# angeladai/sgnn

Measured on AMD Instinct MI355X. Metric: TSDF blocks/sec fwd+bwd (64^3@5% occ, bs32), higher is better.
Workload: dtype f32

## Files before the change

include/sgnn_hip.h:

```cpp
#ifndef SGNN_HIP_H
#define SGNN_HIP_H

#include <stdint.h>

#ifdef __cplusplus
extern "C" {
#endif

#define SGNN_OK 0
#define SGNN_EINVAL (-1)
#define SGNN_EHIP (-2)
#define SGNN_EOVERFLOW (-3)
#define SGNN_ENOWS (-4)

#define SGNN_STATUS_COORD_RANGE 1
#define SGNN_STATUS_DUPLICATE 2
#define SGNN_STATUS_OVERFLOW 4

typedef void *sgnn_stream_t;

const char *sgnn_last_error(void);
int sgnn_version(void);
const char *sgnn_arch(void);

// ... 7 lines not shown

int sgnn_hash_build(const int32_t *coords, int64_t n, uint64_t *keys, int32_t *vals, int64_t cap,
                    int32_t *status, const int64_t *n_dev, sgnn_stream_t stream);

int sgnn_hash_lookup(const uint64_t *keys, const int32_t *vals, int64_t cap, const int32_t *query,
                     int64_t m, int32_t *rows, const int64_t *m_dev, sgnn_stream_t stream);

#define SGNN_TUNE_UNKNOWN INT64_MIN
typedef struct sgnn_tune {
  int64_t conv_small;
  int64_t conv_small_rows;
  int64_t conv_unrolled;
  int64_t conv_one_round;
  int64_t conv_wide_epi;
  int64_t conv_dw_blocks;
  int64_t conv_dw_c1;
  int64_t rulebook_multi;
  int64_t scan_inline;
  int64_t chain_merged;
  int64_t prog_fusion;
  int64_t prog_lin_bn;
  int64_t prog_lin_add;
  int64_t bn_fuse;
} sgnn_tune;
int64_t sgnn_tune_set(const char *name, int64_t value);
int64_t sgnn_tune_get(const char *name);
const char *sgnn_tune_names(void);
const sgnn_tune *sgnn_tune_current(void);


int sgnn_rulebook_subm3(const uint64_t *keys, const int32_t *vals, int64_t cap,
                        const int32_t *coords, int64_t n, int32_t *nbr, int64_t ld,
                        const int64_t *n_dev, sgnn_stream_t stream);

#define SGNN_RULEBOOK_MULTI_MAX 4
int sgnn_rulebook_subm3_multi(int count, const uint64_t *const *keys, const int32_t *const *vals, const int64_t *caps,
                              const int32_t *const *coords, const int64_t *ns, int32_t *const *nbrs, const int64_t *lds,
                              const int64_t *const *n_devs, sgnn_stream_t stream);

int sgnn_rulebook_subm3_dense(const uint64_t *keys, const int32_t *vals, int64_t cap, const int32_t *coords, int64_t n,
                              int dim_z, int dim_y, int dim_x, int32_t *volume, int64_t volume_entries, int32_t *nbr,
                              int64_t ld, const int64_t *n_dev, sgnn_stream_t stream);
int sgnn_rulebook_subm3_volume(const int32_t *coords, int64_t n, int dim_z, int dim_y, int dim_x, int32_t *volume,
                               int64_t volume_entries, int32_t *nbr, int64_t ld, const int64_t *n_dev, int32_t *status,
                               sgnn_stream_t stream);

int64_t sgnn_down2_ws_bytes(int64_t nf);
int sgnn_rulebook_down2(const int32_t *fine_coords, int64_t nf, uint64_t *ckeys, int32_t *cvals,
                        int64_t ccap, int32_t *parent, int32_t *coarse_coords, int64_t *n_coarse,
                        void *ws, int64_t ws_bytes, sgnn_stream_t stream);
int sgnn_down2_tables(const int32_t *fine_coords, const int32_t *parent, int64_t nf,
                      int32_t *children, int64_t ldc, int64_t nc, int32_t *ptable, int64_t ldf,
                      const int64_t *nf_dev, const int64_t *nc_dev, sgnn_stream_t stream);

int64_t sgnn_down2_chain_ws_bytes(int64_t cap);
int sgnn_down2_chain(const int32_t *fine_coords, int64_t n0, const int64_t *n0_dev, int64_t cap, int depth,
                     void *const *ckeys, void *const *cvals, int64_t ccap, void *const *parent,
                     void *const *coarse_coords, int64_t *counts_dev, const int64_t *level_caps, int32_t *status,
                     void *ws, int64_t ws_bytes, sgnn_stream_t stream);

int64_t sgnn_down2_chain_tables_ws_bytes(int64_t cap, int depth);
int sgnn_down2_chain_tables(const int32_t *fine_coords, const int64_t *n0_dev, int64_t cap, int depth,
                            void *const *ckeys, void *const *cvals, int64_t ccap, void *const *parent,
                            void *const *coarse_coords, int64_t *counts_dev, const int64_t *level_caps,
                            void *const *children, void *const *ptable, int32_t *status, void *ws, int64_t ws_bytes,
                            sgnn_stream_t stream);

#define SGNN_CONV_TRANSPOSE_W 1
#define SGNN_CONV_FLIP_K 2
int sgnn_conv_fwd(const float *x, int64_t n_in, int cin, const float *w, int K, const int32_t *table,
                  int64_t ld, int64_t n_out, int cout, float *y, int flags, int in_shift,
                  sgnn_stream_t stream);

int sgnn_conv_fwd_ex(const float *x, int64_t n_in, int cin, const float *w, int K, const int32_t *table,
                     int64_t ld, int64_t n_out, int cout, float *y, int flags, int in_shift,
                     const int32_t *kmap, const int32_t *kadd, int in_mul, int groups, int table_rows,
                     sgnn_stream_t stream);
int sgnn_conv_bwd_weight_ex(const float *x, int64_t n_in, int cin, const float *dy, int cout,
                            const int32_t *table, int64_t ld, int K, int64_t n_out, float *dw, int in_shift,
                            const int32_t *kmap, const int32_t *kadd, int in_mul, int groups, int table_rows,
                            void *ws, int64_t ws_bytes, sgnn_stream_t stream);

int64_t sgnn_conv_stats_blocks(int64_t n_out);
int sgnn_conv_fwd_epi(const float *x, int64_t n_in, int cin, int64_t ldx, const float *w, int K,
                      const int32_t *table, int64_t ld, int64_t n_out, int cout, float *y, int64_t ldy, int flags,
                      const float *addend, int64_t ld_add, int stats, double *partial, const float *bn_x,
                      int64_t ld_bnx, const float *mean, const float *invstd, const float *gamma, const float *beta,
                      float leak, sgnn_stream_t stream);

int64_t sgnn_conv_bwd_weight_ws_bytes(int64_t n_out, int K, int cin, int cout);
int sgnn_conv_bwd_weight(const float *x, int64_t n_in, int cin, const float *dy, int cout,
                         const int32_t *table, int64_t ld, int K, int64_t n_out, float *dw, int in_shift, void *ws,
                         int64_t ws_bytes, sgnn_stream_t stream);

int sgnn_expand_weights(const float *w, int cin, int cout, float *wc, sgnn_stream_t stream);
int sgnn_expand_weights_bwd(const float *dwc, int cin, int cout, float *dw, sgnn_stream_t stream);

int64_t sgnn_bn_ws_bytes(int64_t n, int c);
int sgnn_bn_fwd(const float *x, int64_t n, int c, const float *gamma, const float *beta,
                float *running_mean, float *running_var, float eps, float momentum, int training,
                float leak, float *save_mean, float *save_invstd, float *y, void *ws,
                int64_t ws_bytes, sgnn_stream_t stream);
int sgnn_bn_bwd(const float *x, const float *dy, int64_t n, int c, const float *gamma,
                const float *beta, const float *save_mean, const float *save_invstd, int training,
                float leak, float *dx, float *dgamma, float *dbeta, void *ws, int64_t ws_bytes,
                sgnn_stream_t stream);
int sgnn_bn_bwd_add(const float *x, const float *dy, int64_t n, int c, const float *gamma, const float *beta,
                    const float *save_mean, const float *save_invstd, int training, float leak,
                    const float *addend, float *dx, float *dgamma, float *dbeta, void *ws, int64_t ws_bytes,
                    sgnn_stream_t stream);

int sgnn_bn_fwd_ex(const float *x, int64_t ldx, int64_t n, int c, const float *gamma, const float *beta,
                   float *running_mean, float *running_var, float eps, float momentum, int training, float leak,
                   float *save_mean, float *save_invstd, float *y, int64_t ldy, const double *pre_partial,
                   int64_t pre_nblk, void *ws, int64_t ws_bytes, sgnn_stream_t stream);
int sgnn_bn_bwd_ex(const float *x, int64_t ldx, const float *dy, int64_t ld_dy, int64_t n, int c, const float *gamma,
                   const float *beta, const float *save_mean, const float *save_invstd, int training, float leak,
                   const float *addend, int64_t ld_add, float *dx, int64_t ld_dx, float *dgamma, float *dbeta,
                   const double *pre_partial, int64_t pre_nblk, void *ws, int64_t ws_bytes, sgnn_stream_t stream);

int sgnn_copy_multi(void *const *dst, const void *const *src, const int64_t *bytes, int nregions, sgnn_stream_t stream);

int sgnn_gather_rows(const float *src, int c, const int32_t *idx, int64_t m, float *dst,
                     sgnn_stream_t stream);
int sgnn_gather_rows_dn(const float *src, int c, const int32_t *idx, const int64_t *m_dev, int64_t m_cap,
                        float *dst, sgnn_stream_t stream);
int sgnn_concat3_rows(const float *a, int ca, const int32_t *ia, const float *b, int cb, const int32_t *ib,
                      const float *c, int cc, const int32_t *ic, int64_t m, float *dst, sgnn_stream_t stream);
int sgnn_concat3_rows_bwd(const float *ddst, int ca, const int32_t *ia, int cb, const int32_t *ib, int cc,
                          const int32_t *ic, int64_t m, float *da, int64_t na, float *db, int64_t nb, float *dc,
                          int64_t nc, sgnn_stream_t stream);
int sgnn_scatter_rows(const float *src, int c, const int32_t *idx, int64_t m, float *dst,
                      int64_t n_dst, const int64_t *m_dev, sgnn_stream_t stream);
int sgnn_gather_sum(const float *src, int c, const int32_t *table, int64_t ld, int K,
                    int64_t n_out, float *dst, sgnn_stream_t stream);
int sgnn_repeat_rows(const float *src, int c, int64_t n, int rep, float *dst, sgnn_stream_t stream);
int sgnn_sum_groups(const float *src, int c, int64_t n, int rep, float *dst, sgnn_stream_t stream);
int sgnn_concat_rows(const float *a, int ca, const int32_t *ia, const float *b, int cb,
                     const int32_t *ib, int64_t m, float *dst, sgnn_stream_t stream);
int sgnn_concat_rows_bwd(const float *ddst, int ca, const int32_t *ia, int cb, const int32_t *ib,
                         int64_t m, float *da, int64_t na, float *db, int64_t nb,
// ... 15 lines not shown
                             int64_t *count2, int64_t keep_cap, int32_t *status, void *ws, int64_t ws_bytes,
                             sgnn_stream_t stream);
int sgnn_compact_dense_cap(const int32_t *coords, int64_t n, const int64_t *n_dev, const float *vol, int batch, int d0,
                           int d1, int d2, int32_t *sel, int64_t *count2, int64_t keep_cap, int32_t *status, void *ws,
                           int64_t ws_bytes, sgnn_stream_t stream);
int sgnn_compact_sigmoid_cap_locs(const float *logits, int64_t stride, int64_t n, const int64_t *n_dev,
                                  const int32_t *coords, int32_t *sel, int32_t *locs, int64_t *count2, int64_t keep_cap,
                                  int32_t *status, void *ws, int64_t ws_bytes, sgnn_stream_t stream);
int sgnn_compact_dense_cap_locs(const int32_t *coords, int64_t n, const int64_t *n_dev, const float *vol, int batch, int d0,
                                int d1, int d2, int32_t *sel, int32_t *locs, int64_t *count2, int64_t keep_cap,
                                int32_t *status, void *ws, int64_t ws_bytes, sgnn_stream_t stream);

int sgnn_sparse_to_dense(const float *feats, const int32_t *coords, int64_t n, int c, float *dense,
                         int batch, int d0, int d1, int d2, sgnn_stream_t stream);
int sgnn_dense_to_sparse(const float *dense, const int32_t *coords, int64_t n, int c, float *feats,
                         int batch, int d0, int d1, int d2, sgnn_stream_t stream);

int64_t sgnn_linear_ws_bytes(int64_t n, int cin, int cout);
int sgnn_linear_fwd(const float *x, int64_t n, int cin, const float *w, const float *bias, int cout,
                    float *y, sgnn_stream_t stream);
int sgnn_linear_bwd(const float *x, const float *dy, int64_t n, int cin, const float *w, int cout,
                    float *dx, float *dw, float *dbias, void *ws, int64_t ws_bytes,
                    sgnn_stream_t stream);

int64_t sgnn_loss_multi_ws_bytes(void);
int sgnn_loss_levels_fwd(const int64_t *levels, int n, const float *coef_host, double *sums, float *out2s, float *total,
                         float *cur, void *ws, int64_t ws_bytes, sgnn_stream_t stream);
int sgnn_loss_levels_bwd(const int64_t *levels, int n, const float *coef_host, const double *sums, const float *g,
                         void *const *dvals, sgnn_stream_t stream);

int sgnn_loss_targets(const float *sdf, const uint8_t *known, const int64_t *input_locs, int64_t n_locs,
                      const int64_t *n_locs_dev, int batch,
                      int d0, int d1, int d2, float trunc, int masking, float weight_missing_geo, int ncoarse,
                      void *const *hier_in, float *tsdf, float *hier_last, float *occ_last, float *w_last,
                      void *const *occ, void *const *w, void *const *hier, sgnn_stream_t stream);

int64_t sgnn_prog_arena_floats(const int32_t *ops, int nops, const int32_t *bufs, int nbuf, int n_ext,
                               const int64_t *lev_n, int nlev, const int32_t *keep, int mode);
int64_t sgnn_prog_ws_bytes(const int32_t *ops, int nops, const int64_t *lev_n, int nlev);
int64_t sgnn_prog_buffer_offset(const int32_t *ops, int nops, const int32_t *bufs, int nbuf, int n_ext,
                                const int64_t *lev_n, int nlev, const int32_t *keep, int infer, int b);
int sgnn_prog_plan(const int32_t *ops, int nops, const int32_t *bufs, int nbuf, int n_ext, const int64_t *lev_n,
                   int nlev, const int32_t *keep, int mode, int32_t *out);
int sgnn_prog_forward(const int32_t *ops, const float *opf, int nops, const int32_t *bufs, int nbuf, int n_ext,
                      const int64_t *lev_n, const int64_t *lev_ld, void *const *lev_nbr,
                      void *const *lev_children, void *const *lev_ptable, void *const *lev_parent,
                      void *const *lev_cnt, int nlev, void *const *params, int nparams,
                      void *const *ext, void *const *idx, int nidx,
                      float *arena, int64_t arena_floats, const int32_t *keep, int training, void *wait_event,
                      void *ws, int64_t ws_bytes, sgnn_stream_t stream);
int sgnn_prog_backward(const int32_t *ops, const float *opf, int nops, const int32_t *bufs, int nbuf, int n_ext,
                       const int64_t *lev_n, const int64_t *lev_ld, void *const *lev_nbr,
                       void *const *lev_children, void *const *lev_ptable, void *const *lev_parent,
                       void *const *lev_cnt, int nlev, void *const *params, void *const *pgrads,
                       int nparams, void *const *ext,
                       void *const *gext, void *const *idx, int nidx, const float *arena, float *garena,
                       int64_t arena_floats, void *const *gout, const int32_t *keep, int training, void *ws,
                       int64_t ws_bytes, sgnn_stream_t stream);

int sgnn_prog_set_side_stream(sgnn_stream_t stream2, void *ws2, int64_t ws2_bytes);
int sgnn_prog_defer_join(int on);
int64_t sgnn_bf16_conv_ws_bytes(int cin, int cout, int K, int expand);
int sgnn_bf16_conv_fwd(const void *x, int64_t n_in, int cin, int64_t ldx, const float *w, int K, const int32_t *table,
                       int64_t ld, int64_t n_out, int cout, void *y, int64_t ldy, const void *addend, int64_t ld_add,
                       const int64_t *n_dev, void *ws, int64_t ws_bytes, sgnn_stream_t stream);
int sgnn_bf16_conv_expand(const void *x, int64_t n, int cin, int64_t ldx, const float *w, const int32_t *nbr, int64_t ld,
                          int cout, void *y, int64_t ldy, const int64_t *n_dev, void *ws, int64_t ws_bytes,
                          sgnn_stream_t stream);
int sgnn_bf16_bn_eval(const void *x, int64_t ldx, int64_t n, int c, const float *gamma, const float *beta,
                      const float *running_mean, const float *running_var, float eps, float leak, void *y, int64_t ldy,
                      const int64_t *n_dev, sgnn_stream_t stream);
int sgnn_bf16_gather_rows(const void *x, int64_t ldx, int c, const int32_t *idx, int64_t m, void *y, int64_t ldy,
                          const int64_t *n_dev, sgnn_stream_t stream);
int sgnn_bf16_add(const void *a, int64_t lda, const void *b, int64_t ldb, int64_t n, int c, void *y, int64_t ldy,
                  const int64_t *n_dev, sgnn_stream_t stream);
int sgnn_bf16_join(const void *a, int64_t lda, int ca, const void *b, int64_t ldb, int cb, int64_t n, void *y, int64_t ldy,
                   const int64_t *n_dev, sgnn_stream_t stream);
int sgnn_bf16_concat3(const float *a, int ca, const int32_t *ia, const float *b, int cb, const int32_t *ib, const float *c,
                      int cc, const int32_t *ic, int64_t m, void *y, int64_t ldy, const int64_t *n_dev, sgnn_stream_t stream);
int sgnn_bf16_linear(const void *x, int64_t ldx, int64_t n, int cin, const float *w, const float *bias, int cout, float *y,
                     const int64_t *n_dev, sgnn_stream_t stream);
int sgnn_bf16_to_f32(const void *x, int64_t ldx, int64_t n, int c, float *y, const int64_t *n_dev, sgnn_stream_t stream);
int sgnn_adam_flat(float *params, const float *grads, float *exp_avg, float *exp_avg_sq, int64_t n, const int64_t *seg,
                   int nseg, const float *lr_dev, float beta1, float beta2, float eps, float weight_decay,
                   float grad_scale, const int32_t *status, sgnn_stream_t stream);
int sgnn_seg_flags(const int64_t *cnt_ptrs, int nseg, float *flags, const int32_t *status, sgnn_stream_t stream);
int sgnn_status_merge(const float *overflow_flag, int32_t *status, sgnn_stream_t stream);

int sgnn_io_layout(const void *bytes, int64_t nbytes, int kind, int64_t *out);
int sgnn_io_flag_entries(const uint32_t *locs_xyz, const float *vals, const float *voxelsize,
                         const int64_t *seg, int nb, int64_t n, float truncation, int64_t max_z,
                         uint8_t *mask, sgnn_stream_t stream);
int sgnn_io_emit_entries(const uint32_t *locs_xyz, const float *vals, const float *voxelsize,
                         const int64_t *seg, int nb, const int32_t *sel, const int64_t *count,
                         int64_t n_max, int64_t *out_locs, float *out_feats, sgnn_stream_t stream);
int sgnn_io_scatter_dense(const uint32_t *locs_xyz, const float *vals, const float *voxelsize,
                          const int64_t *seg, int nb, int64_t n, int d0, int d1, int d2, int64_t max_z,
                          float *dense, sgnn_stream_t stream);

typedef struct sgnn_fuse_frame {
  float m[12];
  float intr[4];
  int32_t box[6];
  int64_t offset;
} sgnn_fuse_frame;
int sgnn_fuse_depth_raw(const uint16_t *raw, int nframes, int h_raw, int w_raw, int h, int w, float depth_shift,
// ... 200 lines not shown
```

sgnn_amd/_lib.py:

```python
import ctypes
import os

import torch

_HERE = os.path.dirname(os.path.abspath(__file__))
LIB_PATH = os.environ.get('SGNN_LIB') or os.path.join(_HERE, 'lib', 'libsgnn_hip.so')

c_i32, c_i64, c_f32, c_vp, c_cp = ctypes.c_int, ctypes.c_int64, ctypes.c_float, ctypes.c_void_p, ctypes.c_char_p

PROTOTYPES = {
    'sgnn_last_error': (c_cp, []),
    'sgnn_version': (c_i32, []),
    'sgnn_arch': (c_cp, []),
    'sgnn_tune_set': (c_i64, [c_cp, c_i64]),
    'sgnn_tune_get': (c_i64, [c_cp]),
    'sgnn_tune_names': (c_cp, []),
    'sgnn_tune_current': (c_vp, []),
    'sgnn_hash_capacity': (c_i64, [c_i64]),
    'sgnn_coords_from_i64': (c_i32, [c_vp, c_i64, c_vp, c_vp, c_vp, c_vp]),
    'sgnn_coords_to_i64': (c_i32, [c_vp, c_i64, c_vp, c_vp, c_vp]),
    'sgnn_hash_build': (c_i32, [c_vp, c_i64, c_vp, c_vp, c_i64, c_vp, c_vp, c_vp]),
    'sgnn_hash_lookup': (c_i32, [c_vp, c_vp, c_i64, c_vp, c_i64, c_vp, c_vp, c_vp]),
    'sgnn_rulebook_subm3': (c_i32, [c_vp, c_vp, c_i64, c_vp, c_i64, c_vp, c_i64, c_vp, c_vp]),
    'sgnn_rulebook_subm3_multi': (c_i32, [c_i32, c_vp, c_vp, c_vp, c_vp, c_vp, c_vp, c_vp, c_vp, c_vp]),
    'sgnn_rulebook_subm3_dense': (c_i32, [c_vp, c_vp, c_i64, c_vp, c_i64, c_i32, c_i32, c_i32, c_vp, c_i64, c_vp, c_i64, c_vp, c_vp]),
    'sgnn_rulebook_subm3_volume': (c_i32, [c_vp, c_i64, c_i32, c_i32, c_i32, c_vp, c_i64, c_vp, c_i64, c_vp, c_vp, c_vp]),
    'sgnn_down2_ws_bytes': (c_i64, [c_i64]),
    'sgnn_rulebook_down2': (c_i32, [c_vp, c_i64, c_vp, c_vp, c_i64, c_vp, c_vp, c_vp, c_vp, c_i64, c_vp]),
    'sgnn_down2_chain_ws_bytes': (c_i64, [c_i64]),
    'sgnn_down2_chain': (c_i32, [c_vp, c_i64, c_vp, c_i64, c_i32, c_vp, c_vp, c_i64, c_vp, c_vp, c_vp, c_vp, c_vp, c_vp, c_i64, c_vp]),
    'sgnn_down2_chain_tables_ws_bytes': (c_i64, [c_i64, c_i32]),
    'sgnn_down2_chain_tables': (c_i32, [c_vp, c_vp, c_i64, c_i32, c_vp, c_vp, c_i64, c_vp, c_vp, c_vp, c_vp, c_vp, c_vp, c_vp, c_vp,
                                        c_i64, c_vp]),
    'sgnn_down2_tables': (c_i32, [c_vp, c_vp, c_i64, c_vp, c_i64, c_i64, c_vp, c_i64, c_vp, c_vp, c_vp]),
    'sgnn_conv_fwd': (c_i32, [c_vp, c_i64, c_i32, c_vp, c_i32, c_vp, c_i64, c_i64, c_i32, c_vp, c_i32, c_i32, c_vp]),
    'sgnn_conv_fwd_ex': (c_i32, [c_vp, c_i64, c_i32, c_vp, c_i32, c_vp, c_i64, c_i64, c_i32, c_vp, c_i32, c_i32, c_vp, c_vp, c_i32, c_i32, c_i32, c_vp]),
    'sgnn_conv_bwd_weight_ex': (c_i32, [c_vp, c_i64, c_i32, c_vp, c_i32, c_vp, c_i64, c_i32, c_i64, c_vp, c_i32, c_vp, c_vp, c_i32, c_i32, c_i32, c_vp, c_i64, c_vp]),
    'sgnn_conv_stats_blocks': (c_i64, [c_i64]),
    'sgnn_conv_fwd_epi': (c_i32, [c_vp, c_i64, c_i32, c_i64, c_vp, c_i32, c_vp, c_i64, c_i64, c_i32, c_vp, c_i64, c_i32, c_vp, c_i64, c_i32, c_vp, c_vp, c_i64, c_vp, c_vp, c_vp, c_vp, c_f32, c_vp]),
    'sgnn_conv_bwd_weight_ws_bytes': (c_i64, [c_i64, c_i32, c_i32, c_i32]),
    'sgnn_conv_bwd_weight': (c_i32, [c_vp, c_i64, c_i32, c_vp, c_i32, c_vp, c_i64, c_i32, c_i64, c_vp, c_i32, c_vp, c_i64, c_vp]),
    'sgnn_bn_ws_bytes': (c_i64, [c_i64, c_i32]),
    'sgnn_bn_fwd': (c_i32, [c_vp, c_i64, c_i32, c_vp, c_vp, c_vp, c_vp, c_f32, c_f32, c_i32, c_f32, c_vp, c_vp, c_vp, c_vp, c_i64, c_vp]),
    'sgnn_bn_bwd': (c_i32, [c_vp, c_vp, c_i64, c_i32, c_vp, c_vp, c_vp, c_vp, c_i32, c_f32, c_vp, c_vp, c_vp, c_vp, c_i64, c_vp]),
    'sgnn_bn_bwd_add': (c_i32, [c_vp, c_vp, c_i64, c_i32, c_vp, c_vp, c_vp, c_vp, c_i32, c_f32, c_vp, c_vp, c_vp, c_vp, c_vp, c_i64, c_vp]),
    'sgnn_bn_fwd_ex': (c_i32, [c_vp, c_i64, c_i64, c_i32, c_vp, c_vp, c_vp, c_vp, c_f32, c_f32, c_i32, c_f32, c_vp, c_vp, c_vp, c_i64, c_vp, c_i64, c_vp, c_i64, c_vp]),
    'sgnn_bn_bwd_ex': (c_i32, [c_vp, c_i64, c_vp, c_i64, c_i64, c_i32, c_vp, c_vp, c_vp, c_vp, c_i32, c_f32, c_vp, c_i64, c_vp, c_i64, c_vp, c_vp, c_vp, c_i64, c_vp, c_i64, c_vp]),
    'sgnn_copy_multi': (c_i32, [c_vp, c_vp, c_vp, c_i32, c_vp]),
    'sgnn_gather_rows': (c_i32, [c_vp, c_i32, c_vp, c_i64, c_vp, c_vp]),
    'sgnn_gather_rows_dn': (c_i32, [c_vp, c_i32, c_vp, c_vp, c_i64, c_vp, c_vp]),
    'sgnn_scatter_rows': (c_i32, [c_vp, c_i32, c_vp, c_i64, c_vp, c_i64, c_vp, c_vp]),
    'sgnn_gather_sum': (c_i32, [c_vp, c_i32, c_vp, c_i64, c_i32, c_i64, c_vp, c_vp]),
    'sgnn_repeat_rows': (c_i32, [c_vp, c_i32, c_i64, c_i32, c_vp, c_vp]),
    'sgnn_sum_groups': (c_i32, [c_vp, c_i32, c_i64, c_i32, c_vp, c_vp]),
    'sgnn_concat_rows': (c_i32, [c_vp, c_i32, c_vp, c_vp, c_i32, c_vp, c_i64, c_vp, c_vp]),
    'sgnn_concat_rows_bwd': (c_i32, [c_vp, c_i32, c_vp, c_i32, c_vp, c_i64, c_vp, c_i64, c_vp, c_i64, c_vp]),
    'sgnn_add': (c_i32, [c_vp, c_vp, c_i64, c_vp, c_vp]),
    'sgnn_expand8_coords': (c_i32, [c_vp, c_i64, c_vp, c_vp, c_vp]),
    'sgnn_expand8_coords_i64': (c_i32, [c_vp, c_i64, c_vp, c_vp, c_vp, c_vp]),
    'sgnn_dense_coords': (c_i32, [c_i32, c_i32, c_i32, c_i32, c_vp, c_vp]),
    'sgnn_compact_ws_bytes': (c_i64, [c_i64]),
    'sgnn_compact_sigmoid': (c_i32, [c_vp, c_i64, c_i64, c_vp, c_vp, c_vp, c_i64, c_vp]),
    'sgnn_compact_dense': (c_i32, [c_vp, c_i64, c_vp, c_i32, c_i32, c_i32, c_i32, c_vp, c_vp, c_vp, c_i64, c_vp]),
    'sgnn_compact_mask': (c_i32, [c_vp, c_i64, c_vp, c_vp, c_vp, c_i64, c_vp]),
    'sgnn_compact_sigmoid_cap': (c_i32, [c_vp, c_i64, c_i64, c_vp, c_vp, c_vp, c_i64, c_vp, c_vp, c_i64, c_vp]),
    'sgnn_compact_dense_cap': (c_i32, [c_vp, c_i64, c_vp, c_vp, c_i32, c_i32, c_i32, c_i32, c_vp, c_vp, c_i64, c_vp, c_vp, c_i64, c_vp]),
    'sgnn_compact_sigmoid_cap_locs': (c_i32, [c_vp, c_i64, c_i64, c_vp, c_vp, c_vp, c_vp, c_vp, c_i64, c_vp, c_vp, c_i64, c_vp]),
    'sgnn_compact_dense_cap_locs': (c_i32, [c_vp, c_i64, c_vp, c_vp, c_i32, c_i32, c_i32, c_i32, c_vp, c_vp, c_vp, c_i64, c_vp, c_vp, c_i64, c_vp]),
    'sgnn_adam_flat': (c_i32, [c_vp, c_vp, c_vp, c_vp, c_i64, c_vp, c_i32, c_vp, c_f32, c_f32, c_f32, c_f32, c_f32, c_vp, c_vp]),
    'sgnn_seg_flags': (c_i32, [c_vp, c_i32, c_vp, c_vp, c_vp]),
    'sgnn_status_merge': (c_i32, [c_vp, c_vp, c_vp]),
    'sgnn_sparse_to_dense': (c_i32, [c_vp, c_vp, c_i64, c_i32, c_vp, c_i32, c_i32, c_i32, c_i32, c_vp]),
    'sgnn_dense_to_sparse': (c_i32, [c_vp, c_vp, c_i64, c_i32, c_vp, c_i32, c_i32, c_i32, c_i32, c_vp]),
    'sgnn_linear_ws_bytes': (c_i64, [c_i64, c_i32, c_i32]),
    'sgnn_linear_fwd': (c_i32, [c_vp, c_i64, c_i32, c_vp, c_vp, c_i32, c_vp, c_vp]),
    'sgnn_linear_bwd': (c_i32, [c_vp, c_vp, c_i64, c_i32, c_vp, c_i32, c_vp, c_vp, c_vp, c_vp, c_i64, c_vp]),
    'sgnn_loss_targets': (c_i32, [c_vp, c_vp, c_vp, c_i64, c_vp, c_i32, c_i32, c_i32, c_i32, c_f32, c_i32, c_f32, c_i32, c_vp, c_vp, c_vp,
                                  c_vp, c_vp, c_vp, c_vp, c_vp, c_vp]),
    'sgnn_loss_multi_ws_bytes': (c_i64, []),
    'sgnn_loss_levels_fwd': (c_i32, [c_vp, c_i32, c_vp, c_vp, c_vp, c_vp, c_vp, c_vp, c_i64, c_vp]),
    'sgnn_loss_levels_bwd': (c_i32, [c_vp, c_i32, c_vp, c_vp, c_vp, c_vp, c_vp]),
    'sgnn_prog_arena_floats': (c_i64, [c_vp, c_i32, c_vp, c_i32, c_i32, c_vp, c_i32, c_vp, c_i32]),
    'sgnn_prog_ws_bytes': (c_i64, [c_vp, c_i32, c_vp, c_i32]),
    'sgnn_prog_buffer_offset': (c_i64, [c_vp, c_i32, c_vp, c_i32, c_i32, c_vp, c_i32, c_vp, c_i32, c_i32]),
    'sgnn_prog_plan': (c_i32, [c_vp, c_i32, c_vp, c_i32, c_i32, c_vp, c_i32, c_vp, c_i32, c_vp]),
    'sgnn_prog_set_side_stream': (c_i32, [c_vp, c_vp, c_i64]),
    'sgnn_prog_defer_join': (c_i32, [c_i32]),
    'sgnn_bf16_conv_ws_bytes': (c_i64, [c_i32, c_i32, c_i32, c_i32]),
    'sgnn_bf16_conv_fwd': (c_i32, [c_vp, c_i64, c_i32, c_i64, c_vp, c_i32, c_vp, c_i64, c_i64, c_i32, c_vp, c_i64, c_vp,
                                   c_i64, c_vp, c_vp, c_i64, c_vp]),
    'sgnn_bf16_conv_expand': (c_i32, [c_vp, c_i64, c_i32, c_i64, c_vp, c_vp, c_i64, c_i32, c_vp, c_i64, c_vp, c_vp, c_i64,
                                      c_vp]),
    'sgnn_bf16_bn_eval': (c_i32, [c_vp, c_i64, c_i64, c_i32, c_vp, c_vp, c_vp, c_vp, c_f32, c_f32, c_vp, c_i64, c_vp, c_vp]),
    'sgnn_bf16_gather_rows': (c_i32, [c_vp, c_i64, c_i32, c_vp, c_i64, c_vp, c_i64, c_vp, c_vp]),
    'sgnn_bf16_add': (c_i32, [c_vp, c_i64, c_vp, c_i64, c_i64, c_i32, c_vp, c_i64, c_vp, c_vp]),
    'sgnn_bf16_join': (c_i32, [c_vp, c_i64, c_i32, c_vp, c_i64, c_i32, c_i64, c_vp, c_i64, c_vp, c_vp]),
    'sgnn_bf16_concat3': (c_i32, [c_vp, c_i32, c_vp, c_vp, c_i32, c_vp, c_vp, c_i32, c_vp, c_i64, c_vp, c_i64, c_vp, c_vp]),
    'sgnn_bf16_linear': (c_i32, [c_vp, c_i64, c_i64, c_i32, c_vp, c_vp, c_i32, c_vp, c_vp, c_vp]),
    'sgnn_bf16_to_f32': (c_i32, [c_vp, c_i64, c_i64, c_i32, c_vp, c_vp, c_vp]),
    'sgnn_prog_forward': (c_i32, [c_vp, c_vp, c_i32, c_vp, c_i32, c_i32, c_vp, c_vp, c_vp, c_vp, c_vp, c_vp, c_vp, c_i32, c_vp,
                                  c_i32, c_vp, c_vp, c_i32, c_vp, c_i64, c_vp, c_i32, c_vp, c_vp, c_i64, c_vp]),
    'sgnn_prog_backward': (c_i32, [c_vp, c_vp, c_i32, c_vp, c_i32, c_i32, c_vp, c_vp, c_vp, c_vp, c_vp, c_vp, c_vp, c_i32, c_vp,
                                   c_vp, c_i32, c_vp, c_vp, c_vp, c_i32, c_vp, c_vp, c_i64, c_vp, c_vp, c_i32, c_vp, c_i64, c_vp]),
    'sgnn_concat3_rows': (c_i32, [c_vp, c_i32, c_vp, c_vp, c_i32, c_vp, c_vp, c_i32, c_vp, c_i64, c_vp, c_vp]),
    'sgnn_concat3_rows_bwd': (c_i32, [c_vp, c_i32, c_vp, c_i32, c_vp, c_i32, c_vp, c_i64, c_vp, c_i64, c_vp, c_i64, c_vp,
                                      c_i64, c_vp]),
    'sgnn_expand_weights': (c_i32, [c_vp, c_i32, c_i32, c_vp, c_vp]),
    'sgnn_expand_weights_bwd': (c_i32, [c_vp, c_i32, c_i32, c_vp, c_vp]),
    'sgnn_io_layout': (c_i32, [c_vp, c_i64, c_i32, c_vp]),
    'sgnn_io_flag_entries': (c_i32, [c_vp, c_vp, c_vp, c_vp, c_i32, c_i64, c_f32, c_i64, c_vp, c_vp]),
    'sgnn_io_emit_entries': (c_i32, [c_vp, c_vp, c_vp, c_vp, c_i32, c_vp, c_vp, c_i64, c_vp, c_vp, c_vp]),
    'sgnn_io_scatter_dense': (c_i32, [c_vp, c_vp, c_vp, c_vp, c_i32, c_i64, c_i32, c_i32, c_i32, c_i64, c_vp, c_vp]),
    'sgnn_fuse_depth_raw': (c_i32, [c_vp, c_i32, c_i32, c_i32, c_i32, c_i32, c_f32, c_f32, c_f32, c_vp, c_vp]),
    'sgnn_fuse_bilateral': (c_i32, [c_vp, c_i32, c_i32, c_i32, c_f32, c_f32, c_vp, c_vp]),
    'sgnn_fuse_integrate': (c_i32, [c_vp, c_vp, c_vp, c_i32, c_i32, c_i32, c_vp, c_i32, c_i32, c_vp, c_i32, c_i32, c_f32,
                                    c_f32, c_f32, c_vp, c_vp]),
    'sgnn_fuse_flag': (c_i32, [c_vp, c_i32, c_i32, c_i32, c_f32, c_f32, c_f32, c_i64, c_vp, c_vp]),
    'sgnn_fuse_emit_block': (c_i32, [c_vp, c_i32, c_i32, c_vp, c_vp, c_i64, c_vp, c_vp, c_vp]),
    'sgnn_fuse_emit_rows': (c_i32, [c_vp, c_i32, c_i32, c_f32, c_vp, c_vp, c_i64, c_vp, c_vp, c_vp]),
    'sgnn_fuse_known': (c_i32, [c_vp, c_i64, c_f32, c_vp, c_vp]),
    'sgnn_fusecol_pack': (c_i32, [c_vp, c_i32, c_i32, c_i32, c_i32, c_i32, c_i32, c_vp, c_vp]),
    'sgnn_fusecol_integrate': (c_i32, [c_vp, c_vp, c_vp, c_vp, c_i32, c_i32, c_i32, c_vp, c_vp, c_i32, c_i32, c_vp, c_i32,
                                       c_i32, c_f32, c_f32, c_f32, c_vp, c_vp]),
    'sgnn_fusecol_export': (c_i32, [c_vp, c_i64, c_vp, c_vp, c_vp]),
    'sgnn_chunk_score': (c_i32, [c_vp, c_vp, c_i32, c_i32, c_i32, c_f32, c_f32, c_f32, c_i32, c_i32, c_i32, c_i32, c_i32,
                                 c_i32, c_i32, c_i32, c_i32, c_vp, c_vp, c_vp]),
    'sgnn_chunk_flag': (c_i32, [c_vp, c_i32, c_i32, c_i32, c_vp, c_i32, c_i32, c_i32, c_i32, c_f32, c_f32, c_f32, c_vp,
                                c_vp]),
    'sgnn_chunk_emit_rows': (c_i32, [c_vp, c_i32, c_i32, c_i32, c_vp, c_i32, c_i32, c_i32, c_i32, c_f32, c_vp, c_vp,
                                     c_i64, c_vp, c_vp, c_vp]),
    'sgnn_chunk_crop': (c_i32, [c_vp, c_i32, c_i32, c_i32, c_vp, c_i32, c_i32, c_i32, c_i32, c_i32, c_f32, c_f32, c_vp,
                                c_vp, c_vp]),
    'sgnn_render_depth': (c_i32, [c_vp, c_i32, c_vp, c_i32, c_vp, c_i32, c_i32, c_i32, c_i32, c_f32, c_f32, c_f32, c_i32,
                                  c_vp, c_vp, c_vp, c_vp]),
    'sgnn_rendercol_draw': (c_i32, [c_vp, c_i32, c_vp, c_i32, c_vp, c_i32, c_i32, c_i32, c_i32, c_f32, c_f32, c_f32,
                                    c_i32, c_vp, c_vp, c_vp, c_vp, c_vp, c_vp, c_vp]),
    'sgnn_meshdist_pack': (c_i32, [c_vp, c_i32, c_vp, c_i32, c_vp, c_vp, c_vp, c_vp, c_vp]),
    'sgnn_meshdist_count': (c_i32, [c_vp, c_i32, c_f32, c_f32, c_f32, c_f32, c_i32, c_i32, c_i32, c_vp, c_vp]),
    'sgnn_meshdist_fill': (c_i32, [c_vp, c_i32, c_f32, c_f32, c_f32, c_f32, c_i32, c_i32, c_i32, c_vp, c_vp, c_vp, c_vp]),
    'sgnn_meshdist_query': (c_i32, [c_vp, c_i64, c_vp, c_vp, c_vp, c_f32, c_f32, c_f32, c_f32, c_f32, c_f32, c_f32, c_i32,
                                    c_i32, c_i32, c_f32, c_vp, c_vp, c_vp, c_vp]),
    'sgnn_mesh_sample': (c_i32, [c_vp, c_vp, c_i32, c_i32, c_i64, c_i64, c_vp, c_vp, c_vp]),
    'sgnn_raycast_bricks': (c_i32, [c_vp, c_i32, c_i32, c_i32, c_f32, c_vp, c_vp]),
    'sgnn_raycast_cast': (c_i32, [c_vp, c_i32, c_i32, c_i32, c_f32, c_vp, c_vp, c_i32, c_i32, c_i32, c_i32, c_f32, c_f32,
                                  c_i32, c_vp, c_vp, c_vp, c_vp]),
    'sgnn_raycol_cast': (c_i32, [c_vp, c_i32, c_i32, c_i32, c_f32, c_vp, c_vp, c_i32, c_i32, c_i32, c_i32, c_f32, c_f32,
                                 c_i32, c_vp, c_vp, c_vp, c_vp, c_vp, c_vp]),
    'sgnn_track_halve': (c_i32, [c_vp, c_i32, c_i32, c_i32, c_f32, c_vp, c_vp]),
    'sgnn_track_normals': (c_i32, [c_vp, c_vp, c_i32, c_i32, c_i32, c_f32, c_vp, c_vp]),
    'sgnn_track_system': (c_i32, [c_vp, c_vp, c_i32, c_i32, c_vp, c_vp, c_i32, c_i32, c_vp, c_i32, c_f32, c_f32, c_vp, c_vp,
                                  c_vp, c_vp, c_i64, c_vp]),
    'sgnn_cc_volume_link': (c_i32, [c_vp, c_i32, c_i32, c_i32, c_i32, c_i32, c_i32, c_vp, c_vp]),
    'sgnn_cc_mesh_link': (c_i32, [c_vp, c_i32, c_i32, c_vp, c_vp, c_vp]),
    'sgnn_cc_flatten': (c_i32, [c_vp, c_i64, c_vp, c_vp]),
    'sgnn_cc_relabel': (c_i32, [c_vp, c_i64, c_vp, c_i64, c_vp, c_vp, c_vp]),
# ... 150 lines not shown
```

sgnn_amd/csrc/common.h:

```cpp
#pragma once
#include <hip/hip_runtime.h>
#include <stdint.h>
#include <stdio.h>
#include "../../include/sgnn_hip.h"

#define SGNN_EXPORT extern "C" __attribute__((visibility("default")))

extern "C" int sgnn_stamp(const char *label, sgnn_stream_t stream);
extern sgnn_tune g_tune;

void sgnn_set_error(const char *fmt, ...);
int sgnn_prof_begin_launch(int kind, int64_t n_out, int cin, int cout, int K, int flags, hipStream_t s);
void sgnn_prof_end_launch(int slot, hipStream_t s);

__device__ __forceinline__ float sgnn_bn_act(float x, float mean, float invstd, float gamma, float beta, float leak) {
  const float xh = (x - mean) * invstd;
  const float t = fmaf(xh, gamma, beta);
  return t > 0.f ? t : t * leak;
}

struct ConvEpi {
  int64_t ldx, ldy, ld_add;
  const float *addend;
  int stats;
  double *partial;
  const float *bn_x;
  int64_t ld_bnx;
  const float *mean, *invstd, *gamma, *beta;
  float leak;
  const int64_t *n_dev;
};

int sgnn_conv_fwd_impl(const float *x, int64_t n_in, int cin, const float *w, int K, const int32_t *table, int64_t ld,
                       int64_t n_out, int cout, float *y, int flags, int in_shift, const int32_t *kmap,
                       const int32_t *kadd, int in_mul, int groups, int table_rows, const ConvEpi *epi,
                       sgnn_stream_t stream);
int64_t sgnn_conv_grid_blocks(int64_t n_out, int cin, int cout, int K);
struct BnLin {
  const float *g;
  int64_t ldg;
  const float *w[2];
  int nout;
};
int sgnn_bn_fwd_impl(const float *x, int64_t ldx, int64_t n, int c, const float *gamma, const float *beta,
                     float *running_mean, float *running_var, float eps, float momentum, int training, float leak,
                     float *save_mean, float *save_invstd, float *y, int64_t ldy, const double *pre_partial,
                     int64_t pre_nblk, void *ws, int64_t ws_bytes, sgnn_stream_t stream, const int64_t *n_dev = nullptr);
int sgnn_bn_bwd_impl(const float *x, int64_t ldx, const float *dy, int64_t ld_dy, int64_t n, int c, const float *gamma,
                     const float *beta, const float *save_mean, const float *save_invstd, int training, float leak,
                     const float *addend, int64_t ld_add, float *dx, int64_t ld_dx, float *dgamma, float *dbeta,
                     const double *pre_partial, int64_t pre_nblk, void *ws, int64_t ws_bytes, sgnn_stream_t stream,
                     const int64_t *n_dev = nullptr, const struct BnLin *lin = nullptr);
bool sgnn_conv_epi_supported(int cin, int cout);
bool dw_shape_ok(int cin, int cout);
#define DW_BATCH_MAX 28
struct DwDesc {
  const float *partial;
  float *dw;
  int64_t nblk, elems;
  int blk0;
};
struct DwBatch {
  DwDesc d[DW_BATCH_MAX];
  int n;
};
extern DwBatch *sgnn_dw_batch;
int sgnn_dw_batch_flush(DwBatch *b, hipStream_t s);
int sgnn_gather_rows_ld(const float *src, int64_t ld_src, int c, const int32_t *idx, int64_t m, float *dst,
                        int64_t ld_dst, sgnn_stream_t stream, const int64_t *n_dev = nullptr);
int sgnn_gather_sum_ld(const float *src, int64_t ld_src, int c, const int32_t *table, int64_t ld, int K, int64_t n_out,
                       float *dst, int64_t ld_dst, sgnn_stream_t stream, const int64_t *n_dev = nullptr);
int sgnn_add_ld(const float *a, int64_t lda, const float *b, int64_t ldb, int64_t n, int c, float *y, int64_t ldy,
                sgnn_stream_t stream, const int64_t *n_dev = nullptr);
int sgnn_fill32(void *p, uint32_t pattern, int64_t words, hipStream_t s);
int sgnn_fill32_multi(void *const *p, const int64_t *words, int nregions, uint32_t pattern, hipStream_t s);
int sgnn_copy_words(void *dst, const void *src, int64_t words, hipStream_t s);
int sgnn_sum_groups_dn(const float *src, int c, int64_t n, int rep, float *dst, sgnn_stream_t stream, const int64_t *n_dev);
int sgnn_concat_rows_dn(const float *a, int ca, const int32_t *ia, const float *b, int cb, const int32_t *ib, int64_t m,
                        float *dst, sgnn_stream_t stream, const int64_t *n_dev);
int sgnn_concat_rows_bwd_dn(const float *ddst, int ca, const int32_t *ia, int cb, const int32_t *ib, int64_t m, float *da,
                            int64_t na, float *db, int64_t nb, sgnn_stream_t stream, const int64_t *n_dev);
int sgnn_concat3_rows_dn(const float *a, int ca, const int32_t *ia, const float *b, int cb, const int32_t *ib,
                         const float *c, int cc, const int32_t *ic, int64_t m, float *dst, sgnn_stream_t stream,
                         const int64_t *n_dev);
int sgnn_concat3_rows_bwd_dn(const float *ddst, int ca, const int32_t *ia, int cb, const int32_t *ib, int cc,
                             const int32_t *ic, int64_t m, float *da, int64_t na, float *db, int64_t nb, float *dc,
                             int64_t nc, sgnn_stream_t stream, const int64_t *n_dev);
int sgnn_conv_bwd_weight_impl(const float *x, int64_t n_in, int cin, int64_t ldx, const float *dy, int cout, int64_t ld_dy,
                              const int32_t *table, int64_t ld, int K, int64_t n_out, float *dw, int in_shift,
// ... 121 lines not shown
```

sgnn_amd/csrc/conv.hip:

```cpp
#include <stdlib.h>
#include "common.h"

#include "conv_common.h"

#define CONV_SMALL_GRID ((int64_t)((g_tune.conv_small_rows + CONV_ROWS_PER_BLOCK - 1) / CONV_ROWS_PER_BLOCK))

template <int CIN, int COUT, int M, bool EX, bool WEPI>
__device__ __forceinline__ void conv_fwd_body(const float *__restrict__ x, int64_t n_in,
                                              const float *__restrict__ w, const int32_t *__restrict__ table,
                                              int64_t ld, int K, int64_t n_out, float *y, int flags,
                                              int in_shift, const ConvEx &ex, const ConvEpi &epi, int wg_cap) {
  using C = ConvCfg<CIN, COUT>;
  constexpr int V = C::V, CINP = C::CINP, NT = C::NT, KC = C::KC;
  constexpr int RPW = 16 * M;
  __shared__ __attribute__((aligned(16))) float wl[KC * C::PER_K];
  __shared__ double sred[4 * 2 * NT * 16];
  static_assert(!WEPI || (NT == 1 && M == 4 && !EX && COUT % 4 == 0), "wide epilogue: one column tile of whole 16-byte chunks");
  __shared__ float ecst[WEPI ? 64 : 1];

  const int tid = threadIdx.x, lane = tid & 63, wave = tid >> 6;
  const int r = lane & 15, q = lane >> 4;
  const unsigned groups = EX ? (unsigned)ex.groups : 1u;
  unsigned nwg = gridDim.x;
  if (epi.n_dev) n_out = sgnn_dyn_n(n_out, epi.n_dev);
// ... 140 lines not shown
      const int kc = (K - k0) < KC ? (K - k0) : KC;
      if (restage) stage(k0);
      int32_t iv1 = idx_at(k0 + 1), iv2 = idx_at(k0 + 2);
      gather(idx_at(k0), a0);
      load_b(0, b0);
      int kk = 0;
      for (; kk + 1 < kc; kk += 2) {
        gather(iv1, a1);
        const int32_t iv3 = idx_at(k0 + kk + 3);
        load_b(kk + 1, b1);
        __builtin_amdgcn_sched_barrier(0);
        mma_b(a0, b0);
        __builtin_amdgcn_sched_barrier(0);
        gather(iv2, a0);
        iv1 = iv3;
        iv2 = idx_at(k0 + kk + 4);
        load_b(kk + 2 < kc ? kk + 2 : kc - 1, b0);
        __builtin_amdgcn_sched_barrier(0);
        mma_b(a1, b1);
        __builtin_amdgcn_sched_barrier(0);
      }
      if constexpr (WEPI) {
        __builtin_amdgcn_sched_barrier(0);
        if constexpr (SGNN_WEPI_EARLY != 0) conv_epi_wide_prefetch<COUT, M>(erows, row0, n_out, epi, epi.stats, x, SGNN_WEPI_EARLY);
        __builtin_amdgcn_sched_barrier(0);
      }
      if (kk < kc) mma_b(a0, b0);
    }
  }

  if constexpr (WEPI)
    conv_epi_wide_finish<COUT, M>(acc, erows, row0, n_out, y, epi, epi.stats, ecst, s1, s2, x);
  else
    conv_epilogue_rows<COUT, M, NT>(acc, row0, n_out, groups, grp, y, epi, EX ? 0 : epi.stats, x, s1, s2);
  }
  conv_epilogue_stats<COUT, NT>(s1, s2, epi, EX ? 0 : epi.stats, sred, blockIdx.x);
}

template <int CIN, int COUT, int M, bool EX>
__global__ __launch_bounds__(256) void k_conv_fwd(const float *__restrict__ x, int64_t n_in,
                                                 const float *__restrict__ w, const int32_t *__restrict__ table,
                                                 int64_t ld, int K, int64_t n_out, float *y, int flags,
                                                 int in_shift, ConvEx ex, ConvEpi epi, int wg_cap) {
  conv_fwd_body<CIN, COUT, M, EX, false>(x, n_in, w, table, ld, K, n_out, y, flags, in_shift, ex, epi, wg_cap);
}

template <int CIN, int COUT>
__global__ __launch_bounds__(256) __attribute__((amdgpu_waves_per_eu(4, 8))) void k_conv_fwd_w(
    const float *__restrict__ x, int64_t n_in, const float *__restrict__ w, const int32_t *__restrict__ table, int64_t ld,
    int K, int64_t n_out, float *y, int flags, int in_shift, ConvEx ex, ConvEpi epi, int wg_cap) {
  conv_fwd_body<CIN, COUT, CONV_MREP, false, true>(x, n_in, w, table, ld, K, n_out, y, flags, in_shift, ex, epi, wg_cap);
}

template <int CIN, int COUT>
__global__ __launch_bounds__(256) void k_conv_small(const float *__restrict__ x, int64_t n_in,
                                                   const float *__restrict__ w, const int32_t *__restrict__ table,
                                                   int64_t ld, int K, int64_t n_out, float *y, int flags, int in_shift,
                                                   ConvEpi epi) {
  using C = ConvCfg<CIN, COUT>;
  constexpr int V = C::V, CINP = C::CINP, NT = C::NT;
  constexpr int KW = 7;
  __shared__ float red[4][NT * 256];
  __shared__ double sred[4][2][NT * 16];
  const int tid = threadIdx.x, lane = tid & 63, wave = tid >> 6;
  const int r = lane & 15, q = lane >> 4;
  const int64_t row0 = (int64_t)blockIdx.x * 16;
  if (epi.n_dev) {
    n_out = sgnn_dyn_n(n_out, epi.n_dev);
    if (row0 >= n_out) {
      if (epi.stats)
        for (int o = tid; o < 2 * COUT; o += 256) epi.partial[(size_t)blockIdx.x * 2 * COUT + o] = 0.0;
      return;
    }
  }
  const bool transpose = flags & SGNN_CONV_TRANSPOSE_W, flip = flags & SGNN_CONV_FLIP_K;
  const int per = (K + 3) >> 2;
  const int k0 = wave * per;
  const int nk = (K - k0) < per ? ((K - k0) > 0 ? (K - k0) : 0) : per;

  const uint32_t ldx4 = (uint32_t)epi.ldx * 4u, ldy4 = (uint32_t)epi.ldy * 4u;
  const __amdgpu_buffer_rsrc_t rs_x = make_rsrc(x, (uint32_t)(((n_in - 1) * epi.ldx + CIN) * 4));
  const __amdgpu_buffer_rsrc_t rs_t = make_rsrc(table, (uint32_t)((int64_t)K * ld * 4));
  const __amdgpu_buffer_rsrc_t rs_y = make_rsrc(y, (uint32_t)(((n_out - 1) * epi.ldy + COUT) * 4));
  const uint32_t lane_off = (uint32_t)(row0 + r) * 4u;
  const uint32_t ld4 = (uint32_t)ld * 4u;

  int32_t id[KW];
#pragma unroll
  for (int kk = 0; kk < KW; ++kk) {
    const int k = k0 + (kk < nk ? kk : (nk > 0 ? nk - 1 : 0));
    id[kk] = (int32_t)__builtin_amdgcn_raw_buffer_load_b32(rs_t, lane_off, (k < K ? k : K - 1) * ld4, 0) >> in_shift;
  }
  float a[KW][V];
#pragma unroll
  for (int kk = 0; kk < KW; ++kk) buf_load_floats<V>(rs_x, (uint32_t)id[kk] * ldx4 + (uint32_t)(q * V * 4), a[kk]);
  float b[KW][NT][V];
  if (transpose) {
    const __amdgpu_buffer_rsrc_t rs_w = make_rsrc(w, (uint32_t)((int64_t)K * CIN * COUT * 4));
#pragma unroll
    for (int kk = 0; kk < KW; ++kk) {
      const int k = k0 + kk;
      const int ks = flip ? (K - 1 - k) : k;
#pragma unroll
      for (int nt = 0; nt < NT; ++nt) {
        const int n = nt * 16 + r;
        const bool okw = kk < nk && n < COUT;
        buf_load_floats<V>(rs_w, okw ? (uint32_t)((ks * COUT + n) * CIN + q * V) * 4u : 0xFFFFF800u, b[kk][nt]);
        if constexpr (CINP != CIN) {
#pragma unroll
          for (int s = 0; s < V; ++s)
            if (3 * V + s >= CIN) b[kk][nt][s] = (q >= conv_first_pad_quarter<CIN, V>(s)) ? 0.f : b[kk][nt][s];
        }
      }
    }
  } else if constexpr (V == 4 && CIN <= 16 && (CIN * COUT) % 4 == 0) {
    constexpr int SL = CIN * COUT, G4 = SL / 4, NL = (G4 + 63) / 64;
    static_assert(SL <= NT * 256, "the weight slice must fit the wave's partial-tile buffer");
    float *ws = red[wave];
    const __amdgpu_buffer_rsrc_t rs_w = make_rsrc(w, (uint32_t)((int64_t)K * SL * 4));
    float g[KW][NL][4];
#pragma unroll
    for (int kk = 0; kk < KW; ++kk) {
      const int k = k0 + kk;
      const int ks = flip ? (K - 1 - k) : k;
#pragma unroll
      for (int l = 0; l < NL; ++l) {
        const int e4 = l * 64 + lane;
        buf_load_floats<4>(rs_w, (kk < nk && e4 < G4) ? (uint32_t)(ks * SL + e4 * 4) * 4u : 0xFFFFF800u, g[kk][l]);
      }
    }
    auto wave_sync = [] {
      __builtin_amdgcn_fence(__ATOMIC_RELEASE, "wavefront");
      __builtin_amdgcn_wave_barrier();
      __builtin_amdgcn_fence(__ATOMIC_ACQUIRE, "wavefront");
    };
#pragma unroll
    for (int kk = 0; kk < KW; ++kk) {
      wave_sync();
#pragma unroll
      for (int l = 0; l < NL; ++l) {
        const int e4 = l * 64 + lane;
        if (e4 < G4) {
#pragma unroll
          for (int j = 0; j < 4; ++j) ws[e4 * 4 + j] = g[kk][l][j];
// ... 95 lines not shown
        f1 = (double)dz;
        f2 = (double)dz * (double)xh;
      }
      f1 += __shfl_xor(f1, 16); f2 += __shfl_xor(f2, 16);
      f1 += __shfl_xor(f1, 32); f2 += __shfl_xor(f2, 32);
      if (lane < 16) {
        sred[wave][0][nt * 16 + lane] = f1;
        sred[wave][1][nt * 16 + lane] = f2;
      }
    }
  }
  if (stats) {
    __syncthreads();
    for (int o = tid; o < 2 * NT * 16; o += 256) {
      const int which = o / (NT * 16), col = o % (NT * 16);
      if (col < COUT)
        epi.partial[((size_t)blockIdx.x * 2 + which) * COUT + col] =
            (sred[0][which][col] + sred[1][which][col]) + (sred[2][which][col] + sred[3][which][col]);
    }
  }
}

__global__ __launch_bounds__(256) void k_conv_fwd_generic(const float *__restrict__ x, int cin,
                                                         const float *__restrict__ w, int K,
                                                         const int32_t *__restrict__ table, int64_t ld,
                                                         int64_t n_out, int cout, float *__restrict__ y,
                                                         int flags, int in_shift, ConvEx ex, const int64_t *n_dev) {
  n_out = sgnn_dyn_n(n_out, n_dev);
  const int64_t t = (int64_t)blockIdx.x * 256 + threadIdx.x;
  if (t >= n_out * ex.groups * cout) return;
  const int64_t orow = t / cout;
  const int n = (int)(t - orow * cout);
  const int64_t row = orow / ex.groups;
  const int grp = (int)(orow - row * ex.groups);
  w += (int64_t)grp * K * cin * cout;
  const bool transpose = flags & SGNN_CONV_TRANSPOSE_W, flip = flags & SGNN_CONV_FLIP_K;
  float acc = 0.f;
  for (int k = 0; k < K; ++k) {
    const int32_t idx = table[(int64_t)(ex.kmap ? ex.kmap[grp * K + k] : k) * ld + row];
    if (idx < 0) continue;
    const float *xr = x + ((int64_t)(idx >> in_shift) * ex.in_mul + (ex.kadd ? ex.kadd[grp * K + k] : 0)) * cin;
    const int ks = flip ? (K - 1 - k) : k;
    for (int c = 0; c < cin; ++c) {
      const float wv = transpose ? w[((int64_t)ks * cout + n) * cin + c] : w[((int64_t)ks * cin + c) * cout + n];
      acc = fmaf(xr[c], wv, acc);
    }
  }
  y[t] = acc;
}

#define CONV_EX_CASES(X) \
  X(48, 16) X(16, 48) X(24, 8) X(8, 24) X(16, 24) X(24, 16) X(24, 32) X(32, 24) X(64, 32) X(32, 64) X(56, 28) X(28, 56)

#define CONV_FWD_CASES(X) \
  X(1, 8) X(8, 8) X(8, 12) X(12, 12) X(12, 16) X(16, 16) X(34, 16) X(30, 16) X(26, 16) X(48, 16) \
  X(8, 1) X(12, 8) X(16, 12) X(16, 34) X(16, 30) X(16, 26) X(16, 48) X(32, 16) X(16, 32) X(4, 16) X(16, 4) \
  X(16, 24) X(24, 16) X(24, 32) X(32, 24) X(64, 32) X(32, 64) X(56, 28) X(28, 56) X(32, 32) X(28, 16) X(16, 28)

int64_t sgnn_conv_grid_blocks(int64_t n_out, int cin, int cout, int K) {
  const int64_t grid4 = (n_out + CONV_ROWS_PER_BLOCK - 1) / CONV_ROWS_PER_BLOCK;
  if (grid4 < CONV_SMALL_GRID) return (n_out + 15) / 16;
  return grid4;
}


bool sgnn_conv_u_supported(int cin, int cout, int K);
bool sgnn_conv_u_launch(const float *x, int64_t n_in, int cin, const float *w, int K, const int32_t *table, int64_t ld,
                        int64_t n_out, int cout, float *y, int flags, int in_shift, const ConvEpi &epi, hipStream_t s);

bool conv_wide_epi_ok(const ConvEpi &epi, const float *y, int K) {
  if (!g_tune.conv_wide_epi || K > 27 || (epi.ldy & 3) || ((uintptr_t)y & 15)) return false;
  if (epi.addend && ((epi.ld_add & 3) || ((uintptr_t)epi.addend & 15))) return false;
  if (epi.stats == 2 && ((epi.ld_bnx & 3) || ((uintptr_t)epi.bn_x & 15))) return false;
  return true;
}
template <int CI, int CO, bool EXV>
static void conv_launch_big(unsigned grid4, hipStream_t s, const float *x, int64_t n_in, const float *w, const int32_t *table,
                            int64_t ld, int K, int64_t n_out, float *y, int flags, int in_shift, const ConvEx &ex,
                            const ConvEpi &epi) {
  if constexpr (!EXV && CO % 4 == 0 && CO <= 16 && CI <= 16) {
    static_assert(ConvCfg<CI, CO>::KC >= 27, "one weight chunk holds a 3x3x3 filter");
    if (conv_wide_epi_ok(epi, y, K)) {
      SGNN_LAUNCH((k_conv_fwd_w<CI, CO>), dim3(grid4), dim3(256), 0, s, x, n_in, w, table, ld, K, n_out, y, flags, in_shift,
                  ex, epi, !g_tune.conv_one_round ? 0 : conv_wg_capacity<k_conv_fwd_w<CI, CO>>());
      return;
    }
  }
  SGNN_LAUNCH((k_conv_fwd<CI, CO, CONV_MREP, EXV>), dim3(grid4), dim3(256), 0, s, x, n_in, w, table, ld, K, n_out, y,
              flags, in_shift, ex, epi,
              (EXV || !g_tune.conv_one_round) ? 0 : conv_wg_capacity<k_conv_fwd<CI, CO, CONV_MREP, EXV>>());
}

bool sgnn_conv_epi_supported(int cin, int cout) {
#define X(CI, CO) \
  if (cin == CI && cout == CO) return true;
  CONV_FWD_CASES(X)
#undef X
  return false;
}

int sgnn_conv_fwd_impl(const float *x, int64_t n_in, int cin, const float *w, int K, const int32_t *table, int64_t ld,
                       int64_t n_out, int cout, float *y, int flags, int in_shift, const int32_t *kmap,
                       const int32_t *kadd, int in_mul, int groups, int table_rows, const ConvEpi *epi_in,
                       sgnn_stream_t stream) {
  SGNN_CHECK_ARG(cin >= 1 && cout >= 1 && K >= 1 && K <= 64 && n_out >= 0 && ld >= n_out && in_shift >= 0 &&
                 in_shift < 31 && in_mul >= 1 && groups >= 1 && groups <= 64 && table_rows >= 1 &&
                 table_rows <= 64 && (kmap || table_rows >= K));
  if (n_out == 0) return SGNN_OK;
  SGNN_CHECK_ARG(x && w && table && y && n_in >= 1);
  SGNN_CHECK_ARG(ld % CONV_ROWS_PER_BLOCK == 0);
// ... 36 lines not shown
    else                                                                                                \
      conv_launch_big<CI, CO, EXV>(grid4, s, x, n_in, w, table, ld, K, n_out, y, flags, in_shift, ex, epi); \
    done = true;                                                                                        \
  } while (0)
  if (plain && !small && g_tune.conv_unrolled && sgnn_conv_u_supported(cin, cout, K))
    done = sgnn_conv_u_launch(x, n_in, cin, w, K, table, ld, n_out, cout, y, flags, in_shift, epi, s);
#define X(CI, CO) \
  if (!done && plain && cin == CI && cout == CO) LAUNCH_FWD(CI, CO, false);
  CONV_FWD_CASES(X)
#undef X
#define X(CI, CO) \
  if (!done && !plain && cin == CI && cout == CO) LAUNCH_FWD(CI, CO, true);
  CONV_EX_CASES(X)
#undef X
  if (!done) {
    if (has_epi) {
      sgnn_set_error("sgnn_conv_fwd_epi: strided / fused epilogues need one of the compiled (cin, cout) shapes, got (%d, %d)", cin, cout);
      return SGNN_EINVAL;
    }
    const int64_t total = n_out * groups * cout;
    SGNN_LAUNCH(k_conv_fwd_generic, dim3((unsigned)((total + 255) / 256)), dim3(256), 0, s, x, cin, w, K,
                       table, ld, n_out, cout, y, flags, in_shift, ex, epi.n_dev);
  }
  sgnn_prof_end_launch(prof, s);
  SGNN_CHECK_LAUNCH();
  return SGNN_OK;
}

SGNN_EXPORT int sgnn_conv_fwd_ex(const float *x, int64_t n_in, int cin, const float *w, int K, const int32_t *table,
                                 int64_t ld, int64_t n_out, int cout, float *y, int flags, int in_shift,
                                 const int32_t *kmap, const int32_t *kadd, int in_mul, int groups,
                                 int table_rows, sgnn_stream_t stream) {
  return sgnn_conv_fwd_impl(x, n_in, cin, w, K, table, ld, n_out, cout, y, flags, in_shift, kmap, kadd, in_mul,
                            groups, table_rows, nullptr, stream);
}

SGNN_EXPORT int sgnn_conv_fwd(const float *x, int64_t n_in, int cin, const float *w, int K, const int32_t *table,
                              int64_t ld, int64_t n_out, int cout, float *y, int flags, int in_shift,
                              sgnn_stream_t stream) {
  return sgnn_conv_fwd_impl(x, n_in, cin, w, K, table, ld, n_out, cout, y, flags, in_shift, nullptr, nullptr, 1, 1,
                            K, nullptr, stream);
}

SGNN_EXPORT int64_t sgnn_conv_stats_blocks(int64_t n_out) { return n_out > 0 ? sgnn_conv_grid_blocks(n_out, 0, 0, 0) : 0; }

SGNN_EXPORT int sgnn_conv_fwd_epi(const float *x, int64_t n_in, int cin, int64_t ldx, const float *w, int K,
                                  const int32_t *table, int64_t ld, int64_t n_out, int cout, float *y, int64_t ldy,
                                  int flags, const float *addend, int64_t ld_add, int stats, double *partial,
                                  const float *bn_x, int64_t ld_bnx, const float *mean, const float *invstd,
                                  const float *gamma, const float *beta, float leak, sgnn_stream_t stream) {
  ConvEpi epi{ldx, ldy, ld_add, addend, stats, partial, bn_x, ld_bnx, mean, invstd, gamma, beta, leak, nullptr};
  return sgnn_conv_fwd_impl(x, n_in, cin, w, K, table, ld, n_out, cout, y, flags, 0, nullptr, nullptr, 1, 1, K, &epi,
                            stream);
}

__device__ int32_t g_expand_maps[192];

int sgnn_expand_maps(const int32_t **S, const int32_t **ST, const int32_t **PAR) {
  static const int32_t *base = nullptr;
  if (!base) {
    int32_t host[192];
    for (int g = 0; g < 8; ++g)
      for (int i = 0; i < 8; ++i) {
        const int o0 = ((i >> 2) & 1) - 1 + ((g >> 2) & 1), o1 = ((i >> 1) & 1) - 1 + ((g >> 1) & 1),
                  o2 = (i & 1) - 1 + (g & 1);
        const int srow = (o0 + 1) * 9 + (o1 + 1) * 3 + (o2 + 1);
        host[g * 8 + i] = srow;
        host[64 + g * 8 + i] = 26 - srow;
        host[128 + g * 8 + i] = g;
      }
    SGNN_HIP_TRY(hipMemcpyToSymbol(HIP_SYMBOL(g_expand_maps), host, sizeof(host)));
    void *p = nullptr;
    SGNN_HIP_TRY(hipGetSymbolAddress(&p, HIP_SYMBOL(g_expand_maps)));
    base = (const int32_t *)p;
  }
  *S = base;
  *ST = base + 64;
  *PAR = base + 128;
  return SGNN_OK;
}

__device__ __forceinline__ void axis_taps(int j, int i, int &lo, int &hi) {
  if (j == 0) { lo = i ? 0 : -1; hi = i ? 1 : -1; }
  else        { lo = i ? 1 : -1; hi = i ? 1 : 0; }
}

__global__ __launch_bounds__(256) void k_expand_weights(const float *__restrict__ w, int cc, float *__restrict__ wc) {
  const int t = blockIdx.x * 256 + threadIdx.x;
  if (t >= 64 * cc) return;
  const int gi = t / cc, e = t - gi * cc, g = gi >> 3, i = gi & 7;
  int l0, h0, l1, h1, l2, h2;
  axis_taps((g >> 2) & 1, (i >> 2) & 1, l0, h0);
  axis_taps((g >> 1) & 1, (i >> 1) & 1, l1, h1);
  axis_taps(g & 1, i & 1, l2, h2);
  float acc = 0.f;
  for (int dz = l0; dz <= h0; ++dz)
    for (int dy = l1; dy <= h1; ++dy)
      for (int dx = l2; dx <= h2; ++dx) acc += w[(size_t)((dz + 1) * 9 + (dy + 1) * 3 + (dx + 1)) * cc + e];
  wc[t] = acc;
}

__global__ __launch_bounds__(256) void k_expand_weights_bwd(const float *__restrict__ dwc, int cc,
                                                           float *__restrict__ dw) {
  const int t = blockIdx.x * 256 + threadIdx.x;
  if (t >= 27 * cc) return;
  const int tap = t / cc, e = t - tap * cc;
// ... 593 lines not shown
```

sgnn_amd/csrc/conv_common.h:

```cpp
#pragma once
#include <atomic>
#include "common.h"

typedef float f32x4 __attribute__((ext_vector_type(4)));

#define CONV_MREP 4
#define CONV_ROWS_PER_WAVE (16 * CONV_MREP)
#define CONV_ROWS_PER_BLOCK (4 * CONV_ROWS_PER_WAVE)

template <int CIN, int COUT>
struct ConvCfg {
  static constexpr int V = (CIN + 3) / 4;
  static constexpr int CINP = 4 * V;
  static constexpr int NT = (COUT + 15) / 16;
  static constexpr int PER_K = NT * 16 * CINP;
#ifndef CONV_LDS_FLOATS
#define CONV_LDS_FLOATS 8192
#endif
  static constexpr int KC_RAW = CONV_LDS_FLOATS / PER_K;
  static constexpr int KC = KC_RAW < 1 ? 1 : (KC_RAW > 27 ? 27 : KC_RAW);
#ifndef CONV_RESIDENT_LDS_BYTES
#if defined(__HIP_DEVICE_COMPILE__) && !defined(__gfx950__)
#define CONV_RESIDENT_LDS_BYTES 0
#else
#define CONV_RESIDENT_LDS_BYTES 98304
#endif
#endif
  static constexpr int RESIDENT_BYTES = 27 * PER_K * 4 + 4 * 2 * NT * 16 * 8;
  static constexpr int KC27 = (RESIDENT_BYTES <= CONV_RESIDENT_LDS_BYTES) ? 27 : KC;
  static constexpr int ALIGN = ((CIN % 4 == 0) && (V % 4 == 0)) ? 16 : (((CIN % 2 == 0) && (V % 2 == 0)) ? 8 : 4);
};

template <int CIN, int V>
__device__ __forceinline__ constexpr int conv_first_pad_quarter(int s) { return (CIN - s + V - 1) / V; }

struct ConvEx {
  const int32_t *kmap;
  const int32_t *kadd;
  int in_mul;
  int groups;
  int table_rows;
};

template <auto KERNEL>
static int conv_wg_capacity() {
  static std::atomic<int> cache[16];
  int dev = 0;
  if (hipGetDevice(&dev) != hipSuccess) return 0;
  const int slot = dev & 15;
  const int have = cache[slot].load(std::memory_order_relaxed);
  if (have > 0 && (dev < 16)) return have - 1;
  int per_cu = 0, cus = 0;
  if (hipOccupancyMaxActiveBlocksPerMultiprocessor(&per_cu, KERNEL, 256, 0) != hipSuccess ||
      hipDeviceGetAttribute(&cus, hipDeviceAttributeMultiprocessorCount, dev) != hipSuccess)
    return 0;
  if (dev < 16) cache[slot].store(per_cu * cus + 1, std::memory_order_relaxed);
  return per_cu * cus;
}

typedef unsigned int u32x2 __attribute__((ext_vector_type(2)));
typedef unsigned int u32x3 __attribute__((ext_vector_type(3)));
// ... 279 lines not shown
```

sgnn_amd/csrc/conv_unrolled.hip:

```cpp
#include "conv_common.h"

template <int CIN, int COUT, int K, bool WEPI>
__device__ __forceinline__ void conv_fwd_u_body(const float *__restrict__ x, int64_t n_in, const float *__restrict__ w,
                                                const int32_t *__restrict__ table, int64_t ld, int64_t n_out, float *y,
                                                int flags, int in_shift, const ConvEpi &epi, int wg_cap) {
  using C = ConvCfg<CIN, COUT>;
  constexpr int V = C::V, CINP = C::CINP, NT = C::NT, M = 4;
  constexpr int KC = C::KC27 < K ? C::KC27 : K;
  static_assert(KC < 27 || C::RESIDENT_BYTES <= 80 * 1024 || (CIN == 16 && COUT == 34), "resident weight image costs a workgroup per CU");
  __shared__ __attribute__((aligned(16))) float wl[KC * C::PER_K];
  __shared__ double sred[4 * 2 * NT * 16];
  static_assert(!WEPI || (NT == 1 && COUT % 4 == 0), "wide epilogue: one column tile of whole 16-byte chunks");
  __shared__ float ecst[WEPI ? 64 : 1];

  const int tid = threadIdx.x, lane = tid & 63, wave = tid >> 6;
  const int r = lane & 15, q = lane >> 4;
  unsigned nwg = gridDim.x;
  if (epi.n_dev) n_out = sgnn_dyn_n(n_out, epi.n_dev);
  int J = 1;
  if (wg_cap > 0) {
    J = (int)(((n_out + 255) / 256 + wg_cap - 1) / wg_cap);
    if (J < 1) J = 1;
  }
  if (epi.n_dev || J > 1) {
    nwg = (unsigned)((n_out + 256 * (int64_t)J - 1) / (256 * (int64_t)J));
    if (blockIdx.x >= nwg) {
      if (epi.stats)
        for (int o = tid; o < 2 * COUT; o += 256) epi.partial[(size_t)blockIdx.x * 2 * COUT + o] = 0.0;
      return;
    }
  }
  const unsigned tile = sgnn_xcd_tile(blockIdx.x, nwg);
  const bool transpose = flags & SGNN_CONV_TRANSPOSE_W, flip = flags & SGNN_CONV_FLIP_K;

  const uint32_t ldx4 = (uint32_t)epi.ldx * 4u;
  const __amdgpu_buffer_rsrc_t rs_x = make_rsrc(x, (uint32_t)(((n_in - 1) * epi.ldx + CIN) * 4));
  const __amdgpu_buffer_rsrc_t rs_t = make_rsrc(table, (uint32_t)((int64_t)K * ld * 4));
  const uint32_t ld4 = (uint32_t)ld * 4u;
  int perm[M];
#pragma unroll
  for (int m = 0; m < M; ++m) perm[m] = (m * 16 + r) * 4;
  double s1[NT], s2[NT];
#pragma unroll
  for (int nt = 0; nt < NT; ++nt) s1[nt] = s2[nt] = 0.0;
  int32_t idx[K];
  f32x4 acc[M][NT];
  if constexpr (WEPI) conv_epi_wide_constants<COUT>(ecst, epi, epi.stats);

  float a[2][M][V];
  auto gather = [&](int k) {
#pragma unroll
    for (int m = 0; m < M; ++m) {
      const int32_t id = __builtin_amdgcn_ds_bpermute(perm[m], idx[k]);
      buf_load_floats<V>(rs_x, (uint32_t)id * ldx4 + (uint32_t)(q * V * 4), a[k & 1][m]);
    }
  };
  auto stage = [&](int k0) {
    conv_stage_weights<CIN, COUT>(wl, w, K, k0, (K - k0) < KC ? (K - k0) : KC, transpose, flip);
  };
  float bf[2][NT][V];
  auto load_b = [&](int k) {
    const int kk = k % KC;
#pragma unroll
    for (int nt = 0; nt < NT; ++nt) {
      const float *bp = wl + (kk * NT * 16 + nt * 16 + r) * CINP + q * V;
#pragma unroll
      for (int s = 0; s < V; ++s) bf[k & 1][nt][s] = bp[s];
    }
  };
  auto mma = [&](int k) {
    const float(&b)[NT][V] = bf[k & 1];
#pragma unroll
    for (int s = 0; s < V; ++s)
#pragma unroll
      for (int m = 0; m < M; ++m) {
        float av = a[k & 1][m][s];
        if constexpr (CINP != CIN)
          if (3 * V + s >= CIN) av = (q >= conv_first_pad_quarter<CIN, V>(s)) ? 0.f : av;
#pragma unroll
        for (int nt = 0; nt < NT; ++nt)
          acc[m][nt] = __builtin_amdgcn_mfma_f32_16x16x4f32(av, b[nt][s], acc[m][nt], 0, 0, 0);
      }
  };

  for (int j = 0; j < J; ++j) {
  const int64_t wg_row0 = ((int64_t)tile * J + j) * 256;
  if (j > 0 && wg_row0 >= n_out) break;
  const int64_t row0 = wg_row0 + wave * 64;
  const uint32_t lane_off = (uint32_t)(row0 + lane) * 4u;
#pragma unroll
  for (int k = 0; k < K; ++k)
    idx[k] = (int32_t)__builtin_amdgcn_raw_buffer_load_b32(rs_t, lane_off, k * ld4, 0) >> in_shift;
#pragma unroll
  for (int m = 0; m < M; ++m)
#pragma unroll
    for (int nt = 0; nt < NT; ++nt) acc[m][nt] = f32x4{0.f, 0.f, 0.f, 0.f};
  gather(0);
  EpiRows<WEPI ? M : 1> erows;
#pragma unroll
  for (int k = 0; k < K; ++k) {
    if (k % KC == 0) {
      if (KC < K || j == 0) stage(k);
      load_b(k);
    }
    if (k + 1 < K) gather(k + 1);
    if (k + 1 < K && (k + 1) % KC != 0) load_b(k + 1);
    if constexpr (WEPI) {
      if (k == K - 1) conv_epi_wide_prefetch<COUT, M>(erows, row0, n_out, epi, epi.stats, x);
    }
    __builtin_amdgcn_sched_barrier(0);
    mma(k);
    __builtin_amdgcn_sched_barrier(0);
  }

  if constexpr (WEPI)
    conv_epi_wide_finish<COUT, M>(acc, erows, row0, n_out, y, epi, epi.stats, ecst, s1, s2, x);
  else
    conv_epilogue_rows<COUT, M, NT>(acc, row0, n_out, 1u, 0u, y, epi, epi.stats, x, s1, s2);
  }
  conv_epilogue_stats<COUT, NT>(s1, s2, epi, epi.stats, sred, blockIdx.x);
}

template <int CIN, int COUT, int K>
__global__ __launch_bounds__(256) void k_conv_fwd_u(const float *__restrict__ x, int64_t n_in, const float *__restrict__ w,
                                                   const int32_t *__restrict__ table, int64_t ld, int64_t n_out, float *y,
                                                   int flags, int in_shift, ConvEpi epi, int wg_cap) {
  conv_fwd_u_body<CIN, COUT, K, false>(x, n_in, w, table, ld, n_out, y, flags, in_shift, epi, wg_cap);
}

template <int CIN, int COUT>
__global__ __launch_bounds__(256) __attribute__((amdgpu_waves_per_eu(4, 8))) void k_conv_fwd_uw(
    const float *__restrict__ x, int64_t n_in, const float *__restrict__ w, const int32_t *__restrict__ table, int64_t ld,
    int64_t n_out, float *y, int flags, int in_shift, ConvEpi epi, int wg_cap) {
  conv_fwd_u_body<CIN, COUT, 8, true>(x, n_in, w, table, ld, n_out, y, flags, in_shift, epi, wg_cap);
}

#define CONV_U_CASES_27(X) X(34, 16) X(16, 34) X(30, 16) X(16, 30) X(26, 16) X(16, 26)
#define CONV_U_CASES_8(X) X(8, 8) X(8, 12) X(12, 8) X(12, 12) X(12, 16) X(16, 12) X(16, 16)

bool sgnn_conv_u_supported(int cin, int cout, int K) {
#define X(CI, CO) \
  if (K == 27 && cin == CI && cout == CO) return true;
  CONV_U_CASES_27(X)
#undef X
#define X(CI, CO) \
  if (K == 8 && cin == CI && cout == CO) return true;
  CONV_U_CASES_8(X)
#undef X
  return false;
}

bool conv_wide_epi_ok(const ConvEpi &epi, const float *y, int K);

template <int CI, int CO, int KK>
static void conv_u_launch_plain(unsigned grid, hipStream_t s, const float *x, int64_t n_in, const float *w, const int32_t *table,
                                int64_t ld, int64_t n_out, float *y, int flags, int in_shift, const ConvEpi &epi) {
  if constexpr (KK == 8 && CO % 4 == 0 && CO <= 16) {
    if (conv_wide_epi_ok(epi, y, KK)) {
      SGNN_LAUNCH((k_conv_fwd_uw<CI, CO>), dim3(grid), dim3(256), 0, s, x, n_in, w, table, ld, n_out, y, flags, in_shift, epi,
                  g_tune.conv_one_round ? conv_wg_capacity<k_conv_fwd_uw<CI, CO>>() : 0);
      return;
    }
  }
  SGNN_LAUNCH((k_conv_fwd_u<CI, CO, KK>), dim3(grid), dim3(256), 0, s, x, n_in, w, table, ld, n_out, y, flags, in_shift,
              epi, g_tune.conv_one_round ? conv_wg_capacity<k_conv_fwd_u<CI, CO, KK>>() : 0);
}

bool sgnn_conv_u_launch(const float *x, int64_t n_in, int cin, const float *w, int K, const int32_t *table, int64_t ld,
                        int64_t n_out, int cout, float *y, int flags, int in_shift, const ConvEpi &epi, hipStream_t s) {
  const unsigned grid = (unsigned)((n_out + 255) / 256);
#define X(CI, CO)                                                                                    \
  if (K == 27 && cin == CI && cout == CO) {                                                          \
    conv_u_launch_plain<CI, CO, 27>(grid, s, x, n_in, w, table, ld, n_out, y, flags, in_shift, epi); \
    return true;                                                                                     \
  }
  CONV_U_CASES_27(X)
#undef X
#define X(CI, CO)                                                                                   \
  if (K == 8 && cin == CI && cout == CO) {                                                          \
    conv_u_launch_plain<CI, CO, 8>(grid, s, x, n_in, w, table, ld, n_out, y, flags, in_shift, epi); \
    return true;                                                                                    \
  }
  CONV_U_CASES_8(X)
#undef X
  return false;
}
```

sgnn_amd/csrc/grid_rules.hip:

```cpp
#include <stdarg.h>
#include "common.h"

static thread_local char g_err[512] = "";

void sgnn_set_error(const char *fmt, ...) {
  va_list ap;
  va_start(ap, fmt);
  vsnprintf(g_err, sizeof(g_err), fmt, ap);
  va_end(ap);
}

SGNN_EXPORT const char *sgnn_last_error(void) { return g_err; }
SGNN_EXPORT int sgnn_version(void) { return 100; }
SGNN_EXPORT const char *sgnn_arch(void) { return "gfx950"; }

SGNN_EXPORT int64_t sgnn_hash_capacity(int64_t n) {
  const int64_t want = 4 * n < 262144 ? 4 * n : (2 * n > 262144 ? 2 * n : 262144);
  int64_t cap = 1024;
  while (cap < want) cap <<= 1;
  return cap;
}

__global__ __launch_bounds__(256) void k_coords_from_i64(const int64_t *__restrict__ locs, int64_t n,
                                                        int4 *__restrict__ coords, int32_t *status,
// ... 789 lines not shown
  }
  if ((threadIdx.x & 63) == 0) lds[threadIdx.x >> 6] = cnt;
  __syncthreads();
  if (threadIdx.x == 0) block_sums[blockIdx.x] = lds[0] + lds[1] + lds[2] + lds[3];
}

__global__ __launch_bounds__(256) void k_chain_emit(const int4 *__restrict__ fine, const int32_t *__restrict__ slot_of,
                                                   const int32_t *__restrict__ owner, const int64_t *n_dev,
                                                   int64_t n_host, const int32_t *block_offsets,
                                                   int4 *__restrict__ coarse, int32_t *__restrict__ rank_at, ScanInline si) {
  __shared__ int lds[8];
  const int64_t n = sgnn_dyn_n(n_host, n_dev);
  int running;
  if (si.nblk > 0) {
    int64_t total;
    scan_offsets_inline(block_offsets, si.nblk, blockIdx.x, lds, running, total);
    scan_publish(total, si.count, si.lim, blockIdx.x == 0 && threadIdx.x == 0);
  } else {
    running = block_offsets[blockIdx.x];
  }
  scan_emit_rows(FlagOwner{slot_of, owner}, EmitOwner{fine, coarse, rank_at}, n, running, lds);
}

__global__ __launch_bounds__(256) void k_chain_emit2(const int4 *__restrict__ fine, const int32_t *__restrict__ slot_of,
                                                    const int32_t *__restrict__ owner, const int64_t *n_dev,
                                                    int64_t n_host, const int32_t *block_offsets,
                                                    int4 *__restrict__ coarse, int32_t *__restrict__ rank_at,
                                                    const int64_t *nc_dev, int32_t *__restrict__ children, int64_t ldc,
                                                    ScanInline si) {
  __shared__ int lds[8];
  const int64_t n = sgnn_dyn_n(n_host, n_dev);
  int running = 0;
  int64_t nc_live;
  if (si.nblk > 0) {
    int64_t total;
    scan_offsets_inline(block_offsets, si.nblk, blockIdx.x, lds, running, total);
    nc_live = scan_publish(total, si.count, si.lim, blockIdx.x == 0 && threadIdx.x == 0);
  } else {
    nc_live = sgnn_dyn_n(ldc, nc_dev);
  }
  {
    const int64_t end = pad_end(nc_live, ldc);
    const int64_t total = end * 8, stride = (int64_t)gridDim.x * 256;
    for (int64_t g = (int64_t)blockIdx.x * 256 + threadIdx.x; g < total; g += stride) children[(g / end) * ldc + (g % end)] = -1;
  }
  if ((int64_t)blockIdx.x * SCAN_BLOCK >= n) return;
  if (si.nblk <= 0) running = block_offsets[blockIdx.x];
  scan_emit_rows(FlagOwner{slot_of, owner}, EmitOwner{fine, coarse, rank_at}, n, running, lds);
}

template <bool Record>
__device__ __forceinline__ void down2_table_row(int64_t i, bool pad, const int4 *__restrict__ fine, int32_t p, int64_t nc,
                                                int32_t *__restrict__ parent, int32_t *__restrict__ children, int64_t ldc,
                                                int32_t *__restrict__ ptable, int64_t ldf) {
  int off = -1;
  if (!pad) {
    if (p >= nc) p = -1;
    if (Record) parent[i] = p;
    const int4 c = fine[i];
    off = ((c.x & 1) << 2) | ((c.y & 1) << 1) | (c.z & 1);
    if (p >= 0) children[(int64_t)off * ldc + p] = (int32_t)i;
  }
#pragma unroll
  for (int k = 0; k < 8; ++k) ptable[(int64_t)k * ldf + i] = (k == off) ? p : -1;
}

struct ChainTables {
  const int4 *fine;
  const int64_t *n_dev;
  int64_t n_host;
  const int32_t *owner, *rank_at, *slot_of;
  int32_t *parent, *cvals;
  const int64_t *nc_dev;
  int64_t nc_cap;
  int32_t *children;
  int64_t ldc;
  int32_t *ptable;
  int64_t ldf;
};

template <bool Tables>
__device__ __forceinline__ void chain_parent_rows(const int4 *__restrict__ fine, const int64_t *n_dev, int64_t n_host,
                                                  const int32_t *__restrict__ owner,
                                                  const int32_t *__restrict__ rank_at,
                                                  const int32_t *__restrict__ slot_of,
                                                  int32_t *__restrict__ parent, int32_t *__restrict__ cvals,
                                                  const int64_t *nc_dev, int64_t nc_cap,
                                                  int32_t *__restrict__ children, int64_t ldc,
                                                  int32_t *__restrict__ ptable, int64_t ldf) {
  const int64_t nf = sgnn_dyn_n(n_host, n_dev);
  const int64_t nc = Tables ? sgnn_dyn_n(nc_cap, nc_dev) : 0;
  const int64_t iend = Tables ? pad_end(nf, ldf) : nf;
  int64_t i = (int64_t)blockIdx.x * 256 + threadIdx.x;
  const int64_t stride = (int64_t)gridDim.x * 256;
  for (; i < iend; i += stride) {
    if (Tables && i >= nf) {
      down2_table_row<false>(i, true, fine, -1, nc, nullptr, children, ldc, ptable, ldf);
      continue;
    }
    const int32_t sl = slot_of[i];
    const int32_t p = rank_at[owner[sl]];
    if (rank_at[i] >= 0) cvals[sl] = p;
    if (Tables) down2_table_row<true>(i, false, fine, p, nc, parent, children, ldc, ptable, ldf);
    else parent[i] = p;
  }
}

__global__ __launch_bounds__(256) void k_chain_parent(const int64_t *n_dev, int64_t n_host,
                                                     const int32_t *__restrict__ owner,
                                                     const int32_t *__restrict__ rank_at,
                                                     const int32_t *__restrict__ slot_of,
                                                     int32_t *__restrict__ parent, int32_t *__restrict__ cvals) {
  chain_parent_rows<false>(nullptr, n_dev, n_host, owner, rank_at, slot_of, parent, cvals, nullptr, 0, nullptr, 0, nullptr, 0);
}

__global__ __launch_bounds__(256) void k_chain_parent_tables(ChainTables t) {
  chain_parent_rows<true>(t.fine, t.n_dev, t.n_host, t.owner, t.rank_at, t.slot_of, t.parent, t.cvals, t.nc_dev, t.nc_cap,
                          t.children, t.ldc, t.ptable, t.ldf);
}

__global__ __launch_bounds__(256) void k_chain_tables_insert(ChainTables t, unsigned long long *__restrict__ ckeys_next,
                                                            int32_t *__restrict__ owner_next, uint64_t mask,
                                                            int32_t *__restrict__ slot_of_next, const int4 *coarse,
                                                            int64_t n_host_next) {
  chain_parent_rows<true>(t.fine, t.n_dev, t.n_host, t.owner, t.rank_at, t.slot_of, t.parent, t.cvals, t.nc_dev, t.nc_cap,
                          t.children, t.ldc, t.ptable, t.ldf);
  chain_insert_rows(coarse, t.nc_dev, n_host_next, ckeys_next, owner_next, mask, slot_of_next);
}

static void chain_launch_init(const ChainInit &ini, int levels, hipStream_t s) {
  SGNN_LAUNCH(k_chain_init_all, dim3(sgnn_grid_for(ini.ccap, 256, 4096), levels), dim3(256), 0, s, ini);
}

static void chain_launch_insert(const int4 *fine, const int64_t *n_dev, int64_t n_host, int64_t cap, void *ckeys,
                                const ChainScratch &w, int64_t ccap, hipStream_t s) {
  SGNN_LAUNCH(k_chain_insert, dim3(sgnn_grid_for(cap, 256, 8192)), dim3(256), 0, s, fine, n_dev, n_host,
              (unsigned long long *)ckeys, w.owner, (uint64_t)(ccap - 1), w.slot_of);
}

static ScanInline chain_launch_count(const ChainScratch &w, const int64_t *n_dev, int64_t n_host, int64_t cap,
                                     int32_t *block_sums, int64_t *count, const ScanLimit &lim, hipStream_t s) {
  const int64_t nblk = (cap + SCAN_BLOCK - 1) / SCAN_BLOCK;
  SGNN_LAUNCH((k_scan_count<FlagOwner>), dim3((unsigned)nblk), dim3(256), 0, s, FlagOwner{w.slot_of, w.owner}, n_host,
              block_sums, n_dev);
  if (scan_inline_ok(nblk)) return ScanInline{nblk, count, lim};
  SGNN_LAUNCH(k_scan_block_sums, dim3(1), dim3(1024), 0, s, block_sums, nblk, count, lim);
  return kNoInline;
}

SGNN_EXPORT int64_t sgnn_down2_ws_bytes(int64_t nf) { return chain_ws_bytes(nf, sgnn_hash_capacity(nf), 1); }
SGNN_EXPORT int64_t sgnn_down2_chain_ws_bytes(int64_t cap) { return chain_ws_bytes(cap, sgnn_hash_capacity(cap), 1); }
SGNN_EXPORT int64_t sgnn_down2_chain_tables_ws_bytes(int64_t cap, int depth) {
  return chain_ws_bytes(cap, sgnn_hash_capacity(cap), depth);
}

static int chain_hip_result(const char *who, hipError_t e) {
  if (e == hipSuccess) return SGNN_OK;
  sgnn_set_error("%s: HIP error: %s", who, hipGetErrorString(e));
  return SGNN_EHIP;
}

static int down2_chain(const char *who, const int32_t *fine_coords, int64_t n0, const int64_t *n0_dev, int64_t cap,
                       int depth, void *const *ckeys, void *const *cvals, int64_t ccap, void *const *parent,
                       void *const *coarse_coords, int64_t *counts_dev, const int64_t *level_caps, int32_t *status,
                       void *ws, int64_t ws_bytes, hipStream_t s) {
  if (cap == 0) {
    hipError_t e = hipMemsetAsync(counts_dev, 0, depth * sizeof(int64_t), s);
    for (int l = 0; l < depth && e == hipSuccess; ++l) e = hipMemsetAsync(ckeys[l], 0xFF, (size_t)ccap * sizeof(uint64_t), s);
    return chain_hip_result(who, e);
  }
  if (!ws || ws_bytes < chain_ws_bytes(cap, ccap, 1)) {
    sgnn_set_error("%s: workspace too small", who);
    return SGNN_ENOWS;
  }
  ChainScratch w;
  int32_t *block_sums = chain_ws_carve(ws, cap, ccap, 1, &w);
  const int4 *fine = (const int4 *)fine_coords;
  const int64_t *n_dev = n0_dev;
  int64_t n_host = n0_dev ? cap : n0;
  const int64_t nblk = (cap + SCAN_BLOCK - 1) / SCAN_BLOCK;
  const int g = sgnn_grid_for(cap, 256, 8192);
  const bool inl = scan_inline_ok(nblk);
  for (int l = 0; l < depth; ++l) {
    SGNN_LAUNCH(k_chain_init, dim3(sgnn_grid_for(ccap, 256, 4096)), dim3(256), 0, s, (unsigned long long *)ckeys[l],
                w.owner, ccap, w.rank_at, cap);
    chain_launch_insert(fine, n_dev, n_host, cap, ckeys[l], w, ccap, s);
    SGNN_LAUNCH(k_chain_count, dim3((unsigned)nblk), dim3(256), 0, s, (const int32_t *)w.slot_of,
                (const int32_t *)w.owner, n_dev, n_host, block_sums);
    const ScanLimit lim = level_caps ? ScanLimit{level_caps[l] < cap ? level_caps[l] : cap, nullptr, 0, status} : kNoLimit;
    if (!inl) SGNN_LAUNCH(k_scan_block_sums, dim3(1), dim3(1024), 0, s, block_sums, nblk, counts_dev + l, lim);
    SGNN_LAUNCH(k_chain_emit, dim3((unsigned)nblk), dim3(256), 0, s, fine, (const int32_t *)w.slot_of,
                (const int32_t *)w.owner, n_dev, n_host, (const int32_t *)block_sums, (int4 *)coarse_coords[l], w.rank_at,
                inl ? ScanInline{nblk, counts_dev + l, lim} : kNoInline);
    SGNN_LAUNCH(k_chain_parent, dim3(g), dim3(256), 0, s, n_dev, n_host, (const int32_t *)w.owner,
                (const int32_t *)w.rank_at, (const int32_t *)w.slot_of, (int32_t *)parent[l], (int32_t *)cvals[l]);
    fine = (const int4 *)coarse_coords[l];
    n_dev = counts_dev + l;
    n_host = cap;
  }
  return chain_hip_result(who, hipGetLastError());
}

SGNN_EXPORT int sgnn_rulebook_down2(const int32_t *fine_coords, int64_t nf, uint64_t *ckeys, int32_t *cvals,
                                    int64_t ccap, int32_t *parent, int32_t *coarse_coords,
                                    int64_t *n_coarse, void *ws, int64_t ws_bytes, sgnn_stream_t stream) {
  SGNN_CHECK_ARG(nf >= 0 && n_coarse && ckeys && cvals);
  SGNN_CHECK_ARG(ccap >= 2 * nf && ccap >= 2 && (ccap & (ccap - 1)) == 0 && ccap < (1ll << 31));
  SGNN_CHECK_ARG(nf == 0 || (fine_coords && parent && coarse_coords));
  void *const k = ckeys, *const v = cvals, *const p = parent, *const c = coarse_coords;
  return down2_chain("sgnn_rulebook_down2", fine_coords, nf, nullptr, nf, 1, &k, &v, ccap, &p, &c, n_coarse, nullptr,
                     nullptr, ws, ws_bytes, (hipStream_t)stream);
}

SGNN_EXPORT int sgnn_down2_chain(const int32_t *fine_coords, int64_t n0, const int64_t *n0_dev, int64_t cap, int depth,
                                 void *const *ckeys, void *const *cvals, int64_t ccap, void *const *parent,
                                 void *const *coarse_coords, int64_t *counts_dev, const int64_t *level_caps,
                                 int32_t *status, void *ws, int64_t ws_bytes, sgnn_stream_t stream) {
  SGNN_CHECK_ARG(!level_caps || status);
  SGNN_CHECK_ARG(depth >= 1 && depth <= CHAIN_MAX_DEPTH && cap >= 0 && n0 >= 0 && n0 <= cap && counts_dev && ckeys &&
                 cvals && parent && coarse_coords);
  SGNN_CHECK_ARG(ccap >= 2 * cap && ccap >= 2 && (ccap & (ccap - 1)) == 0 && ccap < (1ll << 31));
  for (int l = 0; l < depth; ++l) SGNN_CHECK_ARG(ckeys[l] && (cap == 0 || (cvals[l] && parent[l] && coarse_coords[l])));
  SGNN_CHECK_ARG(cap == 0 || fine_coords);
  return down2_chain("sgnn_down2_chain", fine_coords, n0, n0_dev, cap, depth, ckeys, cvals, ccap, parent, coarse_coords,
                     counts_dev, level_caps, status, ws, ws_bytes, (hipStream_t)stream);
}

SGNN_EXPORT int sgnn_down2_chain_tables(const int32_t *fine_coords, const int64_t *n0_dev, int64_t cap, int depth,
                                        void *const *ckeys, void *const *cvals, int64_t ccap, void *const *parent,
                                        void *const *coarse_coords, int64_t *counts_dev, const int64_t *level_caps,
                                        void *const *children, void *const *ptable, int32_t *status, void *ws,
                                        int64_t ws_bytes, sgnn_stream_t stream) {
  hipStream_t s = (hipStream_t)stream;
  SGNN_CHECK_ARG(depth >= 1 && depth <= CHAIN_MAX_DEPTH && cap >= 1 && n0_dev && counts_dev && level_caps && status &&
                 ckeys && cvals && parent && coarse_coords && children && ptable && fine_coords);
  SGNN_CHECK_ARG(ccap >= 2 * cap && ccap >= 2 && (ccap & (ccap - 1)) == 0 && ccap < (1ll << 31));
  if (!ws || ws_bytes < chain_ws_bytes(cap, ccap, depth)) {
    sgnn_set_error("sgnn_down2_chain_tables: workspace too small");
    return SGNN_ENOWS;
  }
  ChainScratch w[CHAIN_MAX_DEPTH];
  int32_t *block_sums = chain_ws_carve(ws, cap, ccap, depth, w);
  ChainInit ini{};
  for (int l = 0; l < depth; ++l) {
    SGNN_CHECK_ARG(ckeys[l] && cvals[l] && parent[l] && coarse_coords[l] && children[l] && ptable[l] && level_caps[l] >= 1);
    ini.ckeys[l] = (unsigned long long *)ckeys[l];
    ini.owner[l] = w[l].owner;
    ini.rank_at[l] = w[l].rank_at;
  }
  ini.ccap = ccap;
  ini.cap = cap;
  chain_launch_init(ini, depth, s);
  const int4 *fine = (const int4 *)fine_coords;
  const int64_t *n_dev = n0_dev;
  int64_t fine_cap = cap;
  const int g = sgnn_grid_for(cap, 256, 8192);
  const bool merged = g_tune.chain_merged != 0;
  for (int l = 0; l < depth; ++l) {
    const int64_t ccap_l = level_caps[l] < cap ? level_caps[l] : cap;
    const int64_t ldc = ((ccap_l + 255) / 256) * 256, ldf = ((fine_cap + 255) / 256) * 256;
    if (l == 0 || !merged)
      chain_launch_insert(fine, n_dev, cap, cap, ckeys[l], w[l], ccap, s);
    const ScanInline si = chain_launch_count(w[l], n_dev, cap, cap, block_sums, counts_dev + l,
                                             ScanLimit{ccap_l, nullptr, 0, status}, s);
    SGNN_LAUNCH(k_chain_emit2, dim3((unsigned)((cap + SCAN_BLOCK - 1) / SCAN_BLOCK)), dim3(256), 0, s, fine,
                (const int32_t *)w[l].slot_of, (const int32_t *)w[l].owner, n_dev, cap, (const int32_t *)block_sums,
                (int4 *)coarse_coords[l], w[l].rank_at, (const int64_t *)(counts_dev + l), (int32_t *)children[l], ldc, si);
    const ChainTables t{fine, n_dev, cap, w[l].owner, w[l].rank_at, w[l].slot_of, (int32_t *)parent[l], (int32_t *)cvals[l],
                        counts_dev + l, ccap_l, (int32_t *)children[l], ldc, (int32_t *)ptable[l], ldf};
    if (merged && l + 1 < depth)
      SGNN_LAUNCH(k_chain_tables_insert, dim3(g), dim3(256), 0, s, t, (unsigned long long *)ckeys[l + 1], w[l + 1].owner,
                  (uint64_t)(ccap - 1), w[l + 1].slot_of, (const int4 *)coarse_coords[l], cap);
    else
      SGNN_LAUNCH(k_chain_parent_tables, dim3(g), dim3(256), 0, s, t);
    fine = (const int4 *)coarse_coords[l];
    n_dev = counts_dev + l;
    fine_cap = ccap_l;
  }
  SGNN_CHECK_LAUNCH();
  return SGNN_OK;
}

__global__ __launch_bounds__(256) void k_down2_tables(const int4 *__restrict__ fine,
                                                     const int32_t *__restrict__ parent, int64_t nf,
                                                     int32_t *__restrict__ children, int64_t ldc,
                                                     int32_t *__restrict__ ptable, int64_t ldf, int64_t nc,
                                                     const int64_t *nf_dev, const int64_t *nc_dev) {
  nf = sgnn_dyn_n(nf, nf_dev);
  nc = sgnn_dyn_n(nc, nc_dev);
  int64_t i = (int64_t)blockIdx.x * 256 + threadIdx.x;
  const int64_t stride = (int64_t)gridDim.x * 256;
  const int64_t iend = pad_end(nf, ldf);
  for (; i < iend; i += stride) {
    if (i >= nf)
      down2_table_row<false>(i, true, fine, -1, nc, nullptr, children, ldc, ptable, ldf);
    else
      down2_table_row<false>(i, false, fine, parent[i], nc, nullptr, children, ldc, ptable, ldf);
  }
}

SGNN_EXPORT int sgnn_down2_tables(const int32_t *fine_coords, const int32_t *parent, int64_t nf,
                                  int32_t *children, int64_t ldc, int64_t nc, int32_t *ptable, int64_t ldf,
                                  const int64_t *nf_dev, const int64_t *nc_dev, sgnn_stream_t stream) {
  hipStream_t s = (hipStream_t)stream;
  SGNN_CHECK_ARG(nf >= 0 && nc >= 0 && ldc >= nc && ldf >= nf);
  if (nc > 0) {
    SGNN_CHECK_ARG(children);
    if (nc_dev)
      SGNN_LAUNCH(k_fill_rows_dyn, dim3(sgnn_grid_for(8 * nc, 256, 4096)), dim3(256), 0, s, children, 8, ldc, nc, nc_dev);
    else
      if (sgnn_fill32(children, 0xFFFFFFFFu, 8 * ldc, s) != SGNN_OK) return SGNN_EHIP;
  }
  if (nf == 0) return SGNN_OK;
  SGNN_CHECK_ARG(fine_coords && parent && ptable && children);
  SGNN_LAUNCH(k_down2_tables, dim3(sgnn_grid_for(ldf, 256, 8192)), dim3(256), 0, s,
                     (const int4 *)fine_coords, parent, nf, children, ldc, ptable, ldf, nc, nf_dev, nc_dev);
  SGNN_CHECK_LAUNCH();
  return SGNN_OK;
}

__global__ __launch_bounds__(256) void k_expand8(const int4 *__restrict__ coords, int64_t n,
                                                int4 *__restrict__ out, const int64_t *n_dev) {
  n = sgnn_dyn_n(n, n_dev);
  int64_t t = (int64_t)blockIdx.x * 256 + threadIdx.x;
  const int64_t stride = (int64_t)gridDim.x * 256;
  for (; t < 8 * n; t += stride) {
    const int4 c = coords[t >> 3];
    const int j = (int)(t & 7);
    out[t] = make_int4(2 * c.x + (j >> 2), 2 * c.y + ((j >> 1) & 1), 2 * c.z + (j & 1), c.w);
  }
}

SGNN_EXPORT int sgnn_expand8_coords(const int32_t *coords, int64_t n, int32_t *out, const int64_t *n_dev,
                                    sgnn_stream_t stream) {
  SGNN_CHECK_ARG(n >= 0);
  if (n == 0) return SGNN_OK;
  SGNN_CHECK_ARG(coords && out);
  SGNN_LAUNCH(k_expand8, dim3(sgnn_grid_for(8 * n, 256, 8192)), dim3(256), 0, (hipStream_t)stream,
                     (const int4 *)coords, n, (int4 *)out, n_dev);
  SGNN_CHECK_LAUNCH();
  return SGNN_OK;
}

__global__ __launch_bounds__(256) void k_expand8_i64(const int4 *__restrict__ coords, int64_t n, int4 *__restrict__ out,
                                                    int64_t *__restrict__ locs, const int64_t *n_dev) {
  n = sgnn_dyn_n(n, n_dev);
  int64_t t = (int64_t)blockIdx.x * 256 + threadIdx.x;
  const int64_t stride = (int64_t)gridDim.x * 256;
  for (; t < 8 * n; t += stride) {
    const int4 c = coords[t >> 3];
    const int j = (int)(t & 7);
    const int4 o = make_int4(2 * c.x + (j >> 2), 2 * c.y + ((j >> 1) & 1), 2 * c.z + (j & 1), c.w);
    out[t] = o;
    reinterpret_cast<longlong2 *>(locs)[2 * t] = make_longlong2(o.x, o.y);
    reinterpret_cast<longlong2 *>(locs)[2 * t + 1] = make_longlong2(o.z, o.w);
  }
}

SGNN_EXPORT int sgnn_expand8_coords_i64(const int32_t *coords, int64_t n, int32_t *out, int64_t *locs, const int64_t *n_dev,
                                        sgnn_stream_t stream) {
  SGNN_CHECK_ARG(n >= 0);
  if (n == 0) return SGNN_OK;
  SGNN_CHECK_ARG(coords && out && locs);
  SGNN_LAUNCH(k_expand8_i64, dim3(sgnn_grid_for(8 * n, 256, 8192)), dim3(256), 0, (hipStream_t)stream,
                     (const int4 *)coords, n, (int4 *)out, locs, n_dev);
  SGNN_CHECK_LAUNCH();
  return SGNN_OK;
}

__global__ __launch_bounds__(256) void k_dense_coords(int batch, int d0, int d1, int d2,
                                                     int4 *__restrict__ out) {
// ... 25 lines not shown
```

sgnn_amd/csrc/prog.hip:

```cpp
#include <mutex>
#include <vector>
#include "common.h"

enum {
  OP_CONV_SUBM = 0, OP_CONV_DOWN = 1, OP_UNPOOL = 2, OP_BN = 3, OP_ADD = 4, OP_JOIN = 5,
  OP_CONCAT_IN = 6,
  OP_EXPAND = 7,
  OP_LINEAR = 8
};
#define OPW 12
#define EXPAND_DX_SPLIT 4

extern "C" int sgnn_expand_weights(const float *w, int cin, int cout, float *wc, sgnn_stream_t stream);
extern "C" int sgnn_expand_weights_bwd(const float *dwc, int cin, int cout, float *dw, sgnn_stream_t stream);
int64_t sgnn_bf16_wfrag_bytes(int cin, int cout, int K, int groups);
int sgnn_bf16_conv_prepare(const float *w, int cin, int cout, int K, int groups, void *wf, sgnn_stream_t stream);
int sgnn_bf16_conv_run(const void *x, int64_t n_in, int cin, int64_t ldx, const float *w, const void *wf, int K,
                       const int32_t *table, int64_t ld, int64_t n_out, int cout, void *y, int64_t ldy,
                       const void *addend, int64_t ld_add, const int32_t *kmap, int groups, int table_rows,
                       const int64_t *n_dev, sgnn_stream_t stream);
int sgnn_bf16_conv_expand_impl(const void *x, int64_t n, int cin, int64_t ldx, const float *w, const int32_t *nbr,
                               int64_t ld, int cout, void *y, int64_t ldy, const int64_t *n_dev, void *ws,
                               sgnn_stream_t stream);
int sgnn_bf16_linear_rows(const void *x, int64_t ldx, int64_t n, int cin, const float *const *w, const float *const *b,
                          int cout, float *y, const int64_t *n_dev, sgnn_stream_t stream);

namespace {

struct Op {
  int32_t type, in0, in1, out, par, lev, cin, cout, in2, ia, ib, ic;
  bool is_conv() const { return type == OP_CONV_SUBM || type == OP_CONV_DOWN; }
  int K() const { return type == OP_CONV_DOWN ? 8 : 27; }
  int out_class() const { return type == OP_CONV_DOWN ? lev + 1 : lev; }
  template <class F>
  void for_inputs(F f) const {
    f(in0);
    if (type == OP_ADD || type == OP_JOIN || type == OP_CONCAT_IN) f(in1);
    if (type == OP_CONCAT_IN) f(in2);
  }
};
static_assert(sizeof(Op) == sizeof(int32_t[OPW]), "Op mirrors one record of the caller's int32 array");

struct View {
  const int32_t *ops;
  const float *opf;
  int nops;
  const int32_t *bufs;
  int nbuf, n_ext;
  const int64_t *lev_n, *lev_ld;
  void *const *lev_nbr, *const *lev_children, *const *lev_ptable, *const *lev_parent;
  int nlev;
  const Op &op(int i) const { return reinterpret_cast<const Op *>(ops)[i]; }
};

enum Kind { TRAINING, INFERENCE, INFERENCE_BF16 };

Kind kind_of_mode(int mode) { return mode == 3 ? INFERENCE_BF16 : mode == 2 ? INFERENCE : TRAINING; }

inline int64_t round64(int64_t v) { return (v + 63) & ~int64_t(63); }

struct ConvSetup {
  bool ok = false;
  int K = 0, cnt_class = 0;
  int64_t n = 0, n_out = 0;
  const int32_t *tab_f = nullptr, *tab_b = nullptr;
  int64_t ld_f = 0, ld_b = 0;
  int flags_b = 0;
  ConvSetup(const View &v, const Op &o) {
    const bool down = o.type == OP_CONV_DOWN;
    K = o.K();
    cnt_class = o.out_class();
    ok = o.lev >= 0 && cnt_class < v.nlev;
    if (!ok) return;
    n = v.lev_n[o.lev];
    n_out = v.lev_n[cnt_class];
    if (!v.lev_ld) return;
    tab_f = (const int32_t *)(down ? v.lev_children[o.lev] : v.lev_nbr[o.lev]);
    ld_f = v.lev_ld[cnt_class];
    tab_b = (const int32_t *)(down ? v.lev_ptable[o.lev] : v.lev_nbr[o.lev]);
    ld_b = v.lev_ld[o.lev];
    flags_b = down ? SGNN_CONV_TRANSPOSE_W : (SGNN_CONV_TRANSPOSE_W | SGNN_CONV_FLIP_K);
  }
};

std::vector<int> count_readers(const View &v) {
  std::vector<int> r(v.nbuf, 0);
  for (int i = 0; i < v.nops; ++i)
    v.op(i).for_inputs([&](int b) {
      if (b >= 0 && b < v.nbuf) ++r[b];
    });
  return r;
}

#define g_fuse (g_tune.prog_fusion != 0)
#define g_lin_add (g_tune.prog_lin_add != 0)
#define g_lin_bn (g_tune.prog_lin_bn != 0)
struct Plan {
  std::vector<int> add_dst;
  std::vector<int> add_src;
  std::vector<char> skip;
  std::vector<int> root, col;
  std::vector<int64_t> ld;
  std::vector<char> join_view;
  std::vector<int> lin_bn;
  Kind kind = TRAINING;
  std::vector<char> f32;
  bool bf16() const { return kind == INFERENCE_BF16; }
};

inline int64_t round8(int64_t v) { return (v + 7) & ~int64_t(7); }

bool strided_conv_ok(const Op &o) {
  return sgnn_conv_epi_supported(o.cin, o.cout) && sgnn_conv_epi_supported(o.cout, o.cin) && dw_shape_ok(o.cin, o.cout);
}

void make_plan(const View &v, const int32_t *keep, Plan &P, Kind kind) {
  P.kind = kind;
  P.f32.assign(v.nbuf, P.bf16() ? 0 : 1);
  if (P.bf16())
    for (int i = 0; i < v.nops; ++i)
      if (v.op(i).type == OP_LINEAR && v.op(i).out >= 0 && v.op(i).out < v.nbuf) P.f32[v.op(i).out] = 1;
  auto row_ld = [&](int r) -> int64_t { return P.f32[r] ? v.bufs[2 * r + 1] : round8(v.bufs[2 * r + 1]); };
  P.add_dst.assign(v.nops, -1);
  P.add_src.assign(v.nops, -1);
  P.skip.assign(v.nops, 0);
  P.join_view.assign(v.nops, 0);
  P.lin_bn.assign(v.nops, -1);
  P.root.resize(v.nbuf);
  P.col.assign(v.nbuf, 0);
  P.ld.resize(v.nbuf);
  for (int b = 0; b < v.nbuf; ++b) {
    P.root[b] = b;
// ... 721 lines not shown
  }
};

int bwd_unreached(const Ctx &c, const Grads &g, const Op &o) {
  const hipStream_t hs = (hipStream_t)c.stream;
  if (o.is_conv() || o.type == OP_EXPAND) PROG_TRY(sgnn_fill32(g.PG(o.par), 0u, (int64_t)o.K() * o.cin * o.cout, hs));
  if (o.type == OP_BN) {
    void *zp[2] = {g.PG(o.par), g.PG(o.par + 1)};
    const int64_t zw[2] = {o.cin, o.cin};
    PROG_TRY(sgnn_fill32_multi(zp, zw, 2, 0u, hs));
  }
  if (o.type == OP_LINEAR)
    for (int q = 0; q < o.cout; ++q) {
      void *zp[2] = {g.PG(o.par + 2 * q), g.PG(o.par + 2 * q + 1)};
      const int64_t zw[2] = {o.cin, 1};
      PROG_TRY(sgnn_fill32_multi(zp, zw, 2, 0u, hs));
    }
  return SGNN_OK;
}

int bwd_conv(Ctx &c, Grads &g, Lane &lane, int i) {
  const Op &o = c.v.op(i);
  const ConvSetup cs(c.v, o);
  SGNN_CHECK_ARG(cs.ok);
  const int in0 = o.in0, cin = o.cin, cout = o.cout;
  const float *dy = g.read(o.out);
  const int64_t ld_dy = g.read_ld(o.out);
  const hipStream_t ls = lane.fork();
  if (g.wants(in0)) {
    if (g_fuse && sgnn_conv_epi_supported(cout, cin) && cs.n > 0) {
      ConvEpi epi{};
      if (g.has(in0)) {
        epi.addend = g.read(in0);
        epi.ld_add = g.read_ld(in0);
      }
      if (i > 0 && c.v.op(i - 1).type == OP_BN && c.v.op(i - 1).out == in0 && c.v.op(i - 1).cin == cin) {
        const Op &bo = c.v.op(i - 1);
        const float *save = g.arena + c.L.aux_off[i - 1];
        epi.stats = 2;
        epi.partial = c.stats_ws;
        epi.bn_x = g.X(bo.in0);
        epi.ld_bnx = c.ld(bo.in0);
        epi.mean = save;
        epi.invstd = save + cin;
        epi.gamma = c.param(bo.par);
        epi.beta = c.param(bo.par + 1);
        epi.leak = c.v.opf[4 * (i - 1) + 2];
        c.pre[i - 1] = c.stats_ws;
        c.pre_nblk[i - 1] = sgnn_conv_grid_blocks(cs.n, cout, cin, cs.K);
      }
      epi.ldx = ld_dy;
      epi.ldy = c.ld(in0);
      epi.n_dev = c.count(o.lev);
      PROG_TRY(sgnn_conv_fwd_impl(dy, cs.n_out, cout, c.param(o.par), cs.K, cs.tab_b, cs.ld_b, cs.n, cin, g.G(in0), cs.flags_b, 0,
                                  nullptr, nullptr, 1, 1, cs.K, &epi, c.stream));
      g.written(in0);
    } else {
      SGNN_CHECK_ARG(ld_dy == cout);
      float *t = g.target(in0, 0);
      ConvEpi pepi{};
      pepi.n_dev = c.count(o.lev);
      PROG_TRY(sgnn_conv_fwd_impl(dy, cs.n_out, cout, c.param(o.par), cs.K, cs.tab_b, cs.ld_b, cs.n, cin, t, cs.flags_b, 0, nullptr,
                                  nullptr, 1, 1, cs.K, &pepi, c.stream));
      PROG_TRY(g.commit(in0, t));
    }
  }
  const int64_t slice = dw_slice(c.v, i);
  PROG_TRY(sgnn_conv_bwd_weight_impl(g.X(in0), cs.n, cin, c.ld(in0), dy, cout, ld_dy, cs.tab_f, cs.ld_f, cs.K, cs.n_out,
                                     g.PG(o.par), 0, nullptr, nullptr, 1, 1, cs.K, lane.ws + lane.off, slice, (sgnn_stream_t)ls,
                                     c.count(cs.cnt_class)));
  if (ls != lane.hs) sgnn_stamp("dw>", (sgnn_stream_t)ls);
  lane.off += slice;
  return SGNN_OK;
}

int bwd_unpool(Ctx &c, Grads &g, Lane &, int i) {
  const Op &o = c.v.op(i);
  if (!g.wants(o.in0)) return SGNN_OK;
  float *t = g.target(o.in0, 0);
  PROG_TRY(sgnn_gather_sum_ld(g.read(o.out), g.read_ld(o.out), o.cin, (const int32_t *)c.v.lev_children[o.lev],
                              c.v.lev_ld[o.lev + 1], 8, c.v.lev_n[o.lev + 1], t, g.target_ld(o.in0, t), c.stream,
                              c.count(o.lev + 1)));
  return g.commit(o.in0, t);
}

int bwd_bn(Ctx &c, Grads &g, Lane &, int i) {
  const Op &o = c.v.op(i);
  const int in0 = o.in0, cin = o.cin;
  const float *save = g.arena + c.L.aux_off[i];
  const float *addend = nullptr;
  int64_t ld_add = cin;
  if (g.wants(in0) && g.has(in0)) {
    addend = g.read(in0);
    ld_add = g.read_ld(in0);
  }
  float *t = g.wants(in0) ? g.G(in0) : g.scratch[0];
  BnLin bl{};
  const bool lazy = g.lazy_lin[o.out] >= 0;
  if (lazy) {
    const Op &lo = c.v.op(g.lazy_lin[o.out]);
    bl.g = g.read(lo.out);
    bl.ldg = g.read_ld(lo.out);
    bl.nout = lo.cout;
    for (int q = 0; q < lo.cout; ++q) bl.w[q] = c.param(lo.par + 2 * q);
  }
  PROG_TRY(sgnn_bn_bwd_impl(g.X(in0), c.ld(in0), lazy ? nullptr : g.read(o.out), g.read_ld(o.out), c.v.lev_n[o.lev], cin,
                            c.param(o.par), c.param(o.par + 1), save, save + cin, c.training, c.v.opf[4 * i + 2], addend, ld_add,
                            t, g.wants(in0) ? c.ld(in0) : cin, g.PG(o.par), g.PG(o.par + 1), c.pre[i], c.pre_nblk[i], c.ws,
                            c.ws_bytes, c.stream, c.count(o.lev), lazy ? &bl : nullptr));
  if (g.wants(in0)) g.written(in0);
  return SGNN_OK;
}

int bwd_add(Ctx &c, Grads &g, Lane &, int i) {
  const Op &o = c.v.op(i);
  const int64_t n = c.v.lev_n[o.lev];
// ... 69 lines not shown
  float *part = g.garena + c.L.bextra + round64(64 * (int64_t)cin * cout);
  const hipStream_t ls = lane.fork();
  SGNN_CHECK_ARG(g.read_ld(o.out) == cout && c.ld(in0) == cin);
  if (g.wants(in0) && n > 0) {
    const int Gs = EXPAND_DX_SPLIT;
    ConvEpi xepi{};
    xepi.n_dev = c.count(o.lev);
    PROG_TRY(sgnn_conv_fwd_impl(dy, 8 * n, cout, wc, 64 / Gs, nbr, ld_nbr, n, cin, part, SGNN_CONV_TRANSPOSE_W, 0, ST, PAR, 8,
                                Gs, 27, &xepi, c.stream));
    float *t = g.target(in0, 0);
    PROG_TRY(sgnn_sum_groups_dn(part, cin, n, Gs, t, c.stream, c.count(o.lev)));
    PROG_TRY(g.commit(in0, t));
  }
  PROG_TRY(sgnn_conv_bwd_weight_impl(g.X(in0), n, cin, cin, dy, cout, cout, nbr, ld_nbr, 8, n, dwc, 0, S, nullptr, 1, 8, 27,
                                     lane.ws + lane.off, slice, (sgnn_stream_t)ls, c.count(o.lev)));
  lane.off += slice;
  lane.pending_expand.push_back(Lane::PendingExpand{dwc, cin, cout, g.PG(o.par)});
  return SGNN_OK;
}

int bwd_linear(Ctx &c, Grads &g, Lane &, int i) {
  const Op &o = c.v.op(i);
  const int in0 = o.in0, cin = o.cin, cout = o.cout;
  const int64_t n = c.v.lev_n[o.lev];
  const float *dy = g.read(o.out);
  const float *w[4] = {};
  float *dw[4] = {}, *db[4] = {};
  for (int q = 0; q < cout; ++q) {
    w[q] = c.param(o.par + 2 * q);
    dw[q] = g.PG(o.par + 2 * q);
    db[q] = g.PG(o.par + 2 * q + 1);
  }
  SGNN_CHECK_ARG(g.read_ld(o.out) == cout && c.ld(in0) == cin);
  if (c.P.lin_bn[i] >= 0 && g.wants(in0) && !g.has(in0) && n > 0 && !c.pre[c.P.lin_bn[i]]) {
    PROG_TRY(sgnn_linear_bwd_rows(g.X(in0), dy, n, cin, w, cout, nullptr, dw, db, c.ws, c.ws_bytes, c.stream, c.count(o.lev)));
    g.lazy_lin[in0] = i;
    return SGNN_OK;
  }
  const float *have = (g_fuse && g_lin_add && g.wants(in0) && g.has(in0) && n > 0) ? g.read(in0) : nullptr;
  const int64_t have_ld = have ? g.read_ld(in0) : 0;
  if (have && have_ld % 4 == 0 && ((uintptr_t)have & 15) == 0 && !g.viewed[in0]) {
    PROG_TRY(sgnn_linear_bwd_rows(g.X(in0), dy, n, cin, w, cout, g.G(in0), dw, db, c.ws, c.ws_bytes, c.stream, c.count(o.lev),
                                  have, have_ld));
    g.written(in0);
    return SGNN_OK;
  }
  float *t = g.wants(in0) ? g.target(in0, 0) : nullptr;
  PROG_TRY(sgnn_linear_bwd_rows(g.X(in0), dy, n, cin, w, cout, t, dw, db, c.ws, c.ws_bytes, c.stream, c.count(o.lev)));
  return t ? g.commit(in0, t) : SGNN_OK;
}

}

SGNN_EXPORT int sgnn_prog_backward(const int32_t *ops, const float *opf, int nops, const int32_t *bufs, int nbuf, int n_ext,
                                   const int64_t *lev_n, const int64_t *lev_ld, void *const *lev_nbr,
                                   void *const *lev_children, void *const *lev_ptable, void *const *lev_parent,
                                   void *const *lev_cnt, int nlev, void *const *params,
                                   void *const *pgrads, int nparams,
                                   void *const *ext, void *const *gext, void *const *idx, int nidx,
                                   const float *arena, float *garena, int64_t arena_floats, void *const *gout,
                                   const int32_t *keep, int training, void *ws, int64_t ws_bytes,
                                   sgnn_stream_t stream) {
  SGNN_CHECK_ARG(ops && opf && bufs && lev_n && lev_ld && params && pgrads && arena && garena && gout &&
                 n_ext >= 0 && n_ext <= nbuf && (n_ext == 0 || (ext && gext)));
  Ctx c{View{ops, opf, nops, bufs, nbuf, n_ext, lev_n, lev_ld, lev_nbr, lev_children, lev_ptable, lev_parent, nlev},
        params, idx, lev_cnt, nparams, nidx, training, ws, ws_bytes, stream};
  SGNN_CHECK_ARG(c.prepare(TRAINING, keep));
  if (arena_floats < c.L.total || ws_bytes < ws_need(c.v)) {
    sgnn_set_error("sgnn_prog_backward: arena or workspace too small");
    return SGNN_ENOWS;
  }
  Grads g(c, pgrads, ext, gext, gout, arena, garena);
  PROG_TRY(g.adopt_outputs());
  Lane lane(c, (hipStream_t)stream);
  for (int i = nops - 1; i >= 0; --i) {
    const Op &o = c.v.op(i);
    if (!g.has(o.out) && !(o.type == OP_BN && g.lazy_lin[o.out] >= 0)) {
      PROG_TRY(bwd_unreached(c, g, o));
      continue;
    }
    switch (o.type) {
      case OP_CONV_SUBM:
      case OP_CONV_DOWN: PROG_TRY(bwd_conv(c, g, lane, i)); break;
      case OP_UNPOOL: PROG_TRY(bwd_unpool(c, g, lane, i)); break;
      case OP_BN: PROG_TRY(bwd_bn(c, g, lane, i)); break;
      case OP_ADD: PROG_TRY(bwd_add(c, g, lane, i)); break;
      case OP_JOIN: PROG_TRY(bwd_join(c, g, lane, i)); break;
      case OP_CONCAT_IN: PROG_TRY(bwd_concat_in(c, g, lane, i)); break;
      case OP_EXPAND: PROG_TRY(bwd_expand(c, g, lane, i)); break;
      case OP_LINEAR: PROG_TRY(bwd_linear(c, g, lane, i)); break;
      default:
        sgnn_set_error("sgnn_prog_backward: unknown op %d", o.type);
        return SGNN_EINVAL;
    }
  }
  PROG_TRY(g.finish_externals());
  return lane.finish();
}
```

sgnn_amd/scn/metadata.py:

```python
import numpy as np
import os
import threading
from contextlib import nullcontext as _nullcontext

import torch

from .. import _lib
from .._lib import ptr
from .sites import info, attach, carry


SIDE_LANE = os.environ.get('SGNN_SIDE_LANE', '1') != '0'
SIDE_PRIORITY = int(os.environ.get('SGNN_SIDE_PRIORITY', '0'))
SIDE_PYRAMID = os.environ.get('SGNN_SIDE_PYRAMID', '1') != '0'
PYRAMID_LANE = 2


class _Runtime(object):

    def __init__(self, device):
        self.device = device
        self.ws = torch.empty(1 << 20, dtype=torch.uint8, device=device)
        self.state = torch.zeros(8, dtype=torch.int64, device=device)
        self.status32 = self.state[1:2].view(torch.int32)
# ... 135 lines not shown
        if self.keys is None:
            rt = runtime(self.device)
            self.cap = _lib.query('sgnn_hash_capacity', self.n)
            self.keys = torch.empty(self.cap, dtype=torch.int64, device=self.device)
            self.vals = torch.empty(self.cap, dtype=torch.int32, device=self.device)
            _lib.call('sgnn_hash_build', ptr(self.coords), self.n, ptr(self.keys), ptr(self.vals), self.cap,
                      ptr(rt.status32), ptr(self.cnt))
        return self.keys, self.vals, self.cap

    def lookup(self, query32, m_cnt=None):
        keys, vals, cap = self.hash()
        m = int(query32.shape[0])
        rows = torch.empty(m, dtype=torch.int32, device=self.device)
        _lib.call('sgnn_hash_lookup', ptr(keys), ptr(vals), cap, ptr(query32), m, ptr(rows), ptr(m_cnt))
        return rows

    def subm_table(self):
        if self._nbr is None:
            d, vb = self.dims, self.bounds
            dense = (d is not None and len(d) == 3 and self.n >= DENSE_RULEBOOK_MIN_ROWS
                     and 0 < d[0] * d[1] * d[2] <= INDEX_VOLUME_ENTRIES and max(d) <= 65536)
            if (dense and VOLUME_ONLY and vb is not None and self.keys is None and all(int(vb[1 + a]) <= int(d[a]) for a in range(3))
                    and int(vb[0]) * d[0] * d[1] * d[2] <= INDEX_VOLUME_ENTRIES):
                rt = runtime(self.device)
                self._nbr = torch.empty(27 * self.ld, dtype=torch.int32, device=self.device)
                vol = rt.index_volume()
                _lib.call('sgnn_rulebook_subm3_volume', ptr(self.coords), self.n, int(d[0]), int(d[1]), int(d[2]), ptr(vol),
                          vol.numel(), ptr(self._nbr), self.ld, ptr(self.cnt), ptr(rt.status32))
                return self._nbr
            keys, vals, cap = self.hash()
            self._nbr = torch.empty(27 * self.ld, dtype=torch.int32, device=self.device)
            if dense:
                vol = runtime(self.device).index_volume()
                _lib.call('sgnn_rulebook_subm3_dense', ptr(keys), ptr(vals), cap, ptr(self.coords), self.n, int(d[0]),
                          int(d[1]), int(d[2]), ptr(vol), vol.numel(), ptr(self._nbr), self.ld, ptr(self.cnt))
            else:
                _lib.call('sgnn_rulebook_subm3', ptr(keys), ptr(vals), cap, ptr(self.coords), self.n, ptr(self._nbr),
                          self.ld, ptr(self.cnt))
        return self._nbr

    def locations_i64(self):
        return rows_i64(self.coords, self.n, self.cnt)


def rows_i64(coords32, n, cnt):
    out = torch.empty(n, 4, dtype=torch.int64, device=coords32.device)
    _lib.call('sgnn_coords_to_i64', ptr(coords32), n, ptr(out), ptr(cnt))
    return out if cnt is None else attach(out, cnt=cnt)


class Down2(object):
    ready = None

    def __init__(self, fine, coarse, parent, children, ldc, ptable, ldf):
        self.fine, self.coarse = fine, coarse
        self.parent, self.children, self.ldc, self.ptable, self.ldf = parent, children, ldc, ptable, ldf


def build_down2(fine):
    rt = runtime(fine.device)
    nf, dev = fine.n, fine.device
    ccap = _lib.query('sgnn_hash_capacity', nf)
    ckeys = torch.empty(ccap, dtype=torch.int64, device=dev)
    cvals = torch.empty(ccap, dtype=torch.int32, device=dev)
    parent = torch.empty(max(nf, 1), dtype=torch.int32, device=dev)
    ccoords = torch.empty(max(nf, 1), 4, dtype=torch.int32, device=dev)
    wsb = _lib.query('sgnn_down2_ws_bytes', nf)
    ws = rt.workspace(wsb)
    _lib.call('sgnn_rulebook_down2', ptr(fine.coords), nf, ptr(ckeys), ptr(cvals), ccap, ptr(parent), ptr(ccoords),
              ptr(rt.state), ptr(ws), wsb)
    nc = rt.read_count()
    return _down2_tables(fine, Grid(ccoords[:nc], ckeys, cvals, ccap), parent)


CHAIN = True
MAX_CHAIN = 6


class PendingChain(object):

    def __init__(self, coords_cap, n0, n0_on_device, depth, n0_cnt=None, counts=None, level_caps=None):
        dev = coords_cap.device
        rt = runtime(dev)
        cap = int(coords_cap.shape[0])
        depth = min(depth, MAX_CHAIN)
        self.n0_cnt, self.counts, self.level_caps = n0_cnt, counts, level_caps
        self.coords_cap, self.cap, self.depth = coords_cap, cap, depth
        self.ccap = _lib.query('sgnn_hash_capacity', cap)
        mk = lambda shape, dt: torch.empty(shape, dtype=dt, device=dev)
        self.ckeys = [mk(self.ccap, torch.int64) for _ in range(depth)]
        self.cvals = [mk(self.ccap, torch.int32) for _ in range(depth)]
        self.parent = [mk(max(cap, 1), torch.int32) for _ in range(depth)]
        self.ccoords = [mk((max(cap, 1), 4), torch.int32) for _ in range(depth)]
        wsb = _lib.query('sgnn_down2_chain_ws_bytes', cap)
        ws = rt.workspace(wsb)
        arr = lambda ts: np.ascontiguousarray(np.array([t.data_ptr() for t in ts], dtype=np.uint64))
        self._keep = [arr(self.ckeys), arr(self.cvals), arr(self.parent), arr(self.ccoords)]
        if counts is not None:
            assert n0_cnt is not None and level_caps is not None and len(level_caps) >= depth and counts.numel() >= depth
            caps = [min(int(c), cap) for c in level_caps[:depth]]
            caps_np = np.ascontiguousarray(np.array(caps, dtype=np.int64))
            ld = [_round_up(max(cap, 1), 256)] + [_round_up(max(c, 1), 256) for c in caps]
            self.children = [mk(8 * ld[l + 1], torch.int32) for l in range(depth)]
            self.ptable = [mk(8 * ld[l], torch.int32) for l in range(depth)]
            self._keep += [arr(self.children), arr(self.ptable)]
            wsb = _lib.query('sgnn_down2_chain_tables_ws_bytes', cap, depth)
            self.side = None
            if SIDE_PYRAMID:
                self.side = rt.pyramid_stream()
                with lane(PYRAMID_LANE):
                    rt2 = runtime(dev)
                    if rt2.ws.numel() < wsb:
                        self.side.synchronize()
                    ws = rt2.workspace(wsb)
                _lib.stamp('fork')
                self.side.wait_stream(torch.cuda.current_stream(dev))
            else:
                ws = rt.workspace(wsb)
            with (torch.cuda.stream(self.side) if self.side is not None else _nullcontext()):
                _lib.stamp('lane<')
                _lib.call('sgnn_down2_chain_tables', ptr(coords_cap), ptr(n0_cnt), cap, depth,
                          self._keep[0].ctypes.data, self._keep[1].ctypes.data, self.ccap, self._keep[2].ctypes.data,
                          self._keep[3].ctypes.data, ptr(counts), caps_np.ctypes.data, self._keep[4].ctypes.data,
                          self._keep[5].ctypes.data, ptr(rt.status32), ptr(ws), wsb)
            return
        _lib.call('sgnn_down2_chain', ptr(coords_cap), 0 if n0_on_device else int(n0),
                  rt.state.data_ptr() if n0_on_device else None, cap, depth, self._keep[0].ctypes.data,
                  self._keep[1].ctypes.data, self.ccap, self._keep[2].ctypes.data, self._keep[3].ctypes.data,
                  rt.state.data_ptr() + 16, None, None, ptr(ws), wsb)

    def finalize(self, n0, host_state):
        counts = [int(v) for v in host_state[2:2 + self.depth]]
        fine = Grid(self.coords_cap[:n0])
        fine.bounds = info(self.coords_cap).bounds
        grid0, downs = fine, []
        for l in range(self.depth):
            nc = counts[l]
            coarse = Grid(self.ccoords[l][:nc], self.ckeys[l], self.cvals[l], self.ccap)
            downs.append(_down2_tables(fine, coarse, self.parent[l]))
            fine = coarse
        return grid0, downs

    def finalize_capped(self, grid0=None):
        fine = grid0 if grid0 is not None else Grid(self.coords_cap, cnt=self.n0_cnt)
        grid0, downs = fine, []
        for l in range(self.depth):
            cap_l = min(int(self.level_caps[l]), self.cap)
            coarse = Grid(self.ccoords[l][:cap_l], self.ckeys[l], self.cvals[l], self.ccap, cnt=self.counts[l:l + 1])
            assert coarse.ld * 8 == self.children[l].numel() and fine.ld * 8 == self.ptable[l].numel()
            downs.append(Down2(fine, coarse, self.parent[l][:fine.n], self.children[l], coarse.ld, self.ptable[l], fine.ld))
            fine = coarse
        if getattr(self, 'side', None) is not None:
            for d in downs:
                g = d.coarse
                g._nbr = torch.empty(27 * g.ld, dtype=torch.int32, device=g.device)
            with torch.cuda.stream(self.side):
                for i in range(0, len(downs), _lib.RULEBOOK_MULTI_MAX):
                    gs = [d.coarse for d in downs[i:i + _lib.RULEBOOK_MULTI_MAX]]
                    arr = [np.array(v, dtype=np.int64) for v in (
                        [ptr(g.keys) for g in gs], [ptr(g.vals) for g in gs], [g.cap for g in gs],
                        [ptr(g.coords) for g in gs], [g.n for g in gs], [ptr(g._nbr) for g in gs], [g.ld for g in gs],
                        [ptr(g.cnt) for g in gs])]
                    _lib.call('sgnn_rulebook_subm3_multi', len(gs), *[a.ctypes.data for a in arr])
                _lib.stamp('lane>')
                ev = torch.cuda.Event()
                ev.record(self.side)
            for d in downs:
                d.ready = d.coarse.ready = ev
        return grid0, downs


def _down2_tables(fine, coarse, parent):
    dev = fine.device
    nf, nc = fine.n, coarse.n
    ldc, ldf = coarse.ld, fine.ld
    children = torch.empty(8 * ldc, dtype=torch.int32, device=dev)
    ptable = torch.empty(8 * ldf, dtype=torch.int32, device=dev)
    _lib.call('sgnn_down2_tables', ptr(fine.coords), ptr(parent), nf, ptr(children), ldc, nc, ptr(ptable), ldf,
              ptr(fine.cnt), ptr(coarse.cnt))
    return Down2(fine, coarse, parent[:nf], children, ldc, ptable, ldf)


class Metadata(object):
    def __init__(self, dimension=3):
        self.dimension = dimension
        self.grids = {}
        self.down = {}

    @staticmethod
    def key(spatial_size):
        return spatial_size if isinstance(spatial_size, tuple) else tuple(int(s) for s in spatial_size)

    def _register(self, key, grid):
        self.grids[key] = grid
        if grid.dims is None:
            grid.dims = key

    def set_input(self, spatial_size, grid):
        self._register(self.key(spatial_size), grid)

    def adopt(self, spatial_size, grid0, downs):
        key = self.key(spatial_size)
        self._register(key, grid0)
        for d in downs:
            nxt = tuple(v // 2 for v in key)
            self.down[(key, nxt)] = d
            self._register(nxt, d.coarse)
            key = nxt

    def prebuild(self, spatial_size, depth, capacity=None):
        key = self.key(spatial_size)
        k, todo = key, 0
        for _ in range(depth):
            if any(v % 2 for v in k):
                break
            nxt = tuple(v // 2 for v in k)
            if (k, nxt) not in self.down:
                todo += 1
            k = nxt
        g0 = self.grids[key]
        if capacity is not None:
            if g0.cnt is None or len(self.down) or todo != depth:
                raise _lib.SgnnError('capacity mode: the level-0 grid needs a device row count and an unbuilt pyramid')
            caps, counts = capacity
            chain = PendingChain(g0.coords, g0.n, True, depth, n0_cnt=g0.cnt, counts=counts, level_caps=caps)
            _, downs = chain.finalize_capped(g0)
            self.adopt(key, g0, downs)
            return
        if not CHAIN or todo < 2 or g0.n == 0 or len(self.down):
            return
        chain = PendingChain(g0.coords, g0.n, False, todo)
        host = runtime(g0.device).read_counts()
        if COUNT_LOG is not None:
# ... 49 lines not shown
```

sgnn_amd/scn/program.py:

```python
import contextlib

import numpy as np
import torch
from torch.autograd import Function

from .. import _lib
from . import modules as M
from .metadata import runtime

OP_SUBM, OP_DOWN, OP_UNPOOL, OP_BN, OP_ADD, OP_JOIN, OP_CONCAT_IN, OP_EXPAND, OP_LINEAR = range(9)
OPW = 12
ENABLED = True
PERSISTENT_ARENAS = False
_garenas = {}
DEFER_JOIN = False
_deferred = []
_iarenas = {}
_bf16_depth = 0


@contextlib.contextmanager
def bf16_inference():
    global _bf16_depth
    _bf16_depth += 1
# ... 223 lines not shown
            return (b, lev, ch)
        raise Unsupported('module %s' % type(m).__name__)


def _ptr_array(values):
    return np.ascontiguousarray(np.array(values, dtype=np.uint64))


class _Run(object):
    pass


def _levels(prog, md, key, grid0):
    grids, downs = [grid0], []
    for _ in range(prog.nlev - 1):
        if any(v % 2 for v in key):
            raise ValueError('Convolution(2,2): spatial size %s is not even' % list(key))
        nxt = tuple(v // 2 for v in key)
        d = md.down2(key, nxt)
        downs.append(d)
        grids.append(d.coarse)
        key = nxt
    return grids, downs


class _ProgramFn(Function):
    @staticmethod
    def forward(ctx, run, *tensors):
        prog = run.prog
        n_ext = prog.n_ext
        ext = [t.contiguous() for t in tensors[:n_ext]]
        params = tensors[n_ext:]
        dev = ext[0].device
        rt = runtime(dev)
        lev_n = np.zeros(prog.n_classes, dtype=np.int64)
        lev_ld = np.zeros(prog.n_classes, dtype=np.int64)
        for l, g in enumerate(run.grids):
            lev_n[l], lev_ld[l] = g.n, g.ld
        for name, cid in prog.class_ids.items():
            lev_n[cid] = run.extra_rows[name]
        nbr = [0] * prog.n_classes
        cnts = [0] * prog.n_classes
        for l, g in enumerate(run.grids):
            if g.cnt is not None:
                cnts[l] = g.cnt.data_ptr()
        for name, cid in prog.class_ids.items():
            c = run.extra_cnt.get(name)
            if c is not None:
                cnts[cid] = c.data_ptr()
        for l in prog.subm_levels:
            nbr[l] = run.grids[l].subm_table().data_ptr()
        pad = [0] * (prog.n_classes - len(run.downs))
        children = [d.children.data_ptr() for d in run.downs] + pad
        ptable = [d.ptable.data_ptr() for d in run.downs] + pad
        parent = [d.parent.data_ptr() if d.parent.numel() else 0 for d in run.downs] + pad
        run.lev_n, run.lev_ld = lev_n, lev_ld
        prog.last_lev_n = lev_n.copy()
        run.tabs = [_ptr_array(v) for v in (nbr, children, ptable, parent, cnts)]
        run.pptr = _ptr_array([0 if p is None else p.data_ptr() for p in params])
        run.eptr = _ptr_array([t.data_ptr() for t in ext])
        run.iptr = _ptr_array([t.data_ptr() for t in run.idx] + [0])
        ops, opf, bufs = prog.ops_np, prog.opf_np, prog.bufs_np
        nops, nbuf, ncls = ops.shape[0], bufs.shape[0], prog.n_classes
        keep = np.zeros(nbuf, dtype=np.int32)
        keep[run.out_bufs] = 1
        run.keep = keep
        qa = (ops.ctypes.data, nops, bufs.ctypes.data, nbuf, n_ext, lev_n.ctypes.data, ncls, keep.ctypes.data)
        infer = bool(run.infer)
        bf16 = bool(run.bf16)
        total = _lib.query('sgnn_prog_arena_floats', *qa, 0)
        fwd_total = _lib.query('sgnn_prog_arena_floats', *qa, 3 if bf16 else (2 if infer else 1))
        wsb = _lib.query('sgnn_prog_ws_bytes', ops.ctypes.data, nops, lev_n.ctypes.data, ncls)
        run.total, run.wsb = total, wsb
        prog.last_arena_floats = (fwd_total, total)
        if infer:
            arena = _arena(_iarenas, str(dev), fwd_total, dev, 1.1)
        elif PERSISTENT_ARENAS:
            arena = _arena(prog.__dict__.setdefault('_arenas', {}), 'fwd', fwd_total, dev)
        else:
            arena = torch.empty(fwd_total, dtype=torch.float32, device=dev)
        ws = rt.workspace(wsb)
        ready = next((d.ready for d in run.downs if d.ready is not None), None)
        wait = ready.cuda_event if ready is not None else None
        _lib.stamp('prog<')
        _lib.call('sgnn_prog_forward', ops.ctypes.data, opf.ctypes.data, nops, bufs.ctypes.data, nbuf, n_ext,
                  lev_n.ctypes.data, lev_ld.ctypes.data, run.tabs[0].ctypes.data, run.tabs[1].ctypes.data,
                  run.tabs[2].ctypes.data, run.tabs[3].ctypes.data, run.tabs[4].ctypes.data, ncls,
                  run.pptr.ctypes.data, len(params),
                  run.eptr.ctypes.data, run.iptr.ctypes.data, len(run.idx), arena.data_ptr(), fwd_total,
                  keep.ctypes.data, int(run.training) | (2 if infer else 0) | (4 if bf16 else 0), wait, ws.data_ptr(), wsb)
        _lib.stamp('prog>')
        run.offsets = {}
        outs = []
        for b in run.out_bufs:
            off = _lib.query('sgnn_prog_buffer_offset', *qa, 2 if bf16 else int(infer), b)
            assert off >= 0
            rows, ch = int(lev_n[bufs[b, 0]]), int(bufs[b, 1])
            run.offsets[b] = (off, rows, ch)
            if bf16 and b not in prog.linear_outs:
                o = torch.empty(rows, ch, dtype=torch.float32, device=dev)
                _lib.call('sgnn_bf16_to_f32', arena.data_ptr() + 4 * off, (ch + 7) // 8 * 8, rows, ch, o.data_ptr(), None)
                outs.append(o)
                continue
            o = arena[off:off + rows * ch].view(rows, ch)
            outs.append(o.clone() if infer else o)
        if infer:
            ctx.run = None
            return tuple(outs)
        ctx.run = run
        ctx.save_for_backward(arena, *ext, *[p for p in params if p is not None])
        ctx.param_none = [p is None for p in params]
# ... 6 lines not shown
        n_ext = prog.n_ext
        saved = ctx.saved_tensors
        arena, ext = saved[0], saved[1:1 + n_ext]
        it = iter(saved[1 + n_ext:])
        params = [None if none else next(it) for none in ctx.param_none]
        dev = arena.device
        rt = runtime(dev)
        ops, opf, bufs = prog.ops_np, prog.opf_np, prog.bufs_np
        nops, nbuf, ncls = ops.shape[0], bufs.shape[0], prog.n_classes
        if PERSISTENT_ARENAS and DEFER_JOIN:
            garena = _arena(prog.__dict__.setdefault('_arenas', {}), 'bwd', run.total, dev)
        elif PERSISTENT_ARENAS:
            garena = _arena(_garenas, str(dev), run.total, dev)
        else:
            garena = torch.empty(run.total, dtype=torch.float32, device=dev)
        gout = [0] * nbuf
        held = []
        for b, g in zip(run.out_bufs, gouts):
            if g is None:
                continue
            g = g.contiguous()
            held.append(g)
            gout[b] = g.data_ptr()
        gout = _ptr_array(gout)
        live = prog.tensors()
        direct = [getattr(lp, '_sgnn_flat_grad', None) if (t and p is not None) else None
                  for lp, p, t in zip(live, params, prog.grad_slot)]
        sizes = [p.numel() if (t and p is not None and d is None) else 0 for p, t, d in zip(params, prog.grad_slot, direct)]
        flat = torch.empty(max(sum(sizes), 1), dtype=torch.float32, device=dev)
        gptr, views, o = [], [], 0
        for p, s, d in zip(params, sizes, direct):
            if d is not None:
                gptr.append(d.data_ptr())
                views.append(None)
            elif s:
                v = flat[o:o + s].view_as(p)
                gptr.append(v.data_ptr())
                views.append(v)
                o += s
            else:
                gptr.append(0)
                views.append(None)
        gp = _ptr_array(gptr)
        gext = [torch.empty_like(t) if ctx.needs_input_grad[1 + i] else None for i, t in enumerate(ext)]
        geptr = _ptr_array([0 if t is None else t.data_ptr() for t in gext])
        ws = rt.workspace(run.wsb)
        rt.side_lane(run.wsb)
        defer = bool(DEFER_JOIN and sum(sizes) == 0)
        prev_defer = _lib.query('sgnn_prog_defer_join', int(defer))
        if defer:
            _deferred.append((arena, garena, held, ext, params, run))
        try:
            _lib.stamp('bwd<')
            _lib.call('sgnn_prog_backward', ops.ctypes.data, opf.ctypes.data, nops, bufs.ctypes.data, nbuf, n_ext,
                      run.lev_n.ctypes.data, run.lev_ld.ctypes.data, run.tabs[0].ctypes.data, run.tabs[1].ctypes.data,
                      run.tabs[2].ctypes.data, run.tabs[3].ctypes.data, run.tabs[4].ctypes.data, ncls,
                      run.pptr.ctypes.data, gp.ctypes.data,
                      len(params), run.eptr.ctypes.data, geptr.ctypes.data, run.iptr.ctypes.data, len(run.idx),
                      arena.data_ptr(), garena.data_ptr(), run.total, gout.ctypes.data, run.keep.ctypes.data,
                      int(run.training), ws.data_ptr(), run.wsb)
        finally:
            _lib.query('sgnn_prog_defer_join', prev_defer)
        _lib.stamp('bwd>')
        return (None,) + tuple(gext) + tuple(views)


def compile_or_none(chain, in_channels, tap_modules=(), sources=None, tail=()):
    try:
        return Program(chain, in_channels, tap_modules, sources, tail)
    except Unsupported:
        return None


def run_program(prog, x, training, out_bufs=None, ext=None, idx=(), extra_rows=None, extra_cnt=None):
    run = _Run()
    run.prog, run.training = prog, training
    run.grids, run.downs = _levels(prog, x.metadata, x.key, x.grid())
    run.out_bufs = list(out_bufs) if out_bufs is not None else [prog.out]
    run.idx = list(idx)
    run.extra_rows = dict(extra_rows or {})
    run.extra_cnt = dict(extra_cnt or {})
    tensors = [x.features] if ext is None else list(ext)
    run.infer = not (torch.is_grad_enabled() and any(t is not None and t.requires_grad
                                                     for t in list(tensors) + list(prog.tensors())))
    run.bf16 = bf16_active()
    if run.bf16 and not run.infer:
        raise RuntimeError('bf16_inference: this program call may be asked for gradients (grad mode is on and an input '
                           'or parameter requires grad); bf16 storage exists for inference only — wrap the forward in '
                           'torch.no_grad() or leave the bf16_inference() context')
    if run.bf16 and training and prog.has_bn:
        raise RuntimeError('bf16_inference: BatchNorm in training mode (batch statistics) is not available with bf16 '
                           'storage; call model.eval() first')
    if 'child' in prog.class_ids and 'child' not in run.extra_rows:
        run.extra_rows['child'] = 8 * run.grids[0].n
    outs = _ProgramFn.apply(run, *tensors, *prog.tensors())
    return list(outs), run.grids, run.downs


def programs_of(model):
    out = []
    for m in model.modules():
        p = m.__dict__.get('_prog')
        if isinstance(p, Program):
            out.append(p)
        for p in (m.__dict__.get('_stage_progs') or {}).values():
            if isinstance(p, Program):
                out.append(p)
# ... 2 lines not shown
```

Before: 5717.

## Replace stride-2 ptable with packed parent codes for the transposed-conv input gradient

Each fine voxel now stores one packed int32 parent code (coarse index shifted left by 3, child slot in the low bits) in place of an 8-wide parent table. Stride-2 input-gradient convolutions read this single code and keep only the matching kernel tap, instead of loading eight table entries per row, which are mostly empty. The pyramid builder fills pcode and skips ptable in capacity mode, and the program backward uses a new pcode entry point. This cuts table memory and gather traffic, at the cost of extra template variants, a generic fallback kernel and an API where ptable can be absent.

```diff
diff --git a/include/sgnn_hip.h b/include/sgnn_hip.h
--- a/include/sgnn_hip.h
+++ b/include/sgnn_hip.h
@@ -83,6 +83,9 @@
 int sgnn_down2_tables(const int32_t *fine_coords, const int32_t *parent, int64_t nf,
                       int32_t *children, int64_t ldc, int64_t nc, int32_t *ptable, int64_t ldf,
                       const int64_t *nf_dev, const int64_t *nc_dev, sgnn_stream_t stream);
+int sgnn_down2_tables_pcode(const int32_t *fine_coords, const int32_t *parent, int64_t nf,
+                            int32_t *children, int64_t ldc, int64_t nc, int32_t *ptable, int32_t *pcode, int64_t ldf,
+                            const int64_t *nf_dev, const int64_t *nc_dev, sgnn_stream_t stream);
 
 int64_t sgnn_down2_chain_ws_bytes(int64_t cap);
 int sgnn_down2_chain(const int32_t *fine_coords, int64_t n0, const int64_t *n0_dev, int64_t cap, int depth,
@@ -96,6 +99,11 @@
                             void *const *coarse_coords, int64_t *counts_dev, const int64_t *level_caps,
                             void *const *children, void *const *ptable, int32_t *status, void *ws, int64_t ws_bytes,
                             sgnn_stream_t stream);
+int sgnn_down2_chain_tables_pcode(const int32_t *fine_coords, const int64_t *n0_dev, int64_t cap, int depth,
+                                  void *const *ckeys, void *const *cvals, int64_t ccap, void *const *parent,
+                                  void *const *coarse_coords, int64_t *counts_dev, const int64_t *level_caps,
+                                  void *const *children, void *const *ptable, void *const *pcode, int32_t *status,
+                                  void *ws, int64_t ws_bytes, sgnn_stream_t stream);
 
 #define SGNN_CONV_TRANSPOSE_W 1
 #define SGNN_CONV_FLIP_K 2
@@ -118,6 +126,12 @@
                       const float *addend, int64_t ld_add, int stats, double *partial, const float *bn_x,
                       int64_t ld_bnx, const float *mean, const float *invstd, const float *gamma, const float *beta,
                       float leak, sgnn_stream_t stream);
+
+int sgnn_conv_down2_dx(const float *dy, int64_t n_coarse, int cout, int64_t ld_dy, const float *w, const int32_t *pcode,
+                       int64_t ld, int64_t n_fine, int cin, float *dx, int64_t ld_dx, const float *addend,
+                       int64_t ld_add, int stats, double *partial, const float *bn_x, int64_t ld_bnx, const float *mean,
+                       const float *invstd, const float *gamma, const float *beta, float leak, const int64_t *n_dev,
+                       sgnn_stream_t stream);
 
 int64_t sgnn_conv_bwd_weight_ws_bytes(int64_t n_out, int K, int cin, int cout);
 int sgnn_conv_bwd_weight(const float *x, int64_t n_in, int cin, const float *dy, int cout,
@@ -239,6 +253,14 @@
 int sgnn_prog_backward(const int32_t *ops, const float *opf, int nops, const int32_t *bufs, int nbuf, int n_ext,
                        const int64_t *lev_n, const int64_t *lev_ld, void *const *lev_nbr,
                        void *const *lev_children, void *const *lev_ptable, void *const *lev_parent,
+                       void *const *lev_cnt, int nlev, void *const *params, void *const *pgrads,
+                       int nparams, void *const *ext,
+                       void *const *gext, void *const *idx, int nidx, const float *arena, float *garena,
+                       int64_t arena_floats, void *const *gout, const int32_t *keep, int training, void *ws,
+                       int64_t ws_bytes, sgnn_stream_t stream);
+int sgnn_prog_backward_pcode(const int32_t *ops, const float *opf, int nops, const int32_t *bufs, int nbuf, int n_ext,
+                       const int64_t *lev_n, const int64_t *lev_ld, void *const *lev_nbr,
+                       void *const *lev_children, void *const *lev_pcode, void *const *lev_parent,
                        void *const *lev_cnt, int nlev, void *const *params, void *const *pgrads,
                        int nparams, void *const *ext,
                        void *const *gext, void *const *idx, int nidx, const float *arena, float *garena,
diff --git a/sgnn_amd/_lib.py b/sgnn_amd/_lib.py
--- a/sgnn_amd/_lib.py
+++ b/sgnn_amd/_lib.py
@@ -33,11 +33,16 @@
     'sgnn_down2_chain_tables': (c_i32, [c_vp, c_vp, c_i64, c_i32, c_vp, c_vp, c_i64, c_vp, c_vp, c_vp, c_vp, c_vp, c_vp, c_vp, c_vp,
                                         c_i64, c_vp]),
     'sgnn_down2_tables': (c_i32, [c_vp, c_vp, c_i64, c_vp, c_i64, c_i64, c_vp, c_i64, c_vp, c_vp, c_vp]),
+    'sgnn_down2_chain_tables_pcode': (c_i32, [c_vp, c_vp, c_i64, c_i32, c_vp, c_vp, c_i64, c_vp, c_vp, c_vp, c_vp, c_vp, c_vp, c_vp,
+                                              c_vp, c_vp, c_i64, c_vp]),
+    'sgnn_down2_tables_pcode': (c_i32, [c_vp, c_vp, c_i64, c_vp, c_i64, c_i64, c_vp, c_vp, c_i64, c_vp, c_vp, c_vp]),
     'sgnn_conv_fwd': (c_i32, [c_vp, c_i64, c_i32, c_vp, c_i32, c_vp, c_i64, c_i64, c_i32, c_vp, c_i32, c_i32, c_vp]),
     'sgnn_conv_fwd_ex': (c_i32, [c_vp, c_i64, c_i32, c_vp, c_i32, c_vp, c_i64, c_i64, c_i32, c_vp, c_i32, c_i32, c_vp, c_vp, c_i32, c_i32, c_i32, c_vp]),
     'sgnn_conv_bwd_weight_ex': (c_i32, [c_vp, c_i64, c_i32, c_vp, c_i32, c_vp, c_i64, c_i32, c_i64, c_vp, c_i32, c_vp, c_vp, c_i32, c_i32, c_i32, c_vp, c_i64, c_vp]),
     'sgnn_conv_stats_blocks': (c_i64, [c_i64]),
     'sgnn_conv_fwd_epi': (c_i32, [c_vp, c_i64, c_i32, c_i64, c_vp, c_i32, c_vp, c_i64, c_i64, c_i32, c_vp, c_i64, c_i32, c_vp, c_i64, c_i32, c_vp, c_vp, c_i64, c_vp, c_vp, c_vp, c_vp, c_f32, c_vp]),
+    'sgnn_conv_down2_dx': (c_i32, [c_vp, c_i64, c_i32, c_i64, c_vp, c_vp, c_i64, c_i64, c_i32, c_vp, c_i64, c_vp, c_i64, c_i32, c_vp,
+                                   c_vp, c_i64, c_vp, c_vp, c_vp, c_vp, c_f32, c_vp, c_vp]),
     'sgnn_conv_bwd_weight_ws_bytes': (c_i64, [c_i64, c_i32, c_i32, c_i32]),
     'sgnn_conv_bwd_weight': (c_i32, [c_vp, c_i64, c_i32, c_vp, c_i32, c_vp, c_i64, c_i32, c_i64, c_vp, c_i32, c_vp, c_i64, c_vp]),
     'sgnn_bn_ws_bytes': (c_i64, [c_i64, c_i32]),
@@ -101,6 +106,8 @@
     'sgnn_prog_forward': (c_i32, [c_vp, c_vp, c_i32, c_vp, c_i32, c_i32, c_vp, c_vp, c_vp, c_vp, c_vp, c_vp, c_vp, c_i32, c_vp,
                                   c_i32, c_vp, c_vp, c_i32, c_vp, c_i64, c_vp, c_i32, c_vp, c_vp, c_i64, c_vp]),
     'sgnn_prog_backward': (c_i32, [c_vp, c_vp, c_i32, c_vp, c_i32, c_i32, c_vp, c_vp, c_vp, c_vp, c_vp, c_vp, c_vp, c_i32, c_vp,
+                                   c_vp, c_i32, c_vp, c_vp, c_vp, c_i32, c_vp, c_vp, c_i64, c_vp, c_vp, c_i32, c_vp, c_i64, c_vp]),
+    'sgnn_prog_backward_pcode': (c_i32, [c_vp, c_vp, c_i32, c_vp, c_i32, c_i32, c_vp, c_vp, c_vp, c_vp, c_vp, c_vp, c_vp, c_i32, c_vp,
                                    c_vp, c_i32, c_vp, c_vp, c_vp, c_i32, c_vp, c_vp, c_i64, c_vp, c_vp, c_i32, c_vp, c_i64, c_vp]),
     'sgnn_concat3_rows': (c_i32, [c_vp, c_i32, c_vp, c_vp, c_i32, c_vp, c_vp, c_i32, c_vp, c_i64, c_vp, c_vp]),
     'sgnn_concat3_rows_bwd': (c_i32, [c_vp, c_i32, c_vp, c_i32, c_vp, c_i32, c_vp, c_i64, c_vp, c_i64, c_vp, c_i64, c_vp,
diff --git a/sgnn_amd/csrc/common.h b/sgnn_amd/csrc/common.h
--- a/sgnn_amd/csrc/common.h
+++ b/sgnn_amd/csrc/common.h
@@ -35,6 +35,8 @@
                        int64_t n_out, int cout, float *y, int flags, int in_shift, const int32_t *kmap,
                        const int32_t *kadd, int in_mul, int groups, int table_rows, const ConvEpi *epi,
                        sgnn_stream_t stream);
+int sgnn_conv_down2_dx_impl(const float *x, int64_t n_in, int cin, const float *w, const int32_t *pcode, int64_t ld,
+                            int64_t n_out, int cout, float *y, const ConvEpi *epi, sgnn_stream_t stream);
 int64_t sgnn_conv_grid_blocks(int64_t n_out, int cin, int cout, int K);
 struct BnLin {
   const float *g;
diff --git a/sgnn_amd/csrc/conv.hip b/sgnn_amd/csrc/conv.hip
--- a/sgnn_amd/csrc/conv.hip
+++ b/sgnn_amd/csrc/conv.hip
@@ -216,7 +216,7 @@
   conv_fwd_body<CIN, COUT, CONV_MREP, false, true>(x, n_in, w, table, ld, K, n_out, y, flags, in_shift, ex, epi, wg_cap);
 }
 
-template <int CIN, int COUT>
+template <int CIN, int COUT, bool PC = false>
 __global__ __launch_bounds__(256) void k_conv_small(const float *__restrict__ x, int64_t n_in,
                                                    const float *__restrict__ w, const int32_t *__restrict__ table,
                                                    int64_t ld, int K, int64_t n_out, float *y, int flags, int in_shift,
@@ -244,16 +244,22 @@
 
   const uint32_t ldx4 = (uint32_t)epi.ldx * 4u, ldy4 = (uint32_t)epi.ldy * 4u;
   const __amdgpu_buffer_rsrc_t rs_x = make_rsrc(x, (uint32_t)(((n_in - 1) * epi.ldx + CIN) * 4));
-  const __amdgpu_buffer_rsrc_t rs_t = make_rsrc(table, (uint32_t)((int64_t)K * ld * 4));
+  const __amdgpu_buffer_rsrc_t rs_t = make_rsrc(table, (uint32_t)((int64_t)(PC ? 1 : K) * ld * 4));
   const __amdgpu_buffer_rsrc_t rs_y = make_rsrc(y, (uint32_t)(((n_out - 1) * epi.ldy + COUT) * 4));
   const uint32_t lane_off = (uint32_t)(row0 + r) * 4u;
   const uint32_t ld4 = (uint32_t)ld * 4u;
 
   int32_t id[KW];
-#pragma unroll
-  for (int kk = 0; kk < KW; ++kk) {
-    const int k = k0 + (kk < nk ? kk : (nk > 0 ? nk - 1 : 0));
-    id[kk] = (int32_t)__builtin_amdgcn_raw_buffer_load_b32(rs_t, lane_off, (k < K ? k : K - 1) * ld4, 0) >> in_shift;
+  if constexpr (PC) {
+    const int32_t code = (int32_t)__builtin_amdgcn_raw_buffer_load_b32(rs_t, lane_off, 0, 0);
+#pragma unroll
+    for (int kk = 0; kk < KW; ++kk) id[kk] = (kk < nk && code >= 0 && (code & 7) == k0 + kk) ? (code >> 3) : -1;
+  } else {
+#pragma unroll
+    for (int kk = 0; kk < KW; ++kk) {
+      const int k = k0 + (kk < nk ? kk : (nk > 0 ? nk - 1 : 0));
+      id[kk] = (int32_t)__builtin_amdgcn_raw_buffer_load_b32(rs_t, lane_off, (k < K ? k : K - 1) * ld4, 0) >> in_shift;
+    }
   }
   float a[KW][V];
 #pragma unroll
@@ -455,10 +461,6 @@
 #define CONV_EX_CASES(X) \
   X(48, 16) X(16, 48) X(24, 8) X(8, 24) X(16, 24) X(24, 16) X(24, 32) X(32, 24) X(64, 32) X(32, 64) X(56, 28) X(28, 56)
 
-#define CONV_FWD_CASES(X) \
-  X(1, 8) X(8, 8) X(8, 12) X(12, 12) X(12, 16) X(16, 16) X(34, 16) X(30, 16) X(26, 16) X(48, 16) \
-  X(8, 1) X(12, 8) X(16, 12) X(16, 34) X(16, 30) X(16, 26) X(16, 48) X(32, 16) X(16, 32) X(4, 16) X(16, 4) \
-  X(16, 24) X(24, 16) X(24, 32) X(32, 24) X(64, 32) X(32, 64) X(56, 28) X(28, 56) X(32, 32) X(28, 16) X(16, 28)
 
 int64_t sgnn_conv_grid_blocks(int64_t n_out, int cin, int cout, int K) {
   const int64_t grid4 = (n_out + CONV_ROWS_PER_BLOCK - 1) / CONV_ROWS_PER_BLOCK;
@@ -601,6 +603,86 @@
   ConvEpi epi{ldx, ldy, ld_add, addend, stats, partial, bn_x, ld_bnx, mean, invstd, gamma, beta, leak, nullptr};
   return sgnn_conv_fwd_impl(x, n_in, cin, w, K, table, ld, n_out, cout, y, flags, 0, nullptr, nullptr, 1, 1, K, &epi,
                             stream);
+}
+
+bool sgnn_conv_down2_dx_launch(const float *x, int64_t n_in, int cin, const float *w, const int32_t *pcode, int64_t ld,
+                               int64_t n_out, int cout, float *y, const ConvEpi &epi, hipStream_t s);
+
+__global__ __launch_bounds__(256) void k_conv_down2_dx_generic(const float *__restrict__ x, int cin, const float *__restrict__ w,
+                                                              const int32_t *__restrict__ pcode, int64_t n_out, int cout,
+                                                              float *__restrict__ y, const int64_t *n_dev) {
+  n_out = sgnn_dyn_n(n_out, n_dev);
+  const int64_t t = (int64_t)blockIdx.x * 256 + threadIdx.x;
+  if (t >= n_out * cout) return;
+  const int64_t row = t / cout;
+  const int n = (int)(t - row * cout);
+  const int32_t code = pcode[row];
+  float acc = 0.f;
+  if (code >= 0) {
+    const float *xr = x + (int64_t)(code >> 3) * cin;
+    const float *wk = w + ((int64_t)(code & 7) * cout + n) * cin;
+    for (int c = 0; c < cin; ++c) acc = fmaf(xr[c], wk[c], acc);
+  }
+  y[t] = acc;
+}
+
+int sgnn_conv_down2_dx_impl(const float *x, int64_t n_in, int cin, const float *w, const int32_t *pcode, int64_t ld,
+                            int64_t n_out, int cout, float *y, const ConvEpi *epi_in, sgnn_stream_t stream) {
+  SGNN_CHECK_ARG(cin >= 1 && cout >= 1 && n_out >= 0 && ld >= n_out && n_in < (1ll << 28));
+  if (n_out == 0) return SGNN_OK;
+  SGNN_CHECK_ARG(x && w && pcode && y && n_in >= 1);
+  SGNN_CHECK_ARG(ld % CONV_ROWS_PER_BLOCK == 0);
+  ConvEpi epi{};
+  if (epi_in) epi = *epi_in;
+  if (epi.ldx <= 0) epi.ldx = cin;
+  if (epi.ldy <= 0) epi.ldy = cout;
+  if (epi.ld_add <= 0) epi.ld_add = cout;
+  if (epi.ld_bnx <= 0) epi.ld_bnx = cout;
+  const bool has_epi = epi.ldx != cin || epi.ldy != cout || epi.addend || epi.stats;
+  SGNN_CHECK_ARG(epi.ldx >= cin && epi.ldx <= 1024 && epi.ldy >= cout && epi.ldy <= 1024 && epi.ld_add >= cout &&
+                 epi.ld_add <= 1024 && epi.ld_bnx >= cout && epi.ld_bnx <= 1024);
+  SGNN_CHECK_ARG(epi.stats >= 0 && epi.stats <= 2 && (!epi.stats || epi.partial));
+  SGNN_CHECK_ARG(epi.stats != 2 || (epi.bn_x && epi.mean && epi.invstd));
+  const int64_t lmax = epi.ldy > epi.ld_add ? (epi.ldy > epi.ld_bnx ? epi.ldy : epi.ld_bnx)
+                                            : (epi.ld_add > epi.ld_bnx ? epi.ld_add : epi.ld_bnx);
+  if (n_in * epi.ldx * 4 > 0xFFFFF000ll || n_out * lmax * 4 > 0xFFFFF000ll || ld * 4 > 0xFFFFF000ll) {
+    sgnn_set_error("sgnn_conv_down2_dx: a slab exceeds the 4 GiB raw-buffer window (n_in=%lld cin=%d n_out=%lld cout=%d)",
+                   (long long)n_in, cin, (long long)n_out, cout);
+    return SGNN_EOVERFLOW;
+  }
+  hipStream_t s = (hipStream_t)stream;
+  const bool small = (n_out + CONV_ROWS_PER_BLOCK - 1) / CONV_ROWS_PER_BLOCK < CONV_SMALL_GRID;
+  bool done = false;
+  const int prof = sgnn_prof_begin_launch(0, n_out, cin, cout, 8, SGNN_CONV_TRANSPOSE_W, s);
+  if (!small) done = sgnn_conv_down2_dx_launch(x, n_in, cin, w, pcode, ld, n_out, cout, y, epi, s);
+#define X(CI, CO)                                                                                               \
+  if (!done && cin == CI && cout == CO) {                                                                       \
+    SGNN_LAUNCH((k_conv_small<CI, CO, true>), dim3((unsigned)((n_out + 15) / 16)), dim3(256), 0, s, x, n_in, w, \
+                pcode, ld, 8, n_out, y, SGNN_CONV_TRANSPOSE_W, 0, epi);                                          \
+    done = true;                                                                                                \
+  }
+  CONV_FWD_CASES(X)
+#undef X
+  if (!done) {
+    if (has_epi) {
+      sgnn_set_error("sgnn_conv_down2_dx: strided / fused epilogues need one of the compiled (cin, cout) shapes, got (%d, %d)", cin, cout);
+      return SGNN_EINVAL;
+    }
+    SGNN_LAUNCH(k_conv_down2_dx_generic, dim3((unsigned)((n_out * cout + 255) / 256)), dim3(256), 0, s, x, cin, w, pcode,
+                n_out, cout, y, epi.n_dev);
+  }
+  sgnn_prof_end_launch(prof, s);
+  SGNN_CHECK_LAUNCH();
+  return SGNN_OK;
+}
+
+SGNN_EXPORT int sgnn_conv_down2_dx(const float *dy, int64_t n_coarse, int cout, int64_t ld_dy, const float *w,
+                                   const int32_t *pcode, int64_t ld, int64_t n_fine, int cin, float *dx, int64_t ld_dx,
+                                   const float *addend, int64_t ld_add, int stats, double *partial, const float *bn_x,
+                                   int64_t ld_bnx, const float *mean, const float *invstd, const float *gamma,
+                                   const float *beta, float leak, const int64_t *n_dev, sgnn_stream_t stream) {
+  ConvEpi epi{ld_dy, ld_dx, ld_add, addend, stats, partial, bn_x, ld_bnx, mean, invstd, gamma, beta, leak, n_dev};
+  return sgnn_conv_down2_dx_impl(dy, n_coarse, cout, w, pcode, ld, n_fine, cin, dx, &epi, stream);
 }
 
 __device__ int32_t g_expand_maps[192];
diff --git a/sgnn_amd/csrc/conv_common.h b/sgnn_amd/csrc/conv_common.h
--- a/sgnn_amd/csrc/conv_common.h
+++ b/sgnn_amd/csrc/conv_common.h
@@ -7,6 +7,11 @@
 #define CONV_MREP 4
 #define CONV_ROWS_PER_WAVE (16 * CONV_MREP)
 #define CONV_ROWS_PER_BLOCK (4 * CONV_ROWS_PER_WAVE)
+
+#define CONV_FWD_CASES(X) \
+  X(1, 8) X(8, 8) X(8, 12) X(12, 12) X(12, 16) X(16, 16) X(34, 16) X(30, 16) X(26, 16) X(48, 16) \
+  X(8, 1) X(12, 8) X(16, 12) X(16, 34) X(16, 30) X(16, 26) X(16, 48) X(32, 16) X(16, 32) X(4, 16) X(16, 4) \
+  X(16, 24) X(24, 16) X(24, 32) X(32, 24) X(64, 32) X(32, 64) X(56, 28) X(28, 56) X(32, 32) X(28, 16) X(16, 28)
 
 template <int CIN, int COUT>
 struct ConvCfg {
diff --git a/sgnn_amd/csrc/conv_unrolled.hip b/sgnn_amd/csrc/conv_unrolled.hip
--- a/sgnn_amd/csrc/conv_unrolled.hip
+++ b/sgnn_amd/csrc/conv_unrolled.hip
@@ -1,6 +1,6 @@
 #include "conv_common.h"
 
-template <int CIN, int COUT, int K, bool WEPI>
+template <int CIN, int COUT, int K, bool WEPI, bool PC = false>
 __device__ __forceinline__ void conv_fwd_u_body(const float *__restrict__ x, int64_t n_in, const float *__restrict__ w,
                                                 const int32_t *__restrict__ table, int64_t ld, int64_t n_out, float *y,
                                                 int flags, int in_shift, const ConvEpi &epi, int wg_cap) {
@@ -35,7 +35,9 @@
 
   const uint32_t ldx4 = (uint32_t)epi.ldx * 4u;
   const __amdgpu_buffer_rsrc_t rs_x = make_rsrc(x, (uint32_t)(((n_in - 1) * epi.ldx + CIN) * 4));
-  const __amdgpu_buffer_rsrc_t rs_t = make_rsrc(table, (uint32_t)((int64_t)K * ld * 4));
+  static_assert(!PC || K == 8, "parent codes carry a 3-bit offset");
+  constexpr int KT = PC ? 1 : K;
+  const __amdgpu_buffer_rsrc_t rs_t = make_rsrc(table, (uint32_t)((int64_t)KT * ld * 4));
   const uint32_t ld4 = (uint32_t)ld * 4u;
   int perm[M];
 #pragma unroll
@@ -89,8 +91,13 @@
   const int64_t row0 = wg_row0 + wave * 64;
   const uint32_t lane_off = (uint32_t)(row0 + lane) * 4u;
 #pragma unroll
-  for (int k = 0; k < K; ++k)
-    idx[k] = (int32_t)__builtin_amdgcn_raw_buffer_load_b32(rs_t, lane_off, k * ld4, 0) >> in_shift;
+  for (int k = 0; k < KT; ++k)
+    idx[k] = (int32_t)__builtin_amdgcn_raw_buffer_load_b32(rs_t, lane_off, k * ld4, 0) >> (PC ? 0 : in_shift);
+  if constexpr (PC) {
+    const int32_t code = idx[0];
+#pragma unroll
+    for (int k = 0; k < K; ++k) idx[k] = (code >= 0 && (code & 7) == k) ? (code >> 3) : -1;
+  }
 #pragma unroll
   for (int m = 0; m < M; ++m)
 #pragma unroll
@@ -133,6 +140,19 @@
     const float *__restrict__ x, int64_t n_in, const float *__restrict__ w, const int32_t *__restrict__ table, int64_t ld,
     int64_t n_out, float *y, int flags, int in_shift, ConvEpi epi, int wg_cap) {
   conv_fwd_u_body<CIN, COUT, 8, true>(x, n_in, w, table, ld, n_out, y, flags, in_shift, epi, wg_cap);
+}
+
+template <int CIN, int COUT>
+__global__ __launch_bounds__(256) void k_conv_down2_dx(const float *__restrict__ x, int64_t n_in, const float *__restrict__ w,
+                                                      const int32_t *__restrict__ pcode, int64_t ld, int64_t n_out, float *y,
+                                                      ConvEpi epi, int wg_cap) {
+  conv_fwd_u_body<CIN, COUT, 8, false, true>(x, n_in, w, pcode, ld, n_out, y, SGNN_CONV_TRANSPOSE_W, 0, epi, wg_cap);
+}
+template <int CIN, int COUT>
+__global__ __launch_bounds__(256) __attribute__((amdgpu_waves_per_eu(4, 8))) void k_conv_down2_dx_w(
+    const float *__restrict__ x, int64_t n_in, const float *__restrict__ w, const int32_t *__restrict__ pcode, int64_t ld,
+    int64_t n_out, float *y, ConvEpi epi, int wg_cap) {
+  conv_fwd_u_body<CIN, COUT, 8, true, true>(x, n_in, w, pcode, ld, n_out, y, SGNN_CONV_TRANSPOSE_W, 0, epi, wg_cap);
 }
 
 #define CONV_U_CASES_27(X) X(34, 16) X(16, 34) X(30, 16) X(16, 30) X(26, 16) X(16, 26)
@@ -185,3 +205,30 @@
 #undef X
   return false;
 }
+
+template <int CI, int CO>
+static void conv_down2_dx_launch(unsigned grid, hipStream_t s, const float *x, int64_t n_in, const float *w, const int32_t *pcode,
+                                 int64_t ld, int64_t n_out, float *y, const ConvEpi &epi) {
+  if constexpr (CO % 4 == 0 && CO <= 16) {
+    if (conv_wide_epi_ok(epi, y, 8)) {
+      SGNN_LAUNCH((k_conv_down2_dx_w<CI, CO>), dim3(grid), dim3(256), 0, s, x, n_in, w, pcode, ld, n_out, y, epi,
+                  g_tune.conv_one_round ? conv_wg_capacity<k_conv_down2_dx_w<CI, CO>>() : 0);
+      return;
+    }
+  }
+  SGNN_LAUNCH((k_conv_down2_dx<CI, CO>), dim3(grid), dim3(256), 0, s, x, n_in, w, pcode, ld, n_out, y, epi,
+              g_tune.conv_one_round ? conv_wg_capacity<k_conv_down2_dx<CI, CO>>() : 0);
+}
+
+bool sgnn_conv_down2_dx_launch(const float *x, int64_t n_in, int cin, const float *w, const int32_t *pcode, int64_t ld,
+                               int64_t n_out, int cout, float *y, const ConvEpi &epi, hipStream_t s) {
+  const unsigned grid = (unsigned)((n_out + 255) / 256);
+#define X(CI, CO)                                                                       \
+  if (cin == CI && cout == CO) {                                                        \
+    conv_down2_dx_launch<CI, CO>(grid, s, x, n_in, w, pcode, ld, n_out, y, epi);        \
+    return true;                                                                        \
+  }
+  CONV_FWD_CASES(X)
+#undef X
+  return false;
+}
diff --git a/sgnn_amd/csrc/grid_rules.hip b/sgnn_amd/csrc/grid_rules.hip
--- a/sgnn_amd/csrc/grid_rules.hip
+++ b/sgnn_amd/csrc/grid_rules.hip
@@ -865,7 +865,7 @@
 template <bool Record>
 __device__ __forceinline__ void down2_table_row(int64_t i, bool pad, const int4 *__restrict__ fine, int32_t p, int64_t nc,
                                                 int32_t *__restrict__ parent, int32_t *__restrict__ children, int64_t ldc,
-                                                int32_t *__restrict__ ptable, int64_t ldf) {
+                                                int32_t *__restrict__ ptable, int64_t ldf, int32_t *__restrict__ pcode) {
   int off = -1;
   if (!pad) {
     if (p >= nc) p = -1;
@@ -874,8 +874,11 @@
     off = ((c.x & 1) << 2) | ((c.y & 1) << 1) | (c.z & 1);
     if (p >= 0) children[(int64_t)off * ldc + p] = (int32_t)i;
   }
-#pragma unroll
-  for (int k = 0; k < 8; ++k) ptable[(int64_t)k * ldf + i] = (k == off) ? p : -1;
+  if (ptable) {
+#pragma unroll
+    for (int k = 0; k < 8; ++k) ptable[(int64_t)k * ldf + i] = (k == off) ? p : -1;
+  }
+  if (pcode) pcode[i] = p >= 0 ? (p << 3) | off : -1;
 }
 
 struct ChainTables {
@@ -890,6 +893,7 @@
   int64_t ldc;
   int32_t *ptable;
   int64_t ldf;
+  int32_t *pcode;
 };
 
 template <bool Tables>
@@ -900,7 +904,8 @@
                                                   int32_t *__restrict__ parent, int32_t *__restrict__ cvals,
                                                   const int64_t *nc_dev, int64_t nc_cap,
                                                   int32_t *__restrict__ children, int64_t ldc,
-                                                  int32_t *__restrict__ ptable, int64_t ldf) {
+                                                  int32_t *__restrict__ ptable, int64_t ldf,
+                                                  int32_t *__restrict__ pcode) {
   const int64_t nf = sgnn_dyn_n(n_host, n_dev);
   const int64_t nc = Tables ? sgnn_dyn_n(nc_cap, nc_dev) : 0;
   const int64_t iend = Tables ? pad_end(nf, ldf) : nf;
@@ -908,13 +913,13 @@
   const int64_t stride = (int64_t)gridDim.x * 256;
   for (; i < iend; i += stride) {
     if (Tables && i >= nf) {
-      down2_table_row<false>(i, true, fine, -1, nc, nullptr, children, ldc, ptable, ldf);
+      down2_table_row<false>(i, true, fine, -1, nc, nullptr, children, ldc, ptable, ldf, pcode);
       continue;
     }
     const int32_t sl = slot_of[i];
     const int32_t p = rank_at[owner[sl]];
     if (rank_at[i] >= 0) cvals[sl] = p;
-    if (Tables) down2_table_row<true>(i, false, fine, p, nc, parent, children, ldc, ptable, ldf);
+    if (Tables) down2_table_row<true>(i, false, fine, p, nc, parent, children, ldc, ptable, ldf, pcode);
     else parent[i] = p;
   }
 }
@@ -924,12 +929,12 @@
                                                      const int32_t *__restrict__ rank_at,
                                                      const int32_t *__restrict__ slot_of,
                                                      int32_t *__restrict__ parent, int32_t *__restrict__ cvals) {
-  chain_parent_rows<false>(nullptr, n_dev, n_host, owner, rank_at, slot_of, parent, cvals, nullptr, 0, nullptr, 0, nullptr, 0);
+  chain_parent_rows<false>(nullptr, n_dev, n_host, owner, rank_at, slot_of, parent, cvals, nullptr, 0, nullptr, 0, nullptr, 0, nullptr);
 }
 
 __global__ __launch_bounds__(256) void k_chain_parent_tables(ChainTables t) {
   chain_parent_rows<true>(t.fine, t.n_dev, t.n_host, t.owner, t.rank_at, t.slot_of, t.parent, t.cvals, t.nc_dev, t.nc_cap,
-                          t.children, t.ldc, t.ptable, t.ldf);
+                          t.children, t.ldc, t.ptable, t.ldf, t.pcode);
 }
 
 __global__ __launch_bounds__(256) void k_chain_tables_insert(ChainTables t, unsigned long long *__restrict__ ckeys_next,
@@ -937,7 +942,7 @@
                                                             int32_t *__restrict__ slot_of_next, const int4 *coarse,
                                                             int64_t n_host_next) {
   chain_parent_rows<true>(t.fine, t.n_dev, t.n_host, t.owner, t.rank_at, t.slot_of, t.parent, t.cvals, t.nc_dev, t.nc_cap,
-                          t.children, t.ldc, t.ptable, t.ldf);
+                          t.children, t.ldc, t.ptable, t.ldf, t.pcode);
   chain_insert_rows(coarse, t.nc_dev, n_host_next, ckeys_next, owner_next, mask, slot_of_next);
 }
 
@@ -1039,14 +1044,15 @@
                      counts_dev, level_caps, status, ws, ws_bytes, (hipStream_t)stream);
 }
 
-SGNN_EXPORT int sgnn_down2_chain_tables(const int32_t *fine_coords, const int64_t *n0_dev, int64_t cap, int depth,
-                                        void *const *ckeys, void *const *cvals, int64_t ccap, void *const *parent,
-                                        void *const *coarse_coords, int64_t *counts_dev, const int64_t *level_caps,
-                                        void *const *children, void *const *ptable, int32_t *status, void *ws,
-                                        int64_t ws_bytes, sgnn_stream_t stream) {
+SGNN_EXPORT int sgnn_down2_chain_tables_pcode(const int32_t *fine_coords, const int64_t *n0_dev, int64_t cap, int depth,
+                                              void *const *ckeys, void *const *cvals, int64_t ccap, void *const *parent,
+                                              void *const *coarse_coords, int64_t *counts_dev, const int64_t *level_caps,
+                                              void *const *children, void *const *ptable, void *const *pcode,
+                                              int32_t *status, void *ws, int64_t ws_bytes, sgnn_stream_t stream) {
   hipStream_t s = (hipStream_t)stream;
   SGNN_CHECK_ARG(depth >= 1 && depth <= CHAIN_MAX_DEPTH && cap >= 1 && n0_dev && counts_dev && level_caps && status &&
-                 ckeys && cvals && parent && coarse_coords && children && ptable && fine_coords);
+                 ckeys && cvals && parent && coarse_coords && children && fine_coords);
+  SGNN_CHECK_ARG(!pcode || cap < (1ll << 28));
   SGNN_CHECK_ARG(ccap >= 2 * cap && ccap >= 2 && (ccap & (ccap - 1)) == 0 && ccap < (1ll << 31));
   if (!ws || ws_bytes < chain_ws_bytes(cap, ccap, depth)) {
     sgnn_set_error("sgnn_down2_chain_tables: workspace too small");
@@ -1056,7 +1062,7 @@
   int32_t *block_sums = chain_ws_carve(ws, cap, ccap, depth, w);
   ChainInit ini{};
   for (int l = 0; l < depth; ++l) {
-    SGNN_CHECK_ARG(ckeys[l] && cvals[l] && parent[l] && coarse_coords[l] && children[l] && ptable[l] && level_caps[l] >= 1);
+    SGNN_CHECK_ARG(ckeys[l] && cvals[l] && parent[l] && coarse_coords[l] && children[l] && level_caps[l] >= 1);
     ini.ckeys[l] = (unsigned long long *)ckeys[l];
     ini.owner[l] = w[l].owner;
     ini.rank_at[l] = w[l].rank_at;
@@ -1080,7 +1086,8 @@
                 (const int32_t *)w[l].slot_of, (const int32_t *)w[l].owner, n_dev, cap, (const int32_t *)block_sums,
                 (int4 *)coarse_coords[l], w[l].rank_at, (const int64_t *)(counts_dev + l), (int32_t *)children[l], ldc, si);
     const ChainTables t{fine, n_dev, cap, w[l].owner, w[l].rank_at, w[l].slot_of, (int32_t *)parent[l], (int32_t *)cvals[l],
-                        counts_dev + l, ccap_l, (int32_t *)children[l], ldc, (int32_t *)ptable[l], ldf};
+                        counts_dev + l, ccap_l, (int32_t *)children[l], ldc, (int32_t *)(ptable ? ptable[l] : nullptr), ldf,
+                        (int32_t *)(pcode ? pcode[l] : nullptr)};
     if (merged && l + 1 < depth)
       SGNN_LAUNCH(k_chain_tables_insert, dim3(g), dim3(256), 0, s, t, (unsigned long long *)ckeys[l + 1], w[l + 1].owner,
                   (uint64_t)(ccap - 1), w[l + 1].slot_of, (const int4 *)coarse_coords[l], cap);
@@ -1094,11 +1101,21 @@
   return SGNN_OK;
 }
 
+SGNN_EXPORT int sgnn_down2_chain_tables(const int32_t *fine_coords, const int64_t *n0_dev, int64_t cap, int depth,
+                                        void *const *ckeys, void *const *cvals, int64_t ccap, void *const *parent,
+                                        void *const *coarse_coords, int64_t *counts_dev, const int64_t *level_caps,
+                                        void *const *children, void *const *ptable, int32_t *status, void *ws,
+                                        int64_t ws_bytes, sgnn_stream_t stream) {
+  return sgnn_down2_chain_tables_pcode(fine_coords, n0_dev, cap, depth, ckeys, cvals, ccap, parent, coarse_coords, counts_dev,
+                                       level_caps, children, ptable, nullptr, status, ws, ws_bytes, stream);
+}
+
 __global__ __launch_bounds__(256) void k_down2_tables(const int4 *__restrict__ fine,
                                                      const int32_t *__restrict__ parent, int64_t nf,
                                                      int32_t *__restrict__ children, int64_t ldc,
                                                      int32_t *__restrict__ ptable, int64_t ldf, int64_t nc,
-                                                     const int64_t *nf_dev, const int64_t *nc_dev) {
+                                                     const int64_t *nf_dev, const int64_t *nc_dev,
+                                                     int32_t *__restrict__ pcode) {
   nf = sgnn_dyn_n(nf, nf_dev);
   nc = sgnn_dyn_n(nc, nc_dev);
   int64_t i = (int64_t)blockIdx.x * 256 + threadIdx.x;
@@ -1106,17 +1123,18 @@
   const int64_t iend = pad_end(nf, ldf);
   for (; i < iend; i += stride) {
     if (i >= nf)
-      down2_table_row<false>(i, true, fine, -1, nc, nullptr, children, ldc, ptable, ldf);
+      down2_table_row<false>(i, true, fine, -1, nc, nullptr, children, ldc, ptable, ldf, pcode);
     else
-      down2_table_row<false>(i, false, fine, parent[i], nc, nullptr, children, ldc, ptable, ldf);
-  }
-}
-
-SGNN_EXPORT int sgnn_down2_tables(const int32_t *fine_coords, const int32_t *parent, int64_t nf,
-                                  int32_t *children, int64_t ldc, int64_t nc, int32_t *ptable, int64_t ldf,
-                                  const int64_t *nf_dev, const int64_t *nc_dev, sgnn_stream_t stream) {
+      down2_table_row<false>(i, false, fine, parent[i], nc, nullptr, children, ldc, ptable, ldf, pcode);
+  }
+}
+
+SGNN_EXPORT int sgnn_down2_tables_pcode(const int32_t *fine_coords, const int32_t *parent, int64_t nf,
+                                        int32_t *children, int64_t ldc, int64_t nc, int32_t *ptable, int32_t *pcode,
+                                        int64_t ldf, const int64_t *nf_dev, const int64_t *nc_dev, sgnn_stream_t stream) {
   hipStream_t s = (hipStream_t)stream;
   SGNN_CHECK_ARG(nf >= 0 && nc >= 0 && ldc >= nc && ldf >= nf);
+  SGNN_CHECK_ARG(!pcode || nc < (1ll << 28));
   if (nc > 0) {
     SGNN_CHECK_ARG(children);
     if (nc_dev)
@@ -1125,11 +1143,17 @@
       if (sgnn_fill32(children, 0xFFFFFFFFu, 8 * ldc, s) != SGNN_OK) return SGNN_EHIP;
   }
   if (nf == 0) return SGNN_OK;
-  SGNN_CHECK_ARG(fine_coords && parent && ptable && children);
+  SGNN_CHECK_ARG(fine_coords && parent && children);
   SGNN_LAUNCH(k_down2_tables, dim3(sgnn_grid_for(ldf, 256, 8192)), dim3(256), 0, s,
-                     (const int4 *)fine_coords, parent, nf, children, ldc, ptable, ldf, nc, nf_dev, nc_dev);
+                     (const int4 *)fine_coords, parent, nf, children, ldc, ptable, ldf, nc, nf_dev, nc_dev, pcode);
   SGNN_CHECK_LAUNCH();
   return SGNN_OK;
+}
+
+SGNN_EXPORT int sgnn_down2_tables(const int32_t *fine_coords, const int32_t *parent, int64_t nf,
+                                  int32_t *children, int64_t ldc, int64_t nc, int32_t *ptable, int64_t ldf,
+                                  const int64_t *nf_dev, const int64_t *nc_dev, sgnn_stream_t stream) {
+  return sgnn_down2_tables_pcode(fine_coords, parent, nf, children, ldc, nc, ptable, nullptr, ldf, nf_dev, nc_dev, stream);
 }
 
 __global__ __launch_bounds__(256) void k_expand8(const int4 *__restrict__ coords, int64_t n,
diff --git a/sgnn_amd/csrc/prog.hip b/sgnn_amd/csrc/prog.hip
--- a/sgnn_amd/csrc/prog.hip
+++ b/sgnn_amd/csrc/prog.hip
@@ -50,6 +50,7 @@
   const int64_t *lev_n, *lev_ld;
   void *const *lev_nbr, *const *lev_children, *const *lev_ptable, *const *lev_parent;
   int nlev;
+  bool pcode = false;
   const Op &op(int i) const { return reinterpret_cast<const Op *>(ops)[i]; }
 };
 
@@ -66,6 +67,7 @@
   const int32_t *tab_f = nullptr, *tab_b = nullptr;
   int64_t ld_f = 0, ld_b = 0;
   int flags_b = 0;
+  bool pcode_b = false;
   ConvSetup(const View &v, const Op &o) {
     const bool down = o.type == OP_CONV_DOWN;
     K = o.K();
@@ -78,6 +80,7 @@
     tab_f = (const int32_t *)(down ? v.lev_children[o.lev] : v.lev_nbr[o.lev]);
     ld_f = v.lev_ld[cnt_class];
     tab_b = (const int32_t *)(down ? v.lev_ptable[o.lev] : v.lev_nbr[o.lev]);
+    pcode_b = down && v.pcode;
     ld_b = v.lev_ld[o.lev];
     flags_b = down ? SGNN_CONV_TRANSPOSE_W : (SGNN_CONV_TRANSPOSE_W | SGNN_CONV_FLIP_K);
   }
@@ -905,16 +908,22 @@
       epi.ldx = ld_dy;
       epi.ldy = c.ld(in0);
       epi.n_dev = c.count(o.lev);
-      PROG_TRY(sgnn_conv_fwd_impl(dy, cs.n_out, cout, c.param(o.par), cs.K, cs.tab_b, cs.ld_b, cs.n, cin, g.G(in0), cs.flags_b, 0,
-                                  nullptr, nullptr, 1, 1, cs.K, &epi, c.stream));
+      if (cs.pcode_b)
+        PROG_TRY(sgnn_conv_down2_dx_impl(dy, cs.n_out, cout, c.param(o.par), cs.tab_b, cs.ld_b, cs.n, cin, g.G(in0), &epi, c.stream));
+      else
+        PROG_TRY(sgnn_conv_fwd_impl(dy, cs.n_out, cout, c.param(o.par), cs.K, cs.tab_b, cs.ld_b, cs.n, cin, g.G(in0), cs.flags_b, 0,
+                                    nullptr, nullptr, 1, 1, cs.K, &epi, c.stream));
       g.written(in0);
     } else {
       SGNN_CHECK_ARG(ld_dy == cout);
       float *t = g.target(in0, 0);
       ConvEpi pepi{};
       pepi.n_dev = c.count(o.lev);
-      PROG_TRY(sgnn_conv_fwd_impl(dy, cs.n_out, cout, c.param(o.par), cs.K, cs.tab_b, cs.ld_b, cs.n, cin, t, cs.flags_b, 0, nullptr,
-                                  nullptr, 1, 1, cs.K, &pepi, c.stream));
+      if (cs.pcode_b)
+        PROG_TRY(sgnn_conv_down2_dx_impl(dy, cs.n_out, cout, c.param(o.par), cs.tab_b, cs.ld_b, cs.n, cin, t, &pepi, c.stream));
+      else
+        PROG_TRY(sgnn_conv_fwd_impl(dy, cs.n_out, cout, c.param(o.par), cs.K, cs.tab_b, cs.ld_b, cs.n, cin, t, cs.flags_b, 0, nullptr,
+                                    nullptr, 1, 1, cs.K, &pepi, c.stream));
       PROG_TRY(g.commit(in0, t));
     }
   }
@@ -1090,18 +1099,18 @@
 
 }
 
-SGNN_EXPORT int sgnn_prog_backward(const int32_t *ops, const float *opf, int nops, const int32_t *bufs, int nbuf, int n_ext,
-                                   const int64_t *lev_n, const int64_t *lev_ld, void *const *lev_nbr,
-                                   void *const *lev_children, void *const *lev_ptable, void *const *lev_parent,
-                                   void *const *lev_cnt, int nlev, void *const *params,
-                                   void *const *pgrads, int nparams,
-                                   void *const *ext, void *const *gext, void *const *idx, int nidx,
-                                   const float *arena, float *garena, int64_t arena_floats, void *const *gout,
-                                   const int32_t *keep, int training, void *ws, int64_t ws_bytes,
-                                   sgnn_stream_t stream) {
+static int prog_backward(const int32_t *ops, const float *opf, int nops, const int32_t *bufs, int nbuf, int n_ext,
+                         const int64_t *lev_n, const int64_t *lev_ld, void *const *lev_nbr,
+                         void *const *lev_children, void *const *lev_ptable, bool pcode, void *const *lev_parent,
+                         void *const *lev_cnt, int nlev, void *const *params,
+                         void *const *pgrads, int nparams,
+                         void *const *ext, void *const *gext, void *const *idx, int nidx,
+                         const float *arena, float *garena, int64_t arena_floats, void *const *gout,
+                         const int32_t *keep, int training, void *ws, int64_t ws_bytes,
+                         sgnn_stream_t stream) {
   SGNN_CHECK_ARG(ops && opf && bufs && lev_n && lev_ld && params && pgrads && arena && garena && gout &&
                  n_ext >= 0 && n_ext <= nbuf && (n_ext == 0 || (ext && gext)));
-  Ctx c{View{ops, opf, nops, bufs, nbuf, n_ext, lev_n, lev_ld, lev_nbr, lev_children, lev_ptable, lev_parent, nlev},
+  Ctx c{View{ops, opf, nops, bufs, nbuf, n_ext, lev_n, lev_ld, lev_nbr, lev_children, lev_ptable, lev_parent, nlev, pcode},
         params, idx, lev_cnt, nparams, nidx, training, ws, ws_bytes, stream};
   SGNN_CHECK_ARG(c.prepare(TRAINING, keep));
   if (arena_floats < c.L.total || ws_bytes < ws_need(c.v)) {
@@ -1135,3 +1144,31 @@
   PROG_TRY(g.finish_externals());
   return lane.finish();
 }
+
+SGNN_EXPORT int sgnn_prog_backward(const int32_t *ops, const float *opf, int nops, const int32_t *bufs, int nbuf, int n_ext,
+                                   const int64_t *lev_n, const int64_t *lev_ld, void *const *lev_nbr,
+                                   void *const *lev_children, void *const *lev_ptable, void *const *lev_parent,
+                                   void *const *lev_cnt, int nlev, void *const *params,
+                                   void *const *pgrads, int nparams,
+                                   void *const *ext, void *const *gext, void *const *idx, int nidx,
+                                   const float *arena, float *garena, int64_t arena_floats, void *const *gout,
+                                   const int32_t *keep, int training, void *ws, int64_t ws_bytes,
+                                   sgnn_stream_t stream) {
+  return prog_backward(ops, opf, nops, bufs, nbuf, n_ext, lev_n, lev_ld, lev_nbr, lev_children, lev_ptable, false, lev_parent,
+                       lev_cnt, nlev, params, pgrads, nparams, ext, gext, idx, nidx, arena, garena, arena_floats, gout, keep,
+                       training, ws, ws_bytes, stream);
+}
+
+SGNN_EXPORT int sgnn_prog_backward_pcode(const int32_t *ops, const float *opf, int nops, const int32_t *bufs, int nbuf,
+                                         int n_ext, const int64_t *lev_n, const int64_t *lev_ld, void *const *lev_nbr,
+                                         void *const *lev_children, void *const *lev_pcode, void *const *lev_parent,
+                                         void *const *lev_cnt, int nlev, void *const *params,
+                                         void *const *pgrads, int nparams,
+                                         void *const *ext, void *const *gext, void *const *idx, int nidx,
+                                         const float *arena, float *garena, int64_t arena_floats, void *const *gout,
+                                         const int32_t *keep, int training, void *ws, int64_t ws_bytes,
+                                         sgnn_stream_t stream) {
+  return prog_backward(ops, opf, nops, bufs, nbuf, n_ext, lev_n, lev_ld, lev_nbr, lev_children, lev_pcode, true, lev_parent,
+                       lev_cnt, nlev, params, pgrads, nparams, ext, gext, idx, nidx, arena, garena, arena_floats, gout, keep,
+                       training, ws, ws_bytes, stream);
+}
diff --git a/sgnn_amd/scn/metadata.py b/sgnn_amd/scn/metadata.py
--- a/sgnn_amd/scn/metadata.py
+++ b/sgnn_amd/scn/metadata.py
@@ -211,9 +211,15 @@
 class Down2(object):
     ready = None
 
-    def __init__(self, fine, coarse, parent, children, ldc, ptable, ldf):
+    def __init__(self, fine, coarse, parent, children, ldc, ptable, ldf, pcode):
         self.fine, self.coarse = fine, coarse
-        self.parent, self.children, self.ldc, self.ptable, self.ldf = parent, children, ldc, ptable, ldf
+        self.parent, self.children, self.ldc, self._ptable, self.ldf, self.pcode = parent, children, ldc, ptable, ldf, pcode
+
+    @property
+    def ptable(self):
+        if self._ptable is None:
+            raise _lib.SgnnError('this stride-2 rulebook was built in capacity mode: it has parent codes, no ptable')
+        return self._ptable
 
 
 def build_down2(fine):
@@ -261,8 +267,8 @@
             caps_np = np.ascontiguousarray(np.array(caps, dtype=np.int64))
             ld = [_round_up(max(cap, 1), 256)] + [_round_up(max(c, 1), 256) for c in caps]
             self.children = [mk(8 * ld[l + 1], torch.int32) for l in range(depth)]
-            self.ptable = [mk(8 * ld[l], torch.int32) for l in range(depth)]
-            self._keep += [arr(self.children), arr(self.ptable)]
+            self.pcode = [mk(ld[l], torch.int32) for l in range(depth)]
+            self._keep += [arr(self.children), arr(self.pcode)]
             wsb = _lib.query('sgnn_down2_chain_tables_ws_bytes', cap, depth)
             self.side = None
             if SIDE_PYRAMID:
@@ -278,10 +284,10 @@
                 ws = rt.workspace(wsb)
             with (torch.cuda.stream(self.side) if self.side is not None else _nullcontext()):
                 _lib.stamp('lane<')
-                _lib.call('sgnn_down2_chain_tables', ptr(coords_cap), ptr(n0_cnt), cap, depth,
+                _lib.call('sgnn_down2_chain_tables_pcode', ptr(coords_cap), ptr(n0_cnt), cap, depth,
                           self._keep[0].ctypes.data, self._keep[1].ctypes.data, self.ccap, self._keep[2].ctypes.data,
                           self._keep[3].ctypes.data, ptr(counts), caps_np.ctypes.data, self._keep[4].ctypes.data,
-                          self._keep[5].ctypes.data, ptr(rt.status32), ptr(ws), wsb)
+                          None, self._keep[5].ctypes.data, ptr(rt.status32), ptr(ws), wsb)
             return
         _lib.call('sgnn_down2_chain', ptr(coords_cap), 0 if n0_on_device else int(n0),
                   rt.state.data_ptr() if n0_on_device else None, cap, depth, self._keep[0].ctypes.data,
@@ -306,8 +312,8 @@
         for l in range(self.depth):
             cap_l = min(int(self.level_caps[l]), self.cap)
             coarse = Grid(self.ccoords[l][:cap_l], self.ckeys[l], self.cvals[l], self.ccap, cnt=self.counts[l:l + 1])
-            assert coarse.ld * 8 == self.children[l].numel() and fine.ld * 8 == self.ptable[l].numel()
-            downs.append(Down2(fine, coarse, self.parent[l][:fine.n], self.children[l], coarse.ld, self.ptable[l], fine.ld))
+            assert coarse.ld * 8 == self.children[l].numel() and fine.ld == self.pcode[l].numel()
+            downs.append(Down2(fine, coarse, self.parent[l][:fine.n], self.children[l], coarse.ld, None, fine.ld, self.pcode[l]))
             fine = coarse
         if getattr(self, 'side', None) is not None:
             for d in downs:
@@ -335,9 +341,10 @@
     ldc, ldf = coarse.ld, fine.ld
     children = torch.empty(8 * ldc, dtype=torch.int32, device=dev)
     ptable = torch.empty(8 * ldf, dtype=torch.int32, device=dev)
-    _lib.call('sgnn_down2_tables', ptr(fine.coords), ptr(parent), nf, ptr(children), ldc, nc, ptr(ptable), ldf,
-              ptr(fine.cnt), ptr(coarse.cnt))
-    return Down2(fine, coarse, parent[:nf], children, ldc, ptable, ldf)
+    pcode = torch.empty(ldf, dtype=torch.int32, device=dev)
+    _lib.call('sgnn_down2_tables_pcode', ptr(fine.coords), ptr(parent), nf, ptr(children), ldc, nc, ptr(ptable), ptr(pcode),
+              ldf, ptr(fine.cnt), ptr(coarse.cnt))
+    return Down2(fine, coarse, parent[:nf], children, ldc, ptable, ldf, pcode)
 
 
 class Metadata(object):
diff --git a/sgnn_amd/scn/program.py b/sgnn_amd/scn/program.py
--- a/sgnn_amd/scn/program.py
+++ b/sgnn_amd/scn/program.py
@@ -299,11 +299,11 @@
             nbr[l] = run.grids[l].subm_table().data_ptr()
         pad = [0] * (prog.n_classes - len(run.downs))
         children = [d.children.data_ptr() for d in run.downs] + pad
-        ptable = [d.ptable.data_ptr() for d in run.downs] + pad
+        pcode = [d.pcode.data_ptr() for d in run.downs] + pad
         parent = [d.parent.data_ptr() if d.parent.numel() else 0 for d in run.downs] + pad
         run.lev_n, run.lev_ld = lev_n, lev_ld
         prog.last_lev_n = lev_n.copy()
-        run.tabs = [_ptr_array(v) for v in (nbr, children, ptable, parent, cnts)]
+        run.tabs = [_ptr_array(v) for v in (nbr, children, pcode, parent, cnts)]
         run.pptr = _ptr_array([0 if p is None else p.data_ptr() for p in params])
         run.eptr = _ptr_array([t.data_ptr() for t in ext])
         run.iptr = _ptr_array([t.data_ptr() for t in run.idx] + [0])
@@ -416,7 +416,7 @@
             _deferred.append((arena, garena, held, ext, params, run))
         try:
             _lib.stamp('bwd<')
-            _lib.call('sgnn_prog_backward', ops.ctypes.data, opf.ctypes.data, nops, bufs.ctypes.data, nbuf, n_ext,
+            _lib.call('sgnn_prog_backward_pcode', ops.ctypes.data, opf.ctypes.data, nops, bufs.ctypes.data, nbuf, n_ext,
                       run.lev_n.ctypes.data, run.lev_ld.ctypes.data, run.tabs[0].ctypes.data, run.tabs[1].ctypes.data,
                       run.tabs[2].ctypes.data, run.tabs[3].ctypes.data, run.tabs[4].ctypes.data, ncls,
                       run.pptr.ctypes.data, gp.ctypes.data,
```

After: 5727, median of 2. No clear change (+0.2%).
